# Gabrielcb/DaliID

Measured on AMD Instinct MI355X. Metric: images/sec (train step), higher is better.
Workload: dtype bf16; 1 GPU; configs[1]: ResNet-50 ReID bf16 256x128, PK batch 16x16=256 per GPU, center+proxy heads, Adam, EMA; global_batch=256, per_gpu_batch=256, parallelism=dp1

## Files before the change

### daliid_amd/_lib.py

```python
import ctypes
import os
import threading

import torch

_HERE = os.path.dirname(os.path.abspath(__file__))
LIB_PATH = os.environ.get("DALIID_LIB") or os.path.join(_HERE, "libdaliid_hip.so")

c_void_p, c_int, c_float, c_size_t = ctypes.c_void_p, ctypes.c_int, ctypes.c_float, ctypes.c_size_t


class DaliError(RuntimeError):
    pass


_SIGNATURES = {
    "dali_version": [],
    "dali_last_error": [],
    "dali_ctx_create": [c_int, ctypes.POINTER(c_void_p)],
    "dali_ctx_destroy": [c_void_p],
    "dali_ctx_reserve": [c_void_p, c_size_t],
    "dali_comm_unique_id": [c_void_p],
    "dali_ctx_comm_init": [c_void_p, c_void_p, c_int, c_int],
    "dali_ctx_comm_destroy": [c_void_p],
    "dali_allreduce_bucket": [c_void_p, c_void_p, c_void_p, ctypes.c_int64],
    "dali_l2norm_rows": [c_void_p, c_void_p, c_void_p, c_int, c_int, c_float, c_void_p, c_void_p],
    "dali_l2norm_rows_bwd": [c_void_p, c_void_p, c_void_p, c_void_p, c_int, c_int, c_float, c_void_p],
    "dali_pairdist": [c_void_p, c_void_p, c_void_p, c_void_p, c_int, c_int, c_int, c_int, c_int, c_int, c_void_p],
    "dali_pairdist_operand_bytes": [c_int, c_int, c_int],
    "dali_pairdist_prepare": [c_void_p, c_void_p, c_void_p, c_int, c_int, c_int, c_int, c_void_p, c_void_p],
    "dali_pairdist_prepared": [c_void_p, c_void_p, c_void_p, c_void_p, c_void_p, c_void_p, c_int, c_int, c_int, c_int, c_int,
                               c_void_p],
    "dali_rank_eval": [c_void_p, c_void_p, c_void_p, c_void_p, c_void_p, c_void_p, c_void_p, c_int, c_int, c_int,
                       c_void_p, c_void_p, c_void_p, c_void_p, c_void_p, c_void_p, c_void_p],
    "dali_rank_shard_matches": [c_void_p] * 7 + [c_int] * 4 + [c_void_p] * 3,
    "dali_rank_shard_bins": [c_void_p] * 7 + [c_int] * 3 + [c_void_p, c_void_p, c_int, c_int, c_void_p, c_int, c_void_p],
    "dali_rank_shard_finish": [c_void_p] * 4 + [c_int] * 4 + [c_void_p] * 6,
    "dali_rerank": [c_void_p] * 5 + [c_int] * 4 + [ctypes.c_double, c_void_p],
    "dali_roc_scratch_bytes": [c_int, c_int],
    "dali_roc_build": [c_void_p] * 5 + [c_int, c_int, c_void_p, c_size_t, c_void_p],
    "dali_roc_emit": [c_void_p] * 3 + [c_int, c_int, c_int, ctypes.c_int64, c_void_p, c_void_p, c_void_p],
    "dali_topk_rows": [c_void_p, c_void_p, c_void_p, c_int, c_int, ctypes.c_int64, c_int, c_int, c_int, c_int, c_void_p],
    "dali_topk_decode": [c_void_p, c_void_p, c_void_p, c_int, c_int, c_int, c_void_p, c_void_p],
    "dali_pairdist_topk_scratch_bytes": [c_int] * 7,
    "dali_pairdist_topk": [c_void_p] * 6 + [c_int] * 9 + [c_void_p] + [c_int] * 3 + [c_void_p],
    "dali_conv2d_fwd": [c_void_p, c_void_p, c_void_p, c_void_p, c_void_p] + [c_int] * 9 + [c_void_p, c_void_p, c_int, c_void_p],
    "dali_conv2d_bn_act": [c_void_p, c_void_p, c_void_p, c_void_p, c_void_p] + [c_int] * 9 + [c_void_p, c_void_p, c_int],
    "dali_stem_fused_supported": [c_int, c_int, c_int],
    "dali_stem_conv_bn_maxpool": [c_void_p, c_void_p, c_void_p, c_int, c_int, c_int, c_void_p, c_void_p, c_void_p, c_void_p],
    "dali_conv2d_stat_tiles": [c_int] * 10,
    "dali_conv2d_dgrad": [c_void_p, c_void_p, c_void_p, c_void_p, c_void_p, c_void_p, c_void_p] + [c_int] * 9,
    "dali_conv2d_wgrad": [c_void_p, c_void_p, c_void_p, c_void_p, c_void_p] + [c_int] * 9 + [c_void_p, c_void_p, c_int, c_int],
    "dali_conv1x1_fused": [c_void_p] * 5 + [c_int] * 3 + [c_void_p] * 4 + [c_int, c_void_p, c_void_p, c_void_p],
    "dali_conv1x1_cat": [c_void_p, c_void_p, c_void_p, c_int, c_void_p, c_int, c_void_p, c_void_p, c_void_p, c_int, c_int],
    "dali_conv1x1_cat_act": [c_void_p, c_void_p, c_void_p, c_int, c_void_p, c_int, c_void_p, c_int, c_void_p, c_void_p, c_int, c_void_p, c_int, c_int],
    "dali_bnlin_fwd": [c_void_p] * 4 + [c_int] * 3 + [c_void_p] * 4 + [c_float, c_float] + [c_void_p] * 7,
    "dali_bnlin_bwd": [c_void_p] * 5 + [c_int] * 3 + [c_void_p] * 11,
    "dali_bn_finalize": [c_void_p, c_void_p, c_void_p, c_int, c_int, ctypes.c_double, c_void_p, c_void_p, c_void_p, c_void_p,
                         c_float, c_float, c_void_p, c_void_p, c_void_p, c_void_p],
    "dali_bn_act": [c_void_p] * 9 + [c_int, ctypes.c_int64, c_int, c_void_p, c_void_p],
    "dali_bn_bwd": [c_void_p, c_void_p, c_void_p, c_void_p, c_void_p, c_int, ctypes.c_int64, c_int] + [c_void_p] * 16,
    "dali_maxpool_bn_fwd": [c_void_p] * 5 + [c_int] * 4 + [c_void_p, c_void_p],
    "dali_maxpool_bn_bwd": [c_void_p] * 8 + [c_int] * 4 + [c_void_p, c_void_p, c_void_p],
    "dali_head_pool_fwd": [c_void_p, c_void_p, c_void_p, c_int, c_int, c_int, c_int, c_void_p, c_void_p],
    "dali_head_pool_bwd": [c_void_p, c_void_p, c_void_p, c_void_p, c_int, c_int, c_int, c_int, c_void_p],
    "dali_bn1d_fwd": [c_void_p, c_void_p, c_void_p, c_int, c_int, c_void_p, c_void_p, c_void_p, c_void_p, c_int, c_float, c_float,
                      c_void_p, c_void_p, c_void_p],
    "dali_bn1d_bwd": [c_void_p, c_void_p, c_void_p, c_void_p, c_int, c_int] + [c_void_p] * 6,
    "dali_linear_fwd": [c_void_p] * 5 + [c_int] + [c_void_p] * 3 + [c_int] * 3,
    "dali_linear_fwd_scaled": [c_void_p] * 5 + [c_int] + [c_void_p] * 3 + [c_int] * 3,
    "dali_linear_dgrad": [c_void_p] * 7 + [c_int] * 3,
    "dali_linear_wgrad": [c_void_p] * 6 + [c_int] * 3,
    "dali_vit_patchify": [c_void_p, c_void_p, c_void_p] + [c_int] * 5 + [c_void_p],
    "dali_vit_assemble_tokens": [c_void_p] * 5 + [c_int] * 3 + [c_void_p],
    "dali_vit_assemble_tokens_bwd": [c_void_p] * 3 + [c_int] * 3 + [c_void_p] * 3,
    "dali_vit_assemble_tokens_sie": [c_void_p] * 7 + [c_int, c_float] + [c_int] * 3 + [c_void_p],
    "dali_vit_sie_grad": [c_void_p] * 4 + [c_int] * 4 + [c_float, c_void_p],
    "dali_vit_jpm_gather": [c_void_p] * 4 + [c_int] * 5 + [c_void_p],
    "dali_vit_jpm_head": [c_void_p] * 8 + [c_int] * 3 + [c_void_p],
    "dali_layernorm_fwd": [c_void_p] * 5 + [c_int, c_int, c_float] + [c_void_p] * 3,
    "dali_layernorm_bwd": [c_void_p] * 8 + [c_int, c_int] + [c_void_p] * 3,
    "dali_attention_fwd": [c_void_p] * 3 + [c_int] * 4 + [c_float, c_void_p, c_void_p],
    "dali_attention_fwd_short": [c_void_p] * 3 + [c_int] * 4 + [c_float, c_void_p, c_void_p],
    "dali_attention_bwd": [c_void_p] * 6 + [c_int] * 4 + [c_float, c_void_p],
    "dali_center_loss_fwd": [c_void_p] * 6 + [c_float, c_int, c_int, c_void_p, c_void_p],
    "dali_center_loss_bwd": [c_void_p] * 6 + [c_float, c_int, c_int, c_void_p, c_float, c_void_p],
    "dali_proxy_loss_fwd": [c_void_p] * 6 + [c_float, c_int, c_int] + [c_void_p] * 5,
    "dali_proxy_loss_bwd": [c_void_p] * 5 + [c_int, c_int, c_void_p, c_float, c_int, c_void_p],
    "dali_proxy_kmax": [],
    "dali_adam_step": [c_void_p] * 6 + [ctypes.c_int64, c_float, c_float, c_float, c_float, c_float, c_int, c_float, c_void_p],
    "dali_ema_update": [c_void_p, c_void_p, c_void_p, c_void_p, ctypes.c_int64, c_float],
    "dali_triplet_loss_fwd": [c_void_p, c_void_p, c_void_p, c_void_p, c_void_p, c_float, c_int, c_void_p, c_void_p, c_void_p, c_void_p,
                              c_void_p],
    "dali_triplet_loss_bwd": [c_void_p, c_void_p, c_void_p, c_void_p, c_int, c_void_p, c_float, c_void_p],
    "dali_pairdist_blend": [c_void_p, c_void_p, c_void_p, c_void_p, c_int, c_int, c_int, c_int, c_int, c_void_p, c_void_p, c_void_p,
                            c_void_p, c_void_p],
    "dali_class_targets": [c_void_p, c_void_p, c_void_p, c_int, c_int, c_void_p, c_void_p, c_int, c_void_p, c_int, c_void_p, c_void_p,
                           c_void_p, c_void_p],
    "dali_resize_bicubic_u8": [c_void_p] * 7 + [c_int, c_int, c_void_p, c_void_p, c_int, c_void_p, c_void_p, c_int, c_int, c_int, c_void_p],
    "dali_augment_batch": [c_void_p, c_void_p, c_void_p, c_void_p, c_int, c_int, c_int, ctypes.POINTER(c_float), ctypes.POINTER(c_float), c_void_p],
    "dali_augment_gather": [c_void_p, c_void_p, c_void_p, ctypes.c_int64, c_void_p, c_void_p, c_int, c_int, c_int, ctypes.POINTER(c_float),
                            ctypes.POINTER(c_float), c_void_p],
    "dali_gemm_profile_begin": [c_void_p, c_int],
    "dali_gemm_profile_end": [c_void_p, c_void_p, c_void_p, c_void_p],
    "dali_resnet_create": [c_void_p, c_void_p, ctypes.POINTER(c_void_p)],
    "dali_resnet_destroy": [c_void_p],
    "dali_resnet_set_feature": [c_void_p, c_int],
    "dali_resnet_sizes": [c_void_p] + [c_void_p] * 6,
    "dali_resnet_tensor_info": [c_void_p, c_int, c_int, c_void_p, c_int, c_void_p, c_void_p, c_void_p, c_void_p],
    "dali_resnet_stage_param_range": [c_void_p, c_int, c_void_p, c_void_p],
    "dali_resnet_bind": [c_void_p, c_void_p, c_void_p, c_void_p, c_void_p, c_size_t],
    "dali_resnet_refresh_weights": [c_void_p, c_void_p],
    "dali_resnet_forward": [c_void_p, c_void_p, c_void_p, c_int, c_void_p],
    "dali_resnet_backward": [c_void_p, c_void_p, c_void_p, c_int, c_int],
    "dali_resnet_debug_tensor": [c_void_p, ctypes.c_char_p, c_void_p, c_void_p],
    "dali_vit_create": [c_void_p, c_void_p, ctypes.POINTER(c_void_p)],
    "dali_vit_create_ex": [c_void_p, c_void_p, c_void_p, ctypes.POINTER(c_void_p)],
    "dali_vit_destroy": [c_void_p],
    "dali_vit_sizes": [c_void_p] + [c_void_p] * 6,
    "dali_vit_tensor_info": [c_void_p, c_int, c_int, c_void_p, c_int, c_void_p, c_void_p, c_void_p, c_void_p],
    "dali_vit_bind": [c_void_p, c_void_p, c_void_p, c_void_p, c_void_p, c_size_t],
    "dali_vit_refresh_weights": [c_void_p, c_void_p],
    "dali_vit_forward": [c_void_p, c_void_p, c_void_p, c_int, c_void_p, c_void_p],
    "dali_vit_forward_ex": [c_void_p, c_void_p, c_void_p, c_void_p, c_int, c_void_p, c_void_p, c_void_p],
    "dali_vit_backward": [c_void_p, c_void_p, c_void_p],
    "dali_vit_num_stages": [c_void_p],
    "dali_vit_stage_param_range": [c_void_p, c_int, c_void_p, c_void_p],
    "dali_vit_backward_stages": [c_void_p, c_void_p, c_void_p, c_int, c_int],
    "dali_vit_set_drop_path": [c_void_p, c_void_p],
}
_RESTYPES = {"dali_last_error": ctypes.c_char_p, "dali_pairdist_operand_bytes": ctypes.c_size_t, "dali_roc_scratch_bytes": ctypes.c_size_t,
             "dali_pairdist_topk_scratch_bytes": ctypes.c_size_t}

_lock = threading.Lock()
# ... 90 lines not shown
```

### daliid_amd/csrc/conv.hip

```cpp
#include "gemm_tile.h"
#include "kernels.h"
#include <cstdlib>
#include <type_traits>
#include <vector>
#include <string>
#include <cstdio>

namespace dali {

__device__ __forceinline__ void decode_pixel(const GatherGeom& g, int p, int& n, int& ho, int& wo) {
    if (g.lhw >= 0 && g.lw >= 0) {
        n = p >> g.lhw;
        const int rem = p & ((1 << g.lhw) - 1);
        ho = rem >> g.lw;
        wo = rem & ((1 << g.lw) - 1);
    } else {
        const int hw = g.Hout * g.Wout;
        n = p / hw;
        const int rem = p - n * hw;
        ho = rem / g.Wout;
        wo = rem - ho * g.Wout;
    }
}

// ... 86 lines not shown
        X = a.X; sc = a.in_scale; sh = a.in_shift; g = a.g; relu = a.in_relu;
        kc = threadIdx.x & 3;
        tiles_per_tap = g.Ck >> 5;
#pragma unroll
        for (int i = 0; i < BCH; ++i) {
            const int row = (threadIdx.x + i * 256) >> 2;
            const int p = p0 + row;
            ok[i] = p < a.P;
            int n = 0, ho = 0, wo = 0;
            if (ok[i]) decode_pixel(g, p, n, ho, wo);
            img_base[i] = (long long)n * g.img_pitch;
            if (g.mode == 0) { h0[i] = ho * g.stride - g.pad; w0[i] = wo * g.stride - g.pad; }
            else { h0[i] = ho + g.pad; w0[i] = wo + g.pad; }
        }
    }
    __device__ __forceinline__ uint4 operator()(int , int row, int kt, int ) const {
        const int i = row >> 6;
        const int tap = kt / tiles_per_tap;
        const int c0 = (kt - tap * tiles_per_tap) * 32 + kc * 8;
        const int r = tap / g.S, s = tap - r * g.S;
        long long off = -1;
#pragma unroll
        for (int t = 0; t < BCH; ++t)
            if (t == i && ok[t]) off = tap_offset(g, img_base[t], h0[t], w0[t], r, s);
        if (off < 0) return make_uint4(0, 0, 0, 0);
        uint4 v = *reinterpret_cast<const uint4*>(X + off + c0);
        if constexpr (IN_BN) v = bn_relu_chunk(v, sc + c0, sh + c0, relu);
        return v;
    }
};

struct WeightLoader {
    const uint16_t* W; int m0, Cm, K;
    __device__ __forceinline__ uint4 operator()(int , int row, int kt, int kc) const {
        const int m = m0 + row;
        if (m >= Cm) return make_uint4(0, 0, 0, 0);
        return *reinterpret_cast<const uint4*>(W + (size_t)m * K + kt * 32 + kc * 8);
    }
};

__device__ __forceinline__ void lds_barrier() {
    asm volatile("s_waitcnt lgkmcnt(0)" ::: "memory");
    __builtin_amdgcn_s_barrier();
}
__device__ __forceinline__ void lds_barrier_vm() {
    asm volatile("s_waitcnt vmcnt(0) lgkmcnt(0)" ::: "memory");
    __builtin_amdgcn_s_barrier();
}

__device__ __forceinline__ float row16_sum(float v) {
    v += __builtin_bit_cast(float, __builtin_amdgcn_update_dpp(0, __builtin_bit_cast(int, v), 0x128, 0xf, 0xf, false));
    v += __builtin_bit_cast(float, __builtin_amdgcn_update_dpp(0, __builtin_bit_cast(int, v), 0x124, 0xf, 0xf, false));
    v += __builtin_bit_cast(float, __builtin_amdgcn_update_dpp(0, __builtin_bit_cast(int, v), 0x122, 0xf, 0xf, false));
    v += __builtin_bit_cast(float, __builtin_amdgcn_update_dpp(0, __builtin_bit_cast(int, v), 0x121, 0xf, 0xf, false));
    return v;
}

#define DALI_DPP(v, CTRL) __builtin_bit_cast(float, __builtin_amdgcn_update_dpp(0, __builtin_bit_cast(int, (v)), (CTRL), 0xf, 0xf, false))
__device__ __forceinline__ float row16_reduce8(const float (&v)[8], int lane) {
    const bool hi8 = (lane & 8) != 0, hi4 = (lane & 4) != 0, hi2 = (lane & 2) != 0;
    float a[4], b[2];
#pragma unroll
    for (int k = 0; k < 4; ++k) {
        const float keep = hi8 ? v[4 + k] : v[k], send = hi8 ? v[k] : v[4 + k];
        a[k] = keep + DALI_DPP(send, 0x140);
    }
#pragma unroll
    for (int k = 0; k < 2; ++k) {
        const float keep = hi4 ? a[2 + k] : a[k], send = hi4 ? a[k] : a[2 + k];
        b[k] = keep + DALI_DPP(send, 0x141);
    }
    const float keep = hi2 ? b[1] : b[0], send = hi2 ? b[0] : b[1];
    const float c = keep + DALI_DPP(send, 0x4e);
    return c + DALI_DPP(c, 0xb1);
}

enum class Epi : int {
    CONV = 0,
    LIN = 1,
    GENERAL = 2,
    FUSED = 3,
    PARITY = 4,
    FUSED_LEAN = 5,
};
constexpr Epi epi_mode(bool own, Epi asked) { return own ? asked : Epi::GENERAL; }
constexpr bool epi_fused(Epi m) { return m == Epi::FUSED || m == Epi::FUSED_LEAN; }

__device__ __forceinline__ uint32_t gate_bf16x2(uint32_t w, unsigned bits) {
    const uint32_t lo = (uint32_t)__builtin_amdgcn_sbfe((int)bits, 0, 1) & 0xffffu;
    const uint32_t hi = (uint32_t)__builtin_amdgcn_sbfe((int)bits, 1, 1) << 16;
    return w & (lo | hi);
}
__device__ __forceinline__ void gate_bf16x8(uint4& v, unsigned m) {
    v.x = gate_bf16x2(v.x, m); v.y = gate_bf16x2(v.y, m >> 2); v.z = gate_bf16x2(v.z, m >> 4); v.w = gate_bf16x2(v.w, m >> 6);
}
__device__ __forceinline__ void gelu_parts(float v, float& cdf, float& pdf) {
    const float z = fabsf(v) * 0.70710678118654752f;
    const float e = __builtin_amdgcn_exp2f(-(z * z) * 1.44269504088896341f);
    const float t = __builtin_amdgcn_rcpf(__builtin_fmaf(0.3275911f, z, 1.0f));
    float poly = __builtin_fmaf(1.061405429f, t, -1.453152027f);
    poly = __builtin_fmaf(poly, t, 1.421413741f);
    poly = __builtin_fmaf(poly, t, -0.284496736f);
    poly = __builtin_fmaf(poly, t, 0.254829592f);
    const float erf_abs = __builtin_fmaf(-(poly * t), e, 1.0f);
    cdf = __builtin_fmaf(0.5f, copysignf(erf_abs, v), 0.5f);
    pdf = 0.3989422804014327f * e;
}
__device__ __forceinline__ float gelu_f(float v) { float c, p; gelu_parts(v, c, p); return v * c; }
__device__ __forceinline__ float gelu_grad_f(float x) { float c, p; gelu_parts(x, c, p); return __builtin_fmaf(x, p, c); }
__device__ __forceinline__ void unpack4(uint2 q, float (&f)[4]) {
    f[0] = bf16_bits_to_f32(q.x & 0xffffu); f[1] = bf16_bits_to_f32(q.x >> 16); f[2] = bf16_bits_to_f32(q.y & 0xffffu); f[3] = bf16_bits_to_f32(q.y >> 16);
}
__device__ __forceinline__ uint2 pack4(const float (&v)[4]) { return make_uint2(pack_bf16x2(v[0], v[1]), pack_bf16x2(v[2], v[3])); }
template <int FM>
__device__ __forceinline__ void load_rows4(float4 (&d)[FM], const float* vec) {
#pragma unroll
    for (int i = 0; i < FM; ++i) d[i] = *reinterpret_cast<const float4*>(vec + i * 16);
}
__device__ __forceinline__ unsigned pos_bits_bf16x2(uint32_t w) {
    return ((int)(int16_t)(w & 0xffffu) > 0 ? 1u : 0u) | (((int)w >> 16) > 0 ? 2u : 0u);
}
template <int TM, int TN, int FM_, int FN_, int WNW, int NT>
__device__ __forceinline__ void conv_epilogue_cols(const IGemmArgs& a, f32x4_t (&acc)[FM_][FN_], int tm, int tn, uint16_t* smem, int wm, int wn) {
    constexpr int ROWB = TM * 4 + 16, ROWS = WNW * 16, CPR = TM / 8, ITERS = ROWS * CPR / NT;
    static_assert(ROWS * CPR % NT == 0 && NT % CPR == 0, "staged store: threads must tile the column block evenly");
    const int lane = threadIdx.x & 63;
    const int mb = wm * (FM_ * 16) + (lane >> 4) * 4;
    char* stage = reinterpret_cast<char*>(smem);
    char* my_stage = stage + (wn * 16 + (lane & 15)) * ROWB + mb * 4;
    const int ch = threadIdx.x % CPR, lp0 = threadIdx.x / CPR;
    const uint16_t* in_tile = a.Res ? a.Res : a.dact_pre;
    const float* bias_c = a.bias ? a.bias + tm * TM + ch * 8 : nullptr;
#pragma unroll
    for (int j = 0; j < FN_; ++j) {
        uint32_t gofs[ITERS];
        uint4 tin[ITERS];
#pragma unroll
        for (int it = 0; it < ITERS; ++it) {
            const int lp = lp0 + it * (NT / CPR);
            const int pix = tn * TN + (lp >> 4) * (FN_ * 16) + j * 16 + (lp & 15);
            gofs[it] = ((uint32_t)pix * (uint32_t)a.Cm + (uint32_t)(tm * TM + ch * 8)) * 2u;
            if (in_tile) tin[it] = *reinterpret_cast<const uint4*>(reinterpret_cast<const char*>(in_tile) + gofs[it]);
        }
#pragma unroll
        for (int i = 0; i < FM_; ++i) *reinterpret_cast<f32x4_t*>(my_stage + i * 64) = acc[i][j];
        lds_barrier();
#pragma unroll
        for (int it = 0; it < ITERS; ++it) {
            const int lp = lp0 + it * (NT / CPR);
            float v[8];
            *reinterpret_cast<float4*>(v) = *reinterpret_cast<const float4*>(stage + lp * ROWB + ch * 32);
            *reinterpret_cast<float4*>(v + 4) = *reinterpret_cast<const float4*>(stage + lp * ROWB + ch * 32 + 16);
            if (bias_c) {
                const float4 b0 = *reinterpret_cast<const float4*>(bias_c), b1 = *reinterpret_cast<const float4*>(bias_c + 4);
                v[0] += b0.x; v[1] += b0.y; v[2] += b0.z; v[3] += b0.w; v[4] += b1.x; v[5] += b1.y; v[6] += b1.z; v[7] += b1.w;
            }
            if (a.O2) *reinterpret_cast<uint4*>(reinterpret_cast<char*>(a.O2) + gofs[it]) = pack8(v);
            if (a.act == 1) {
#pragma unroll
                for (int t = 0; t < 8; ++t) v[t] = gelu_f(v[t]);
            }
            if (a.dact_pre) {
                float x8[8];
                unpack8(tin[it], x8);
#pragma unroll
                for (int t = 0; t < 8; ++t) v[t] *= gelu_grad_f(x8[t]);
            }
            if (a.row_scale) {
// ... 43 lines not shown
    __device__ __forceinline__ uint4 in(const uint16_t* src, int h, int it) const {
        return *reinterpret_cast<const uint4*>(reinterpret_cast<const char*>(src) + offset(h, it));
    }
    __device__ __forceinline__ void out(uint16_t* dst, int h, int it) const {
        *reinterpret_cast<uint4*>(reinterpret_cast<char*>(dst) + offset(h, it)) = *chunk(it);
    }
};

template <int TM, int TN, int FM, int FN, int WNW, int NT>
__device__ __forceinline__ void epi_stats(const IGemmArgs& a, f32x4_t (&acc)[FM][FN], int tm, int tn, uint16_t* smem, int wn, int mb) {
    const int lane = threadIdx.x & 63;
    float* red = reinterpret_cast<float*>(reinterpret_cast<char*>(smem) + epi_stage_bytes(TM, TN));
#pragma unroll
    for (int i = 0; i < FM; ++i) {
        float s1[4] = {0.f, 0.f, 0.f, 0.f}, s2[4] = {0.f, 0.f, 0.f, 0.f};
#pragma unroll
        for (int j = 0; j < FN; ++j)
#pragma unroll
            for (int r = 0; r < 4; ++r) { const float v = acc[i][j][r]; s1[r] += v; s2[r] = __builtin_fmaf(v, v, s2[r]); }
        const float v8[8] = {s1[0], s1[1], s1[2], s1[3], s2[0], s2[1], s2[2], s2[3]};
        const float tot = row16_reduce8(v8, lane);
        if ((lane & 1) == 0) {
            const int r = ((lane & 4) >> 1) | ((lane & 2) >> 1);
            red[(wn * TM + mb + i * 16 + r) * 2 + ((lane >> 3) & 1)] = tot;
        }
    }
    lds_barrier();
    for (int t = threadIdx.x; t < TM; t += NT) {
        const int c = tm * TM + t;
        if (c < a.Cm) {
            float s1 = 0.f, s2 = 0.f;
#pragma unroll
            for (int w = 0; w < WNW; ++w) { const float2 v = *reinterpret_cast<const float2*>(red + (w * TM + t) * 2); s1 += v.x; s2 += v.y; }
            *reinterpret_cast<float2*>(a.stats + ((size_t)tn * a.Cm + c) * 2) = make_float2(s1, s2);
        }
    }
}
template <bool SUB, int TM, int TN, int FM, int FN, int WNW, int NT>
__device__ __forceinline__ void epi_store_lean(const IGemmArgs& a, f32x4_t (&acc)[FM][FN], int tm, int tn, uint16_t* smem, int wn, int mb) {
    using Stage = EpiStage<SUB, TM, TN, FM, FN, WNW, NT>;
    constexpr int ITERS = Stage::ITERS;
    const Stage st(a, tm, tn, smem, wn, mb);
    float4 bias4[FM];
#pragma unroll
    for (int i = 0; i < FM; ++i)
        bias4[i] = a.bias ? *reinterpret_cast<const float4*>(a.bias + tm * TM + mb + i * 16) : make_float4(0.f, 0.f, 0.f, 0.f);
#pragma unroll
    for (int h = 0; h < 2; ++h) {
        if (a.Res) {
            unsigned rm[ITERS];
            if (a.res_mask) {
#pragma unroll
                for (int it = 0; it < ITERS; ++it) rm[it] = a.res_mask[st.offset(h, it) >> 4];
            }
#pragma unroll
            for (int it = 0; it < ITERS; ++it) {
                uint4 rv = st.in(a.Res, h, it);
                if (a.res_mask) gate_bf16x8(rv, rm[it]);
                *st.chunk(it) = rv;
            }
            lds_barrier_vm();
        }
#pragma unroll
        for (int jj = 0; jj < Stage::HFN; ++jj) {
            const int j = h * Stage::HFN + jj;
#pragma unroll
            for (int i = 0; i < FM; ++i) {
                float v[4] = {acc[i][j][0] + bias4[i].x, acc[i][j][1] + bias4[i].y, acc[i][j][2] + bias4[i].z, acc[i][j][3] + bias4[i].w};
                uint2* slot = st.slot(jj, i);
                if (a.Res) {
                    float r4[4];
                    unpack4(*slot, r4);
                    v[0] += r4[0]; v[1] += r4[1]; v[2] += r4[2]; v[3] += r4[3];
                }
                *slot = pack4(v);
            }
        }
        lds_barrier();
        conv_stamp(a, 6 + 2 * h);
#pragma unroll
        for (int it = 0; it < ITERS; ++it) st.out(a.O, h, it);
        conv_stamp(a, 7 + 2 * h);
        if (h == 0) lds_barrier();
    }
}
template <int TM, int TN, int FM, int FN, int WNW, int NT>
__device__ __forceinline__ void epi_store_lin(const IGemmArgs& a, f32x4_t (&acc)[FM][FN], int tm, int tn, uint16_t* smem, int wn, int mb) {
    using Stage = EpiStage<false, TM, TN, FM, FN, WNW, NT>;
    constexpr int ITERS = Stage::ITERS;
    const Stage st(a, tm, tn, smem, wn, mb);
    const int lane = threadIdx.x & 63;
    float4 bias4[FM];
#pragma unroll
    for (int i = 0; i < FM; ++i)
        bias4[i] = a.bias ? *reinterpret_cast<const float4*>(a.bias + tm * TM + mb + i * 16) : make_float4(0.f, 0.f, 0.f, 0.f);
    const uint16_t* in_tile = a.Res ? a.Res : a.dact_pre;
#pragma unroll
    for (int h = 0; h < 2; ++h) {
        if (a.O2) {
#pragma unroll
            for (int jj = 0; jj < Stage::HFN; ++jj) {
                const int j = h * Stage::HFN + jj;
#pragma unroll
                for (int i = 0; i < FM; ++i) {
                    const float v[4] = {acc[i][j][0] + bias4[i].x, acc[i][j][1] + bias4[i].y, acc[i][j][2] + bias4[i].z, acc[i][j][3] + bias4[i].w};
                    *st.slot(jj, i) = pack4(v);
                }
            }
            lds_barrier();
#pragma unroll
            for (int it = 0; it < ITERS; ++it) st.out(a.O2, h, it);
            lds_barrier();
        }
        if (in_tile) {
#pragma unroll
            for (int it = 0; it < ITERS; ++it) *st.chunk(it) = st.in(in_tile, h, it);
            lds_barrier_vm();
        }
#pragma unroll
        for (int jj = 0; jj < Stage::HFN; ++jj) {
            const int j = h * Stage::HFN + jj;
#pragma unroll
            for (int i = 0; i < FM; ++i) {
                float v[4] = {acc[i][j][0] + bias4[i].x, acc[i][j][1] + bias4[i].y, acc[i][j][2] + bias4[i].z, acc[i][j][3] + bias4[i].w};
                uint2* slot = st.slot(jj, i);
                if (a.act == 1) {
#pragma unroll
                    for (int t = 0; t < 4; ++t) v[t] = gelu_f(v[t]);
                }
                if (a.row_scale) {
                    const float rs = a.row_scale[tn * TN + h * Stage::WROWS + wn * (FN * 16) + jj * 16 + (lane & 15)];
                    v[0] *= rs; v[1] *= rs; v[2] *= rs; v[3] *= rs;
                }
                if (in_tile) {
                    float x4[4];
                    unpack4(*slot, x4);
                    if (a.Res) {
                        v[0] += x4[0]; v[1] += x4[1]; v[2] += x4[2]; v[3] += x4[3];
                    } else {
#pragma unroll
                        for (int t = 0; t < 4; ++t) v[t] *= gelu_grad_f(x4[t]);
                    }
                }
                *slot = pack4(v);
            }
        }
        lds_barrier();
        conv_stamp(a, 6 + 2 * h);
#pragma unroll
        for (int it = 0; it < ITERS; ++it) st.out(a.O, h, it);
        conv_stamp(a, 7 + 2 * h);
        if (h == 0) lds_barrier();
    }
}
template <bool FULL, int TM, int TN, int FM, int FN, int WNW, int NT>
__device__ __forceinline__ void epi_store_fused(const IGemmArgs& a, f32x4_t (&acc)[FM][FN], int tm, int tn, uint16_t* smem, int wn, int mb) {
    using Stage = EpiStage<false, TM, TN, FM, FN, WNW, NT>;
    constexpr int ITERS = Stage::ITERS;
    const Stage st(a, tm, tn, smem, wn, mb);
    const uint16_t* const Res = FULL ? a.Res : nullptr;
    const uint8_t* const out_mask = FULL ? a.out_mask : nullptr;
    uint8_t* const bits_out = FULL ? a.bits_out : nullptr;
    float4 sc4[FM], sh4[FM];
#pragma unroll
    for (int i = 0; i < FM; ++i) { sc4[i] = make_float4(1.f, 1.f, 1.f, 1.f); sh4[i] = make_float4(0.f, 0.f, 0.f, 0.f); }
    if (a.out_scale) load_rows4(sc4, a.out_scale + tm * TM + mb);
// ... 61 lines not shown
            if (bits_out) bits_out[ob >> 4] = (uint8_t)(pos_bits_bf16x2(v.x) | (pos_bits_bf16x2(v.y) << 2) | (pos_bits_bf16x2(v.z) << 4) | (pos_bits_bf16x2(v.w) << 6));
        }
        if (h == 0) lds_barrier();
    }
}
template <Epi MODE, int TM, int TN, int FM, int FN>
__device__ __forceinline__ void epi_store_general(const IGemmArgs& a, f32x4_t (&acc)[FM][FN], int tm, int tn, int mb, int nb) {
    const int lane = threadIdx.x & 63;
#pragma unroll
    for (int j = 0; j < FN; ++j) {
        const int p = tn * TN + nb + j * 16;
        const size_t opix = (p < a.P) ? out_pixel(a.g, p) : 0;
#pragma unroll
        for (int i = 0; i < FM; ++i) {
            const int c = tm * TM + mb + i * 16;
            unsigned nib = 0;
            if (p < a.P && c < a.Cm) {
                float v[4] = {acc[i][j][0], acc[i][j][1], acc[i][j][2], acc[i][j][3]};
                const size_t o = opix * a.Cm + c;
                if constexpr (epi_fused(MODE)) {
                    if (a.out_scale) { const float4 sv = *reinterpret_cast<const float4*>(a.out_scale + c); v[0] *= sv.x; v[1] *= sv.y; v[2] *= sv.z; v[3] *= sv.w; }
                    if (a.out_shift) { const float4 sv = *reinterpret_cast<const float4*>(a.out_shift + c); v[0] += sv.x; v[1] += sv.y; v[2] += sv.z; v[3] += sv.w; }
                }
                if (a.bias) {
                    const float4 bv = *reinterpret_cast<const float4*>(a.bias + c);
                    v[0] += bv.x; v[1] += bv.y; v[2] += bv.z; v[3] += bv.w;
                }
                if constexpr (MODE == Epi::LIN || MODE == Epi::GENERAL) {
                    if (a.O2) *reinterpret_cast<uint2*>(a.O2 + o) = pack4(v);
                    if (a.act == 1) {
#pragma unroll
                        for (int t = 0; t < 4; ++t) v[t] = gelu_f(v[t]);
                    }
                    if (a.dact_pre) {
                        float x4[4];
                        unpack4(*reinterpret_cast<const uint2*>(a.dact_pre + o), x4);
#pragma unroll
                        for (int t = 0; t < 4; ++t) v[t] *= gelu_grad_f(x4[t]);
                    }
                    if (a.row_scale) {
                        const float rs = a.row_scale[p];
                        v[0] *= rs; v[1] *= rs; v[2] *= rs; v[3] *= rs;
                    }
                }
                if (MODE != Epi::FUSED_LEAN && a.Res) {
                    uint2 rv = *reinterpret_cast<const uint2*>(a.Res + o);
                    if constexpr (MODE != Epi::FUSED) if (a.res_mask) {
                        const unsigned m = a.res_mask[o >> 3] >> (o & 4);
                        rv.x = gate_bf16x2(rv.x, m); rv.y = gate_bf16x2(rv.y, m >> 2);
                    }
                    float r4[4];
                    unpack4(rv, r4);
                    if constexpr (MODE == Epi::FUSED) if (a.res_scale) {
                        const float4 rs = *reinterpret_cast<const float4*>(a.res_scale + c);
                        r4[0] *= rs.x; r4[1] *= rs.y; r4[2] *= rs.z; r4[3] *= rs.w;
                    }
                    v[0] += r4[0]; v[1] += r4[1]; v[2] += r4[2]; v[3] += r4[3];
                }
                if constexpr (epi_fused(MODE)) if (a.out_relu) { v[0] = fmaxf(v[0], 0.f); v[1] = fmaxf(v[1], 0.f); v[2] = fmaxf(v[2], 0.f); v[3] = fmaxf(v[3], 0.f); }
                uint2 ov = pack4(v);
                if constexpr (MODE == Epi::FUSED) {
                    if (a.out_mask) {
                        const unsigned m = a.out_mask[o >> 3] >> (o & 4);
                        ov.x = gate_bf16x2(ov.x, m); ov.y = gate_bf16x2(ov.y, m >> 2);
                    }
                    nib = pos_bits_bf16x2(ov.x) | (pos_bits_bf16x2(ov.y) << 2);
                }
                *reinterpret_cast<uint2*>(a.O + o) = ov;
            }
            if constexpr (MODE == Epi::FUSED) {
                const unsigned other = __shfl_xor(nib, 16, 64);
                if (a.bits_out && p < a.P && c < a.Cm && ((lane >> 4) & 1) == 0) a.bits_out[(opix * a.Cm + c) >> 3] = (uint8_t)(nib | (other << 4));
            }
        }
    }
}

template <int TM, int TN, int FM, int FN, int WNW, int NT, Epi MODE = Epi::GENERAL>
__device__ __forceinline__ void conv_epilogue_g(const IGemmArgs& a, f32x4_t (&acc)[FM][FN], int tm, int tn, uint16_t* smem, int wm, int wn) {
    constexpr bool EVEN = FN % 2 == 0;
    constexpr bool FUSED = epi_fused(MODE), SUB = MODE == Epi::PARITY;
    const int lane = threadIdx.x & 63;
    const int mb = wm * (FM * 16) + (lane >> 4) * 4, nb = wn * (FN * 16) + (lane & 15);
    if (a.stats) epi_stats<TM, TN, FM, FN, WNW, NT>(a, acc, tm, tn, smem, wn, mb);
    conv_stamp(a, 5);
    const bool interior = (tm + 1) * TM <= a.Cm && (tn + 1) * TN <= a.P;
    const bool chunks = (a.Cm & 7) == 0;
    const bool extras = a.O2 || a.act != 0 || a.dact_pre || a.row_scale;
    const bool plain = !FUSED && !extras && (SUB || !a.g.sub) && chunks;
    const bool in_once = !(a.Res && a.dact_pre);
    if constexpr (!EVEN) {
        if (interior && !FUSED && !a.g.sub && chunks && in_once && (unsigned long long)a.P * a.Cm * 2ull < 0xffffffffull)
            return conv_epilogue_cols<TM, TN, FM, FN, WNW, NT>(a, acc, tm, tn, smem, wm, wn);
    } else if constexpr (FUSED) {
        if (interior && !a.g.sub && chunks) return epi_store_fused<MODE == Epi::FUSED, TM, TN, FM, FN, WNW, NT>(a, acc, tm, tn, smem, wn, mb);
    } else {
        if (interior && plain) return epi_store_lean<SUB, TM, TN, FM, FN, WNW, NT>(a, acc, tm, tn, smem, wn, mb);
        if constexpr (MODE == Epi::LIN)
            if (interior && !plain && !a.g.sub && chunks && in_once) return epi_store_lin<TM, TN, FM, FN, WNW, NT>(a, acc, tm, tn, smem, wn, mb);
    }
    epi_store_general<MODE, TM, TN, FM, FN>(a, acc, tm, tn, mb, nb);
}
template <class Cfg, Epi MODE = Epi::GENERAL>
__device__ __forceinline__ void conv_epilogue(const IGemmArgs& a, f32x4_t (&acc)[Cfg::FM][Cfg::FN], int tm, int tn, uint16_t* smem) {
    const int wave = threadIdx.x >> 6;
    conv_epilogue_g<Cfg::TM, Cfg::TN, Cfg::FM, Cfg::FN, 2, 256, MODE>(a, acc, tm, tn, smem, wave >> 1, wave & 1);
}

template <int TM, int TN, bool IN_BN>
__global__ __launch_bounds__(256) void igemm_conv_kernel(IGemmArgs a, int tiles_m, int tiles_n) {
    using Cfg = GemmCfg<TM, TN, 1, 1, 1>;
    extern __shared__ __attribute__((aligned(16))) uint16_t smem[];
    int tm, tn;
    if (!xcd_tile_map(blockIdx.x, tiles_m, tiles_n, tm, tn)) return;
    f32x4_t acc[Cfg::FM][Cfg::FN];
#pragma unroll
    for (int i = 0; i < Cfg::FM; ++i)
#pragma unroll
        for (int j = 0; j < Cfg::FN; ++j) acc[i][j] = f32x4_t{0.f, 0.f, 0.f, 0.f};
    const int K = a.g.R * a.g.S * a.g.Ck;
    WeightLoader la{a.W, tm * TM, a.Cm, K};
    PixelLoader<TN, IN_BN> lb;
    lb.init(a, tn * TN);
    gemm_mainloop<Cfg>(acc, la, lb, K >> 5, smem);

    conv_epilogue<Cfg>(a, acc, tm, tn, smem);
}


template <int KT, int TM, int TN, int NW, bool SRC2>
struct ConvGather {
    static_assert(KT == 32 || KT == 64, "k-tile depth");
    static constexpr int ROWS = 512 / KT;
    static constexpr int A_BLK = TM / ROWS / NW, B_BLK = (TN / ROWS + NW - 1) / NW;
    static constexpr bool B_RAGGED = (TN / ROWS) % NW != 0;
    static constexpr int NDMA = A_BLK + B_BLK;
    static_assert(TM % (ROWS * NW) == 0 && TN % ROWS == 0, "DMA pieces: whole pieces, the weight pieces evenly over the waves");
    static_assert(KT == 64 || !B_RAGGED, "k-tile 32: the pixel pieces must divide evenly over the waves");
    static_assert(KT == 32 || NW % 2 == 0, "k-tile 64: an even number of issuing waves (piece wave + NW * i keeps the wave's parity)");
    static_assert(!(SRC2 && B_RAGGED), "the two-tensor branch has no ragged skip");

    const GatherGeom& g;
    int wave, Ck1, Ck2;
    __amdgpu_buffer_rsrc_t rs_w, rs_x, rs_x2;
    int kc;
    uint32_t a_off[A_BLK];
    int b_pix[B_BLK], b_h0[B_BLK], b_w0[B_BLK];
    int kr, ks, kc0, ks_end, kr_end;

    __device__ __forceinline__ ConvGather(const IGemmArgs& a, const GatherGeom& g_, int tm, int tn, int wave_, int lane) : g(g_) {
        wave = wave_;
        const int K = g.R * g.S * g.Ck;
        rs_w = __builtin_amdgcn_make_buffer_rsrc(const_cast<uint16_t*>(a.W), 0, a.Cm * K * 2, 0x00020000);
        const long long x_bytes = SRC2 ? (long long)a.P * a.Ck1 * 2 : (long long)g.img_pitch * 2 * ((a.P + g.Hout * g.Wout - 1) / (g.Hout * g.Wout));
        rs_x = __builtin_amdgcn_make_buffer_rsrc(const_cast<uint16_t*>(a.X), 0, (int)x_bytes, 0x00020000);
        Ck1 = a.Ck1; Ck2 = g.Ck - a.Ck1;
        rs_x2 = __builtin_amdgcn_make_buffer_rsrc(const_cast<uint16_t*>(SRC2 ? a.X2 : a.X), 0, SRC2 ? (int)((long long)a.P * Ck2 * 2) : (int)x_bytes, 0x00020000);
        int r_in;
        if constexpr (KT == 32) { r_in = lane >> 2; kc = (lane & 3) ^ lds_swz(r_in); }
        else { r_in = lane >> 3; kc = (lane & 7) ^ (((wave & 1) << 2) | (r_in >> 1)); }
#pragma unroll
        for (int i = 0; i < A_BLK; ++i) {
            const int m = tm * TM + ROWS * (wave + NW * i) + r_in;
            a_off[i] = (m < a.Cm) ? (uint32_t)(m * K + kc * 8) * 2u : DMA_OOB;
        }
#pragma unroll
// ... 1255 lines not shown
    return (P + tn - 1) / tn;
}


struct GemmProfiler {
    std::vector<hipEvent_t> ev;
    std::vector<int> cls;
    std::vector<double> flops;
    std::vector<std::string> desc;
    size_t used = 0, cap = 0;
};
static GemmProfiler* g_prof = nullptr;
struct ProfScope {
    hipStream_t st; bool on = false; size_t i = 0;
    ProfScope(hipStream_t s, int cls, double flops, const char* what = "") : st(s) {
        if (!g_prof || g_prof->used >= g_prof->cap) return;
        on = true; i = g_prof->used++;
        g_prof->cls[i] = cls; g_prof->flops[i] = flops; g_prof->desc[i] = what;
        (void)hipEventRecord(g_prof->ev[2 * i], st);
    }
    ~ProfScope() { if (on) (void)hipEventRecord(g_prof->ev[2 * i + 1], st); }
};

int gemm_profile_begin(hipStream_t st, int cls, double flops, const char* what) {
    if (!g_prof || g_prof->used >= g_prof->cap) return -1;
    const size_t i = g_prof->used++;
    g_prof->cls[i] = cls; g_prof->flops[i] = flops; g_prof->desc[i] = what;
    (void)hipEventRecord(g_prof->ev[2 * i], st);
    return (int)i;
}
void gemm_profile_end(hipStream_t st, int slot) {
    if (slot >= 0 && g_prof) (void)hipEventRecord(g_prof->ev[2 * slot + 1], st);
}

enum GemmGrid {
    GRID_XCD,
    GRID_CLASSES,
    GRID_CUS,
    GRID_HALO,
    GRID_SPLITS,
    GRID_SPLITS8,
};
struct GemmKernel {
    const void* fn;
    int block;
    int lds;
    int tm, tn;
    GemmGrid grid;
    int plan_wgs = 0;
    int f1_rb = 0;
    mutable DeviceOnce once{};
};
template <class F> static const void* kfn(F* f) { return reinterpret_cast<const void*>(f); }
constexpr int ring_lds(int tm, int tn, int k_tile, int stages) { return (tm + tn) * k_tile * 2 * stages; }
constexpr int REG128_LDS = GemmCfg<128, 128, 1, 1, 1>::LDS_BYTES, REG64_LDS = GemmCfg<64, 256, 1, 1, 1>::LDS_BYTES;
constexpr int DMA128_LDS = REG128_LDS / 2 * 3, DMA64_LDS = REG64_LDS / 2 * 3;
constexpr int HALO64_LDS = (3 * 64 * 64 + HALO64_PX * 64) * 2;

static const GemmKernel
    CONV128_BN{kfn(&igemm_conv_kernel<128, 128, true>), 256, REG128_LDS, 128, 128, GRID_XCD},
    CONV128{kfn(&igemm_conv_kernel<128, 128, false>), 256, REG128_LDS, 128, 128, GRID_XCD},
    DMA128{kfn(&igemm_conv_dma_kernel<128, 128, 3>), 256, DMA128_LDS, 128, 128, GRID_XCD},
    DMA128_LIN{kfn(&igemm_conv_dma_kernel<128, 128, 3, Epi::LIN>), 256, DMA128_LDS, 128, 128, GRID_XCD},
    DMA128_FUSED{kfn(&igemm_conv_dma_kernel<128, 128, 3, Epi::FUSED>), 256, DMA128_LDS, 128, 128, GRID_XCD},
    DMA128_CLS{kfn(&igemm_conv_dma_kernel<128, 128, 3, Epi::PARITY>), 256, DMA128_LDS, 128, 128, GRID_CLASSES},
    DMA128_SRC2{kfn(&igemm_conv_dma_kernel<128, 128, 3, Epi::CONV, true>), 256, DMA128_LDS, 128, 128, GRID_XCD},
    CONV64_BN{kfn(&igemm_conv_kernel<64, 256, true>), 256, REG64_LDS, 64, 256, GRID_XCD},
    CONV64{kfn(&igemm_conv_kernel<64, 256, false>), 256, REG64_LDS, 64, 256, GRID_XCD},
    DMA64{kfn(&igemm_conv_dma_kernel<64, 256, 3>), 256, DMA64_LDS, 64, 256, GRID_XCD},
    DMA64_LEAN{kfn(&igemm_conv_dma_kernel<64, 256, 3, Epi::FUSED_LEAN>), 256, DMA64_LDS, 64, 256, GRID_XCD},
    DMA64_SRC2{kfn(&igemm_conv_dma_kernel<64, 256, 3, Epi::CONV, true>), 256, DMA64_LDS, 64, 256, GRID_XCD},
    K64S64{kfn(&igemm_conv_k64s_kernel<1, 4, 4, 2>), 512, ring_lds(64, 256, 64, 2), 64, 256, GRID_XCD},
    HALO64{kfn(&igemm_conv_halo64_kernel<3>), 512, HALO64_LDS, 64, 256, GRID_HALO},
    HALO64_LEAN{kfn(&igemm_conv_halo64_kernel<3, Epi::FUSED_LEAN>), 512, HALO64_LDS, 64, 256, GRID_HALO},
    WG128{kfn(&igemm_conv_wg_kernel<2, 4, 3>), 512, ring_lds(128, 256, 32, 3), 128, 256, GRID_XCD},
    WG128_LIN{kfn(&igemm_conv_wg_kernel<2, 4, 3, Epi::LIN>), 512, ring_lds(128, 256, 32, 3), 128, 256, GRID_XCD},
    WG128_FUSED{kfn(&igemm_conv_wg_kernel<2, 4, 3, Epi::FUSED>), 512, ring_lds(128, 256, 32, 3), 128, 256, GRID_XCD},
    WG128_CLS{kfn(&igemm_conv_wg_kernel<2, 4, 3, Epi::PARITY>), 512, ring_lds(128, 256, 32, 3), 128, 256, GRID_CLASSES},
    WG256{kfn(&igemm_conv_wg_kernel<4, 4, 4>), 1024, ring_lds(256, 256, 32, 4), 256, 256, GRID_XCD},
    K64S{kfn(&igemm_conv_k64s_kernel<2, 4, 8, 3>), 1024, ring_lds(128, 256, 64, 3), 128, 256, GRID_XCD},
    K64S_LIN{kfn(&igemm_conv_k64s_kernel<2, 4, 8, 3, 4, 4, Epi::LIN>), 1024, ring_lds(128, 256, 64, 3), 128, 256, GRID_XCD},
    K64S_LEAN{kfn(&igemm_conv_k64s_kernel<2, 4, 8, 3, 4, 4, Epi::FUSED_LEAN>), 1024, ring_lds(128, 256, 64, 3), 128, 256, GRID_XCD},
    K64S_SRC2{kfn(&igemm_conv_k64s_kernel<2, 4, 8, 3, 4, 4, Epi::CONV, true>), 1024, ring_lds(128, 256, 64, 3), 128, 256, GRID_XCD},
    K64{kfn(&igemm_conv_k64_kernel<4, 4, 2>), 1024, ring_lds(256, 256, 64, 2), 256, 256, GRID_XCD},
    K64_LIN{kfn(&igemm_conv_k64_kernel<4, 4, 2, 4, 4, Epi::LIN>), 1024, ring_lds(256, 256, 64, 2), 256, 256, GRID_XCD},
    K64_FUSED{kfn(&igemm_conv_k64_kernel<4, 4, 2, 4, 4, Epi::FUSED>), 1024, ring_lds(256, 256, 64, 2), 256, 256, GRID_XCD},
    K64_CLS{kfn(&igemm_conv_k64_kernel<4, 4, 2, 4, 4, Epi::PARITY>), 1024, ring_lds(256, 256, 64, 2), 256, 256, GRID_CLASSES},
    K64_SRC2{kfn(&igemm_conv_k64_kernel<4, 4, 2, 4, 4, Epi::CONV, true>), 1024, ring_lds(256, 256, 64, 2), 256, 256, GRID_XCD},
    K64_FUSED_SRC2{kfn(&igemm_conv_k64_kernel<4, 4, 2, 4, 4, Epi::FUSED, true>), 1024, ring_lds(256, 256, 64, 2), 256, 256, GRID_XCD},
    K64_320{kfn(&igemm_conv_k64_kernel<4, 4, 2, 4, 5, Epi::LIN>), 1024, ring_lds(256, 320, 64, 2), 256, 320, GRID_XCD};

template <int RB, bool RES, bool OM, bool BITS, bool SRC2 = false>
static GemmKernel f1_kernel() {
    return {kfn(&fused1x1_persist_kernel<3, RB, RES, OM, BITS, SRC2>), (F1_NC + F1_NP + F1_NR) * 64, f1_lds_bytes(3, RB, RB == 2 ? 128 : F1_KMAX),
            F1_TM, F1_TN, GRID_CUS, 0, RB};
}
static const GemmKernel F1[2][2][2][2] = {
    {{{f1_kernel<2, false, false, false, true>(), f1_kernel<2, false, false, true>()}, {f1_kernel<2, false, true, false>(), f1_kernel<2, false, true, true>()}},
     {{f1_kernel<2, true, false, false>(), f1_kernel<2, true, false, true>()}, {f1_kernel<2, true, true, false>(), f1_kernel<2, true, true, true>()}}},
    {{{f1_kernel<1, false, false, false, true>(), f1_kernel<1, false, false, true>()}, {f1_kernel<1, false, true, false>(), f1_kernel<1, false, true, true>()}},
     {{f1_kernel<1, true, false, false>(), f1_kernel<1, true, false, true>()}, {f1_kernel<1, true, true, false>(), f1_kernel<1, true, true, true>()}}}};

static const GemmKernel
    WG_BN{kfn(&igemm_wgrad_kernel<true>), 256, 0, 128, 128, GRID_SPLITS},
    WG_PLAIN{kfn(&igemm_wgrad_kernel<false>), 256, 0, 128, 128, GRID_SPLITS},
    WG_3X3{kfn(&igemm_wgrad3x3_kernel<3>), 512, 3 * W3_STAGE * 2, 128, 9 * 64, GRID_SPLITS8, 256};
static const GemmKernel WG_DMA[2] = {
    {kfn(&igemm_wgrad_dma_kernel<false>), 256, 0, 128, 128, GRID_SPLITS8},
    {kfn(&igemm_wgrad_dma_kernel<true>), 256, 0, 128, 128, GRID_SPLITS8}};
static const GemmKernel WG_WG[2] = {
    {kfn(&igemm_wgrad_wg_kernel<2, 4, 3>), 512, ring_lds(128, 256, 32, 3), 128, 256, GRID_SPLITS8, 512},
    {kfn(&igemm_wgrad_wg_kernel<2, 4, 3, true>), 512, ring_lds(128, 256, 32, 3), 128, 256, GRID_SPLITS8, 512}};
static const GemmKernel WG_P[2][2] = {
    {{kfn(&igemm_wgrad_p_kernel<2, 4, 4, 4, 8, 6>), 1024, ring_lds(128, 256, 32, 6), 128, 256, GRID_SPLITS8, 256},
     {kfn(&igemm_wgrad_p_kernel<2, 4, 4, 4, 8, 6, true>), 1024, ring_lds(128, 256, 32, 6), 128, 256, GRID_SPLITS8, 256}},
    {{kfn(&igemm_wgrad_p_kernel<1, 4, 8, 4, 4, 6>), 512, ring_lds(128, 256, 32, 6), 128, 256, GRID_SPLITS8, 256},
     {kfn(&igemm_wgrad_p_kernel<1, 4, 8, 4, 4, 6, true>), 512, ring_lds(128, 256, 32, 6), 128, 256, GRID_SPLITS8, 256}}};

struct GemmChoice {
    const GemmKernel* k = nullptr;
    int tiles_m = 0, tiles_n = 0, lds = 0, class_grid = 0;
    unsigned grid = 0;
    int rc = DALI_OK, why_arg = 0;
    const char* why = nullptr;
    GemmChoice() = default;
    GemmChoice(int rc_, const char* why_, int why_arg_ = 0) : rc(rc_), why_arg(why_arg_), why(why_) {}
    int refuse() const { set_error(why, why_arg); return rc; }
};
static GemmChoice gemm_place(const GemmKernel& k, int rows, int cols, int mult, int Ck) {
    GemmChoice c;
    c.k = &k;
    c.tiles_m = (rows + k.tm - 1) / k.tm;
    c.tiles_n = (cols + k.tn - 1) / k.tn;
    c.lds = k.f1_rb ? f1_lds_bytes(3, k.f1_rb, Ck) : k.lds;
    switch (k.grid) {
        case GRID_XCD: c.grid = xcd_tile_grid(c.tiles_m, c.tiles_n); break;
        case GRID_CLASSES: c.class_grid = xcd_tile_grid(c.tiles_m, c.tiles_n); c.grid = mult * c.class_grid; break;
        case GRID_CUS: c.grid = mult; break;
        case GRID_HALO: c.grid = c.tiles_n; break;
        case GRID_SPLITS: c.grid = c.tiles_m * c.tiles_n * mult; break;
        case GRID_SPLITS8: c.grid = (c.tiles_m * c.tiles_n * mult + 7) / 8 * 8; break;
    }
    return c;
}
template <class Args>
static int gemm_launch(hipStream_t st, const GemmChoice& c, Args& args) {
    const GemmKernel& k = *c.k;
    DeviceOnce::Guard once(k.once);
    if (k.lds > 64 * 1024 && once.first()) {
        DALI_HIP(hipFuncSetAttribute(k.fn, hipFuncAttributeMaxDynamicSharedMemorySize, k.lds));
        once.done();
    }
    int tiles_m = c.tiles_m, tiles_n = c.tiles_n;
    void* tile_args[] = {&args, &tiles_m, &tiles_n};
    void* halo_args[] = {&args, &tiles_n};
    (void)hipLaunchKernel(k.fn, dim3(c.grid), dim3(k.block), k.grid == GRID_HALO ? halo_args : tile_args, c.lds, st);
    DALI_LAUNCH_CHECK();
    return DALI_OK;
}

static unsigned long long* g_conv_stamps = nullptr;

static bool dma_addressable(long long bytes) { return bytes < 0x7ff00000ll; }
static bool gather_dma_ok(const GatherGeom& g, int P, long long other_bytes) {
    return dma_addressable(g.img_pitch * 2 * ((P + g.Hout * g.Wout - 1) / (g.Hout * g.Wout))) && dma_addressable(other_bytes);
}
static bool conv_dma_ok(const IGemmArgs& a) { return !a.in_scale && gather_dma_ok(a.g, a.P, (long long)a.Cm * a.g.R * a.g.S * a.g.Ck * 2); }
static bool plain_rows(const GatherGeom& g) {
    return g.R == 1 && g.S == 1 && g.stride == 1 && g.pad == 0 && g.pix_pitch == g.Ck && g.row_pitch == g.Win * g.Ck &&
           g.img_pitch == (long long)g.Hin * g.Win * g.Ck && g.Hin == g.Hout && g.Win == g.Wout;
}
static bool halo64_ok(const IGemmArgs& a) {
// ... 9 lines not shown
        int dev = 0, v = 0;
        if (hipGetDevice(&dev) != hipSuccess || hipDeviceGetAttribute(&v, hipDeviceAttributeMultiprocessorCount, dev) != hipSuccess) { set_error("conv: device query failed"); return -1; }
        n_cus = v > 8 ? v & ~7 : 8;
    }
    return n_cus;
}
static bool f1_fills(int Cm, int P, int n_cus) {
    const int tiles_m = Cm / F1_TM, tiles_n = (P + F1_TN - 1) / F1_TN;
    return n_cus > 0 && (long long)tiles_m * tiles_n >= 2ll * n_cus && (n_cus / 8) % tiles_m == 0;
}
static bool cat_act_ok(int Cm, int c1, int c2, int P, int parts, int n_cus) {
    const int K = parts * (c1 + c2);
    if (parts != 1 && parts != 2) return false;
    if ((c1 & 63) || (c2 & 63) || (Cm % 128) || !dma_addressable((long long)P * Cm * 2) || !dma_addressable((long long)P * K * 2)) return false;
    if (K <= F1_KMAX) return f1_fills(Cm, P, n_cus);
    return parts == 1 && K >= 1024 && conv_pick_cfg(Cm, P, K) == CONV_256x256;
}
bool conv_cat_act_supported(int Cm, int c1, int c2, int P, int parts) { return cat_act_ok(Cm, c1, c2, P, parts, f1_cu_count()); }

static GemmChoice conv_choose(const IGemmArgs& a, int n_cus) {
    const GatherGeom& g = a.g;
    const bool in_bn = a.in_scale != nullptr, narrow = a.Cm <= 64, dma_ok = conv_dma_ok(a);
    const int K = g.nr * g.ns * g.Ck;
    const bool fused = a.out_scale || a.out_shift || a.out_relu || a.bits_out || a.out_mask || a.res_scale;
    const bool lin = a.act != 0 || a.O2 != nullptr || a.dact_pre != nullptr || a.row_scale != nullptr;
    if (a.res_mask && (fused || lin))
        return GemmChoice(DALI_ERR_INVALID, "conv: a residual mask goes with neither a fused output stage nor the linear-layer extras");
    int cfg = conv_pick_cfg(a.Cm, a.P, K);
    if (dma_ok && !a.stats && !fused && !g.sub && g.Ck % 64 == 0 && (a.Cm & 7) == 0 && conv_prefers_320(a.Cm, a.P, K)) cfg = CONV_256x320;
    if (!dma_ok && !in_bn && a.stats && (cfg == CONV_128x256 || cfg == CONV_256x256))
        return GemmChoice(DALI_ERR_LIMIT, "conv: tensors beyond 2 GiB are not supported together with the BatchNorm statistics epilogue");
    bool k64 = dma_ok && !narrow && g.Ck % 64 == 0;
    const bool narrow_k64 = dma_ok && narrow && g.Ck % 64 == 0 && K >= 512 && !a.X2;
    if (a.X2) {
        const bool fo_simple = !a.bits_out && !a.out_mask && !a.res_scale && !a.Res && (a.out_scale || a.out_shift || a.out_relu);
        const int xr = a.x_rep > 1 ? a.x_rep : 1, c2 = g.Ck / xr - a.Ck1;
        if (xr > 1 && !(fo_simple && g.Ck % xr == 0 && cat_act_ok(a.Cm, a.Ck1, c2, a.P, xr, n_cus) && g.Ck <= F1_KMAX))
            return GemmChoice(DALI_ERR_INVALID, "conv: split weight images (x_rep = %d) are served by the persistent streaming kernel only (K <= 256, >= 2 tiles per CU)", xr);
        if (fo_simple && ((a.Ck1 & 63) || (c2 & 63) || (a.Cm % 128)))
            return GemmChoice(DALI_ERR_INVALID, "conv: two operand tensors with a fused output stage need channel counts that are multiples of 64 and Cm %% 128 == 0");
        if (in_bn || !dma_ok || a.stats || (fused && !fo_simple) || lin || g.sub || g.R != 1 || g.S != 1 || g.stride != 1 || g.pad != 0 || a.Ck1 <= 0 ||
            a.Ck1 >= g.Ck / xr || (a.Ck1 & 31) || (c2 & 31) || (a.Cm & 7))
            return GemmChoice(DALI_ERR_INVALID, "conv: a second operand tensor needs a plain 1x1 / stride 1 problem with both channel counts multiples of 32");
        if ((a.Ck1 & 63) || (c2 & 63)) k64 = false;
    }
    if (k64 && cfg != CONV_256x320 && !((K >= 1024 && (cfg == CONV_256x256 || cfg == CONV_128x256)) || (K >= 768 && cfg == CONV_256x256))) k64 = false;
    if (a.X2 && !narrow && !(k64 && (cfg == CONV_256x256 || cfg == CONV_128x256))) { cfg = CONV_128; k64 = false; }
    auto use = [&](const GemmKernel& k) { return gemm_place(k, a.Cm, a.P, k.grid == GRID_CUS ? n_cus : (g.sub == 2 ? 4 : 1), g.Ck); };
    if (fused) {
        if (in_bn || !dma_ok || (a.Cm & 7) || lin)
            return GemmChoice(DALI_ERR_INVALID, "conv: the fused output stage needs Cm %% 8 == 0, tensors below 2 GiB, no operand transform and no linear-layer extras");
        if (plain_rows(g) && !g.sub && a.Cm % F1_TM == 0 && (g.Ck & 63) == 0 && g.Ck <= F1_KMAX && dma_addressable((long long)a.P * a.Cm * 2) &&
            (a.Res || a.out_mask || a.bits_out || a.X2)) {
            if (n_cus <= 0) return GemmChoice(DALI_ERR_HIP, "conv: device query failed");
            if (f1_fills(a.Cm, a.P, n_cus)) return use(F1[g.Ck > 128][a.Res != nullptr][a.out_mask != nullptr][a.bits_out != nullptr]);
        }
        const bool lean = !a.Res && !a.out_mask && !a.bits_out && !a.res_scale && !a.X2;
        if (lean && narrow_k64 && halo64_ok(a)) return use(HALO64_LEAN);
        if (lean && narrow) return use(DMA64_LEAN);
        if (lean && k64 && cfg == CONV_128x256 && !g.sub) return use(K64S_LEAN);
        if (a.X2) {
            if (!(k64 && cfg == CONV_256x256))
                return GemmChoice(DALI_ERR_INVALID, "conv: two operand tensors with a fused output stage need K <= 256 or a 256 x 256 k-tile-64 problem (K >= 1024, Cm >= 512, >= 16384 pixels)");
            return use(K64_FUSED_SRC2);
        }
        if (k64 && cfg == CONV_256x256) return use(K64_FUSED);
        return use(cfg == CONV_128x256 || cfg == CONV_256x256 ? WG128_FUSED : DMA128_FUSED);
    }
    if (g.sub && dma_ok && !narrow && !lin && (a.Cm & 7) == 0) {
        if (k64 && cfg == CONV_256x256) return use(K64_CLS);
        return use(cfg == CONV_128x256 || cfg == CONV_256x256 ? WG128_CLS : DMA128_CLS);
    }
    if (cfg == CONV_256x320) return use(K64_320);
    if (k64 && cfg == CONV_256x256) return use(a.X2 ? K64_SRC2 : lin ? K64_LIN : K64);
    if (k64 && cfg == CONV_128x256) return use(a.X2 ? K64S_SRC2 : lin ? K64S_LIN : K64S);
    if (narrow_k64 && !lin && halo64_ok(a)) return use(HALO64);
    if (narrow_k64) return use(K64S64);
    if (narrow) return use(in_bn ? CONV64_BN : !dma_ok ? CONV64 : a.X2 ? DMA64_SRC2 : DMA64);
    if (dma_ok && cfg == CONV_256x256) return use(WG256);
    if (dma_ok && cfg == CONV_128x256) return use(lin ? WG128_LIN : WG128);
    return use(in_bn ? CONV128_BN : !dma_ok ? CONV128 : a.X2 ? DMA128_SRC2 : lin ? DMA128_LIN : DMA128);
}

static int launch_igemm_conv_one(hipStream_t st, const IGemmArgs& a) {
    IGemmArgs args = a;
    args.g.lw = ilog2_exact(a.g.Wout);
    args.g.lhw = ilog2_exact(a.g.Hout * a.g.Wout);
    const GemmChoice c = conv_choose(args, f1_cu_count());
    if (c.rc == DALI_ERR_LIMIT) return c.refuse();
    const int K = a.g.nr * a.g.ns * a.g.Ck;
    char what[160] = "";
    if (g_prof)
        snprintf(what, sizeof what, "%s,Cm=%d,K=%d,P=%d,taps=%d,stride=%d,sub=%d,fused=%d,stats=%d,res=%d,mask=%d,lin=%d", a.g.mode ? "dgrad" : "fwd", a.Cm, K, a.P,
                 a.g.R * a.g.S, a.g.stride, a.g.sub, a.out_scale ? 1 : 0, a.stats ? 1 : 0, a.Res ? 1 : 0, (a.res_mask || a.out_mask) ? 1 : 0,
                 (a.bias || a.row_scale || a.act) ? 1 : 0);
    ProfScope prof_scope(st, 0, a.g.sub == 2 ? 2.0 * a.Cm * (double)a.P * a.g.R * a.g.S * a.g.Ck : 2.0 * a.Cm * (double)a.P * K, what);
    if (!c.k) return c.refuse();
    const int stat_tiles = a.stats ? igemm_conv_stat_tiles(a.Cm, a.P, K, a.in_scale != nullptr) : c.tiles_n;
    if (stat_tiles != c.tiles_n) {
        set_error("conv: the statistics slab has %d pixel tiles, the chosen kernel %d", stat_tiles, c.tiles_n);
        return DALI_ERR_UNSUPPORTED;
    }
    if (c.k->grid == GRID_CLASSES) args.g.class_grid = c.class_grid;
    return gemm_launch(st, c, args);
}

int launch_igemm_conv(hipStream_t st, const IGemmArgs& a) {
    IGemmArgs args = a;
    args.stamps = g_conv_stamps;
    GatherGeom& g = args.g;
    g.sub = 0; g.oph = g.opw = 0; g.Hfull = g.Hout; g.Wfull = g.Wout;
    g.r0 = 0; g.rstep = 1; g.nr = g.R; g.s0 = 0; g.sstep = 1; g.ns = g.S;
    if (g.mode == 1 && g.stride == 2 && conv_dma_ok(args) && !a.stats && (g.Hout % 2) == 0 && (g.Wout % 2) == 0 &&
        ilog2_exact(g.Wout / 2) >= 0 && ilog2_exact((g.Hout / 2) * (g.Wout / 2)) >= 0) {
        int nr[2], ns[2];
        for (int ph = 0; ph < 2; ++ph) {
            const int r0 = (ph + g.pad) & 1, s0 = (ph + g.pad) & 1;
            nr[ph] = r0 < g.R ? (g.R - r0 + 1) / 2 : 0;
            ns[ph] = s0 < g.S ? (g.S - s0 + 1) / 2 : 0;
        }
        const bool all_have = nr[0] && nr[1] && ns[0] && ns[1];
        if (all_have && a.Cm > 64 && (a.Cm & 7) == 0) {
            IGemmArgs s = args;
            s.g.sub = 2; s.g.oph = s.g.opw = 0; s.g.Hfull = g.Hout; s.g.Wfull = g.Wout;
            s.g.Hout = g.Hout / 2; s.g.Wout = g.Wout / 2; s.P = a.P / 4;
            s.g.r0 = s.g.s0 = 0; s.g.rstep = s.g.sstep = 2;
            s.g.nr = nr[0] > nr[1] ? nr[0] : nr[1]; s.g.ns = ns[0] > ns[1] ? ns[0] : ns[1];
            return launch_igemm_conv_one(st, s);
        }
        if (all_have || (a.Res != nullptr && a.Res == a.O)) {
            for (int ph = 0; ph < 2; ++ph)
                for (int pw = 0; pw < 2; ++pw) {
                    if (nr[ph] * ns[pw] == 0) continue;
                    IGemmArgs s = args;
                    s.g.sub = 1; s.g.oph = ph; s.g.opw = pw; s.g.Hfull = g.Hout; s.g.Wfull = g.Wout;
                    s.g.Hout = g.Hout / 2; s.g.Wout = g.Wout / 2; s.P = a.P / 4;
                    s.g.r0 = (ph + g.pad) & 1; s.g.rstep = 2; s.g.nr = nr[ph];
                    s.g.s0 = (pw + g.pad) & 1; s.g.sstep = 2; s.g.ns = ns[pw];
                    const int rc = launch_igemm_conv_one(st, s);
                    if (rc) return rc;
                }
            return DALI_OK;
        }
    }
    return launch_igemm_conv_one(st, args);
}

static bool wgrad_spec(int Cm, int Ntot) { return ((Cm + 127) / 128) * ((Ntot + 255) / 256) <= 100; }
static int wgrad_pick_cfg(int Cm, int Ntot, int taps, int P, int halo_w) {
    if (taps == 9 && (halo_w == 8 || halo_w == 16 || halo_w == 32) && Cm % 64 == 0 && (Ntot / 9) % 64 == 0 && P % 32 == 0) return 3;
    if (taps == 7 && Ntot == 224 && P >= 16384) return 2;
    return (taps == 1 && Ntot >= 256 && P >= 16384) ? 2 : 0;
}
static const GemmKernel& wgrad_kernel(int cfg, int Cm, int Ntot, bool in_bn, bool dma_ok, bool colsum, bool flat) {
    if (in_bn) return WG_BN;
    if (!dma_ok) return WG_PLAIN;
    if (cfg == 3) return WG_3X3;
    if (cfg == 2) return wgrad_spec(Cm, Ntot) ? WG_P[flat][colsum] : WG_WG[colsum];
    return WG_DMA[colsum];
}
static bool wgrad_colsum_ok(int cfg, bool in_bn, bool dma_ok) { return cfg != 3 && !in_bn && dma_ok; }
static int colsum_rows_of(const GemmKernel& k, int Ntot, int splits) { return k.tn == 128 ? splits : splits * ((Ntot + k.tn - 1) / k.tn); }

static void wgrad_plan(int Cm, int Ntot, int P, int target_blocks, int* splits, int* pix_per_split, int taps, int halo_w) {
    const GemmKernel& k = wgrad_kernel(wgrad_pick_cfg(Cm, Ntot, taps, P, halo_w), Cm, Ntot, false, true, false, true);
    if (k.plan_wgs) target_blocks = k.plan_wgs;
    const int tiles = ((Cm + k.tm - 1) / k.tm) * ((Ntot + k.tn - 1) / k.tn);
    int sp = (target_blocks + tiles - 1) / tiles;
    const int max_sp = (P + 255) / 256;
    if (sp > max_sp) sp = max_sp;
    if (sp < 1) sp = 1;
    {
        int best = sp;
        double best_cost = (double)((tiles * sp + target_blocks - 1) / target_blocks) / sp;
        for (int c = sp - 1; c >= 1 && c >= sp / 2; --c) {
            const double cost = (double)((tiles * c + target_blocks - 1) / target_blocks) / c;
            if (cost <= best_cost + 1e-12) { best = c; best_cost = cost; }
        }
        sp = best;
    }
    int pps = ((P + sp - 1) / sp + 31) & ~31;
    sp = (P + pps - 1) / pps;
    *splits = sp; *pix_per_split = pps;
}

static int wgrad_halo_w(const GatherGeom& g, bool in_bn) {
    const bool halo = !in_bn && g.R == 3 && g.S == 3 && g.stride == 1 && g.pad == 1 && g.mode == 0 && ilog2_exact(g.Wout) >= 0 &&
                      ilog2_exact(g.Hout * g.Wout) >= 7 && g.Hin == g.Hout && g.Win == g.Wout && g.pix_pitch == g.Ck && g.row_pitch == g.Win * g.Ck;
    return halo ? g.Wout : 0;
}

struct WGradChoice { int Ntot, splits, pix_per_split, colsum_rows; GemmChoice c; };
static WGradChoice wgrad_choose(int Cm, int P, const GatherGeom& g, bool in_bn, bool want_colsum) {
    WGradChoice w{};
    const int taps = g.R * g.S, halo_w = wgrad_halo_w(g, in_bn);
    w.Ntot = taps * g.Ck;
    wgrad_plan(Cm, w.Ntot, P, 512, &w.splits, &w.pix_per_split, taps, halo_w);
    const int cfg = wgrad_pick_cfg(Cm, w.Ntot, taps, P, halo_w);
    const bool dma_ok = gather_dma_ok(g, P, (long long)P * Cm * 2);
    const bool colsum = want_colsum && wgrad_colsum_ok(cfg, in_bn, dma_ok);
    w.c = gemm_place(wgrad_kernel(cfg, Cm, w.Ntot, in_bn, dma_ok, colsum, plain_rows(g)), Cm, w.Ntot, w.splits, g.Ck);
    w.colsum_rows = colsum ? colsum_rows_of(*w.c.k, w.Ntot, w.splits) : 0;
    return w;
}

WGradNeed wgrad_need(int Cm, int P, const GatherGeom& g, bool colsum, bool operand_transform) {
    const WGradChoice w = wgrad_choose(Cm, P, g, operand_transform, colsum);
    return WGradNeed{(size_t)w.splits * Cm * w.Ntot * sizeof(float), colsum ? std::max((size_t)w.colsum_rows * Cm, colsum_partial_floats(P, Cm)) : 0};
}

int launch_wgrad(hipStream_t st, WGradArgs a, const WGradBufs& ws, float* out, int accumulate, float* colsum_out) {
    const WGradChoice w = wgrad_choose(a.Cm, a.P, a.g, a.in_scale != nullptr, colsum_out != nullptr);
    a.Ntot = w.Ntot; a.splits = w.splits; a.pix_per_split = w.pix_per_split;
    a.partial = ws.slab;
    a.colsum = w.colsum_rows ? ws.cs_partial : nullptr;
    a.stamps = g_conv_stamps;
    a.g.lw = ilog2_exact(a.g.Wout);
    a.g.lhw = ilog2_exact(a.g.Hout * a.g.Wout);
    {
    char what[160] = "";
    if (g_prof)
        snprintf(what, sizeof what, "wgrad,Cm=%d,K=%d,P=%d,taps=%d,stride=%d,sub=0,fused=%d,stats=0,res=0,mask=0,lin=%d", a.Cm, a.Ntot, a.P, a.g.R * a.g.S, a.g.stride,
                 a.in_scale ? 1 : 0, a.colsum ? 1 : 0);
    ProfScope prof_scope(st, 1, 2.0 * a.Cm * (double)a.Ntot * a.P, what);
    if (int rc = gemm_launch(st, w.c, a)) return rc;
    }
    if (int rc = launch_splitk_reduce2(st, a.partial, out, (size_t)a.Cm * a.Ntot, a.splits, accumulate, a.colsum, colsum_out, (size_t)a.Cm, w.colsum_rows)) return rc;
    if (!colsum_out || a.colsum) return DALI_OK;
// ... 54 lines not shown
}

extern "C" int dali_gemm_profile_end(dali_ctx* ctx, double* total_ms, double* total_flops, long long* launches) {
    DALI_REQUIRE(ctx && total_ms && total_flops && launches, "dali_gemm_profile_end: null argument");
    DALI_REQUIRE(g_prof, "dali_gemm_profile_end: no open profile");
    GemmProfiler* p = g_prof;
    g_prof = nullptr;
    for (int c = 0; c < 2; ++c) { total_ms[c] = 0; total_flops[c] = 0; launches[c] = 0; }
    int rc = DALI_OK;
    const char* dump_path = getenv("DALI_GEMM_PROFILE_DUMP");
    FILE* dump = dump_path ? fopen(dump_path, "a") : nullptr;
    for (size_t i = 0; i < p->used; ++i) {
        float ms = 0.f;
        if (hipEventSynchronize(p->ev[2 * i + 1]) != hipSuccess || hipEventElapsedTime(&ms, p->ev[2 * i], p->ev[2 * i + 1]) != hipSuccess) {
            set_error("gemm_profile_end: event query failed"); rc = DALI_ERR_HIP; break;
        }
        total_ms[p->cls[i]] += ms; total_flops[p->cls[i]] += p->flops[i]; launches[p->cls[i]] += 1;
        if (dump) fprintf(dump, "%zu,%s,us=%.2f,gflop=%.3f\n", i, p->desc[i].c_str(), ms * 1e3, p->flops[i] * 1e-9);
    }
    if (dump) fclose(dump);
    for (auto& e : p->ev) (void)hipEventDestroy(e);
    delete p;
    return rc;
}

static int fill_geom(GatherGeom& g, int n_img, int Hin, int Win, int Ck, int Hout, int Wout, int R, int S, int stride, int pad, int mode) {
    g.Hout = Hout; g.Wout = Wout; g.Hin = Hin; g.Win = Win; g.Ck = Ck; g.R = R; g.S = S; g.stride = stride; g.pad = pad;
    g.mode = mode;
    g.pix_pitch = Ck; g.row_pitch = Win * Ck; g.img_pitch = (long long)Hin * Win * Ck;
    g.lw = g.lhw = -1;
    (void)n_img;
    return 0;
}

extern "C" int dali_conv2d_fwd(dali_ctx* ctx, void* stream, const uint16_t* x, const uint16_t* w, uint16_t* y,
                               int n, int h, int wd, int cin, int cout, int r, int s, int stride, int pad,
                               const float* in_scale, const float* in_shift, int in_relu, float* stats) {
    DALI_REQUIRE(ctx && x && w && y, "dali_conv2d_fwd: null argument");
    DALI_REQUIRE(cin % 32 == 0 && cout % 4 == 0, "dali_conv2d_fwd: cin must be a multiple of 32 and cout of 4 (cin=%d cout=%d)", cin, cout);
    DALI_REQUIRE(stride == 1 || stride == 2, "dali_conv2d_fwd: stride %d unsupported", stride);
    DALI_REQUIRE((in_scale == nullptr) == (in_shift == nullptr), "dali_conv2d_fwd: in_scale/in_shift must come together");
    const int ho = (h + 2 * pad - r) / stride + 1, wo = (wd + 2 * pad - s) / stride + 1;
    IGemmArgs a{};
    a.W = w; a.X = x; a.O = y; a.Res = nullptr; a.in_scale = in_scale; a.in_shift = in_shift; a.stats = stats;
    a.Cm = cout; a.P = n * ho * wo; a.in_relu = in_relu;
    fill_geom(a.g, n, h, wd, cin, ho, wo, r, s, stride, pad, 0);
    return launch_igemm_conv((hipStream_t)stream, a);
}

extern "C" int dali_conv2d_bn_act(dali_ctx* ctx, void* stream, const uint16_t* x, const uint16_t* w, uint16_t* y, int n, int h, int wd, int cin, int cout,
                                  int r, int s, int stride, int pad, const float* out_scale, const float* out_shift, int out_relu) {
    DALI_REQUIRE(ctx && x && w && y && out_scale && out_shift, "dali_conv2d_bn_act: null argument");
    DALI_REQUIRE(cin % 32 == 0 && cout % 8 == 0, "dali_conv2d_bn_act: cin must be a multiple of 32 and cout of 8 (cin=%d cout=%d)", cin, cout);
    DALI_REQUIRE(stride == 1 || stride == 2, "dali_conv2d_bn_act: stride %d unsupported", stride);
    const int ho = (h + 2 * pad - r) / stride + 1, wo = (wd + 2 * pad - s) / stride + 1;
    IGemmArgs a{};
    a.W = w; a.X = x; a.O = y;
    a.out_scale = out_scale; a.out_shift = out_shift; a.out_relu = out_relu;
    a.Cm = cout; a.P = n * ho * wo;
    fill_geom(a.g, n, h, wd, cin, ho, wo, r, s, stride, pad, 0);
    return launch_igemm_conv((hipStream_t)stream, a);
}

extern "C" int dali_conv2d_stat_tiles(int cout, int cin, int r, int s, int stride, int pad, int n, int ho, int wo, int fused_operand) {
    (void)stride; (void)pad;
    return igemm_conv_stat_tiles(cout, n * ho * wo, r * s * cin, fused_operand != 0);
}

extern "C" int dali_conv2d_dgrad(dali_ctx* ctx, void* stream, const uint16_t* dy, const uint16_t* wt, uint16_t* dx,
                                 const uint16_t* residual, const uint8_t* residual_mask, int n, int h, int wd, int cin, int cout, int r, int s,
                                 int stride, int pad) {
    DALI_REQUIRE(ctx && dy && wt && dx, "dali_conv2d_dgrad: null argument");
    DALI_REQUIRE(!residual_mask || (residual && cin % 8 == 0), "dali_conv2d_dgrad: residual_mask needs a residual and cin %% 8 == 0 (cin=%d)", cin);
    DALI_REQUIRE(cout % 32 == 0 && cin % 4 == 0, "dali_conv2d_dgrad: cout must be a multiple of 32 and cin of 4 (cin=%d cout=%d)", cin, cout);
    DALI_REQUIRE(stride == 1 || stride == 2, "dali_conv2d_dgrad: stride %d unsupported", stride);
    const int ho = (h + 2 * pad - r) / stride + 1, wo = (wd + 2 * pad - s) / stride + 1;
    IGemmArgs a{};
    a.W = wt; a.X = dy; a.O = dx; a.Res = residual; a.res_mask = residual_mask; a.in_scale = nullptr; a.in_shift = nullptr; a.stats = nullptr;
    a.Cm = cin; a.P = n * h * wd; a.in_relu = 0;
    fill_geom(a.g, n, ho, wo, cout, h, wd, r, s, stride, pad, 1);
    return launch_igemm_conv((hipStream_t)stream, a);
}

extern "C" int dali_conv2d_wgrad(dali_ctx* ctx, void* stream, const uint16_t* x, const uint16_t* dy, float* dw,
                                 int n, int h, int wd, int cin, int cout, int r, int s, int stride, int pad,
                                 const float* in_scale, const float* in_shift, int in_relu, int accumulate) {
    DALI_REQUIRE(ctx && x && dy && dw, "dali_conv2d_wgrad: null argument");
    DALI_REQUIRE(cin % 8 == 0 && cout % 8 == 0, "dali_conv2d_wgrad: cin and cout must be multiples of 8 (cin=%d cout=%d)", cin, cout);
    DALI_REQUIRE(stride == 1 || stride == 2, "dali_conv2d_wgrad: stride %d unsupported", stride);
    DALI_REQUIRE((in_scale == nullptr) == (in_shift == nullptr), "dali_conv2d_wgrad: in_scale/in_shift must come together");
    const int ho = (h + 2 * pad - r) / stride + 1, wo = (wd + 2 * pad - s) / stride + 1;
    WGradArgs a{};
    a.dY = dy; a.X = x; a.in_scale = in_scale; a.in_shift = in_shift; a.in_relu = in_relu;
    a.Cm = cout; a.P = n * ho * wo;
    fill_geom(a.g, n, h, wd, cin, ho, wo, r, s, stride, pad, 0);
    float* slab = static_cast<float*>(workspace(ctx, wgrad_need(a.Cm, a.P, a.g, false, in_scale != nullptr).slab_bytes));
    if (!slab) return DALI_ERR_NOMEM;
    return launch_wgrad((hipStream_t)stream, a, WGradBufs{slab, nullptr, nullptr}, dw, accumulate);
}

extern "C" int dali_conv1x1_fused(dali_ctx* ctx, void* stream, const uint16_t* x, const uint16_t* w, uint16_t* y, int pixels, int cin, int cout,
                                  const float* out_scale, const float* out_shift, const float* bias, const uint16_t* residual, int out_relu,
                                  uint8_t* bits_out, const uint8_t* out_mask, const float* res_scale) {
    DALI_REQUIRE(ctx && x && w && y, "dali_conv1x1_fused: null argument");
    DALI_REQUIRE(cin % 32 == 0 && cout % 8 == 0 && pixels > 0, "dali_conv1x1_fused: cin %% 32, cout %% 8 (cin=%d cout=%d)", cin, cout);
    IGemmArgs a{};
    a.W = w; a.X = x; a.O = y; a.Res = residual; a.bias = bias;
    a.out_scale = out_scale; a.out_shift = out_shift; a.out_relu = out_relu; a.bits_out = bits_out; a.out_mask = out_mask; a.res_scale = res_scale;
    a.Cm = cout; a.P = pixels;
    fill_geom(a.g, 1, 1, pixels, cin, 1, pixels, 1, 1, 1, 0, 0);
    return launch_igemm_conv((hipStream_t)stream, a);
}

extern "C" int dali_conv1x1_cat(dali_ctx* ctx, void* stream, const uint16_t* x1, int c1, const uint16_t* x2, int c2, const uint16_t* w, const float* bias,
                                uint16_t* y, int pixels, int cout) {
    DALI_REQUIRE(ctx && x1 && x2 && w && y, "dali_conv1x1_cat: null argument");
    DALI_REQUIRE(c1 > 0 && c2 > 0 && c1 % 32 == 0 && c2 % 32 == 0 && cout % 8 == 0 && pixels > 0, "dali_conv1x1_cat: c1 %% 32, c2 %% 32, cout %% 8 (c1=%d c2=%d cout=%d)", c1, c2, cout);
    IGemmArgs a{};
    a.W = w; a.X = x1; a.X2 = x2; a.Ck1 = c1; a.O = y; a.bias = bias;
    a.Cm = cout; a.P = pixels;
    fill_geom(a.g, 1, 1, pixels, c1 + c2, 1, pixels, 1, 1, 1, 0, 0);
    return launch_igemm_conv((hipStream_t)stream, a);
}

extern "C" int dali_conv1x1_cat_act(dali_ctx* ctx, void* stream, const uint16_t* x1, int c1, const uint16_t* x2, int c2, const uint16_t* w, int weight_parts,
                                    const float* out_scale, const float* out_shift, int out_relu, uint16_t* y, int pixels, int cout) {
    DALI_REQUIRE(ctx && x1 && x2 && w && y && out_shift, "dali_conv1x1_cat_act: null argument");
    DALI_REQUIRE(c1 > 0 && c2 > 0 && c1 % 64 == 0 && c2 % 64 == 0 && cout % 128 == 0 && pixels > 0, "dali_conv1x1_cat_act: c1 %% 64, c2 %% 64, cout %% 128 (c1=%d c2=%d cout=%d)", c1, c2, cout);
    IGemmArgs a{};
    DALI_REQUIRE(weight_parts == 1 || weight_parts == 2, "dali_conv1x1_cat_act: weight_parts must be 1 or 2");
    a.W = w; a.X = x1; a.X2 = x2; a.Ck1 = c1; a.x_rep = weight_parts; a.O = y;
    a.out_scale = out_scale; a.out_shift = out_shift; a.out_relu = out_relu;
    a.Cm = cout; a.P = pixels;
    fill_geom(a.g, 1, 1, pixels, weight_parts * (c1 + c2), 1, pixels, 1, 1, 1, 0, 0);
    return launch_igemm_conv((hipStream_t)stream, a);
}

static void linear_geom(GatherGeom& g, int K) {
    g.Hout = 1; g.Wout = 1; g.Hin = 1; g.Win = 1; g.Ck = K; g.R = 1; g.S = 1; g.stride = 1; g.pad = 0; g.mode = 0;
    g.pix_pitch = K; g.row_pitch = K; g.img_pitch = K; g.lw = g.lhw = -1;
}
namespace dali {
int launch_linear_fwd(hipStream_t st, const uint16_t* x, const uint16_t* w, const float* bias, int act, const uint16_t* residual, uint16_t* y,
                      uint16_t* pre, const uint16_t* dact_pre, int rows, int K, int N, const float* row_scale) {
    IGemmArgs a{};
    a.W = w; a.X = x; a.O = y; a.Res = residual; a.bias = bias; a.act = act; a.O2 = pre; a.dact_pre = dact_pre; a.row_scale = row_scale;
    a.Cm = N; a.P = rows;
    linear_geom(a.g, K);
    return launch_igemm_conv(st, a);
}
int launch_linear_wgrad(hipStream_t st, const uint16_t* x, const uint16_t* dy, float* dw, int rows, int K, int N, const WGradBufs& ws, float* dbias) {
    WGradArgs a{};
    a.dY = dy; a.X = x; a.Cm = N; a.P = rows;
    linear_geom(a.g, K);
    return launch_wgrad(st, a, ws, dw, 0, dbias);
}
WGradNeed linear_wgrad_need(int rows, int K, int N, bool bias) {
    GatherGeom g{};
    linear_geom(g, K);
    return wgrad_need(N, rows, g, bias);
}
}

extern "C" int dali_linear_fwd(dali_ctx* ctx, void* stream, const uint16_t* x, const uint16_t* w, const float* bias, int act,
                               const uint16_t* residual, uint16_t* y, uint16_t* pre, int rows, int K, int N) {
    DALI_REQUIRE(ctx && x && w && y, "dali_linear_fwd: null argument");
// ... 29 lines not shown
```

### daliid_amd/csrc/kernels.h

```cpp
#pragma once
#include "common.h"

namespace dali {

struct GatherGeom {
    int Hout, Wout;
    int Hin, Win;
    int Ck;
    int R, S, stride, pad;
    int mode;
    long long img_pitch;
    int row_pitch, pix_pitch;
    int lw, lhw;
    int sub, oph, opw, Hfull, Wfull;
    int r0, rstep, nr, s0, sstep, ns;
    int class_grid;
};

struct IGemmArgs {
    const uint16_t* W;
    const uint16_t* X;
    uint16_t* O;
    const uint16_t* Res;
    const uint8_t* res_mask;
    const float* in_scale;
    const float* in_shift;
    float* stats;
    const float* bias;
    uint16_t* O2;
    const uint16_t* dact_pre;
    int act;
    int Cm, P, in_relu;
    GatherGeom g;
    unsigned long long* stamps;
    const float* row_scale;
    const float* res_scale;
    const float* out_scale;
    const float* out_shift;
    int out_relu;
    uint8_t* bits_out;
    const uint8_t* out_mask;
    const uint16_t* X2;
    int Ck1;
    int x_rep;
};

struct WGradArgs {
    const uint16_t* dY;
    const uint16_t* X;
    float* partial;
    const float* in_scale; const float* in_shift;
    int Cm, P, Ntot, in_relu;
    int splits, pix_per_split;
    GatherGeom g;
    unsigned long long* stamps;
    float* colsum;
};


struct TransposeJob { const uint16_t* w; uint16_t* wt; int Co, T, Ci, first_block; };
int launch_weight_transpose_batched(hipStream_t st, const TransposeJob* jobs, int n);

struct BnBwdSide { const uint16_t* raw; const float* mean; const float* invstd; const float* scale; const float* shift; };

int launch_igemm_conv(hipStream_t st, const IGemmArgs& a);
int gemm_profile_begin(hipStream_t st, int cls, double flops, const char* what);
void gemm_profile_end(hipStream_t st, int slot);
int igemm_conv_stat_tiles(int Cm, int P, int K, bool operand_transform = false);
bool conv_cat_act_supported(int Cm, int c1, int c2, int P, int parts = 1);
struct WGradNeed { size_t slab_bytes, colsum_floats; };
WGradNeed wgrad_need(int Cm, int P, const GatherGeom& g, bool colsum, bool operand_transform = false);
struct WGradBufs { float* slab; float* cs_partial; double* scratch; };
int launch_wgrad(hipStream_t st, WGradArgs a, const WGradBufs& ws, float* out, int accumulate, float* colsum_out = nullptr);
int launch_splitk_reduce2(hipStream_t st, const float* partial, float* out, size_t elems, int splits, int accumulate,
                          const float* partial2, float* out2, size_t elems2, int splits2);
int launch_splitk_reduce(hipStream_t st, const float* partial, float* out, size_t elems, int splits, int accumulate);

int launch_linear_fwd(hipStream_t st, const uint16_t* x, const uint16_t* w, const float* bias, int act, const uint16_t* residual, uint16_t* y,
                      uint16_t* pre, const uint16_t* dact_pre, int rows, int K, int N, const float* row_scale = nullptr);
int launch_linear_wgrad(hipStream_t st, const uint16_t* x, const uint16_t* dy, float* dw, int rows, int K, int N, const WGradBufs& ws, float* dbias = nullptr);
WGradNeed linear_wgrad_need(int rows, int K, int N, bool bias);

int launch_bnlin_stats(hipStream_t st, const uint16_t* W, const uint16_t* Wt, const float* gram, const float* m2, int C, int w, double count, const float* gamma,
                       const float* beta, float* rm, float* rv, float momentum, float eps, float* ut, float* dot, float* scale, float* shift,
                       float* mean, float* invstd);
int launch_bnlin_ut(hipStream_t st, const uint16_t* W, const float* gram, int C, int w, float* ut);
int launch_bnlin_bwd(hipStream_t st, const uint16_t* W, const uint16_t* Wt, const float* ut, const float* m2, const float* s_dz, int C,
                     int w, double count, const float* scale, const float* mean, const float* invstd, float* dW, float* dgamma, float* dbeta,
                     uint16_t* wd1, uint16_t* wd2, float* bvec, float* qk, int ld1 = 0, int ld2 = 0);

constexpr int REDUCE_SMAX = 64;
inline size_t reduce_scratch_bytes(int C, int NV) { return (size_t)REDUCE_SMAX * C * NV * sizeof(double); }
int launch_bn_finalize(hipStream_t st, const float* partial, int tiles, int C, double count, const float* gamma, const float* beta,
                       float* rm, float* rv, float momentum, float eps, float* scale, float* shift, float* mean, float* invstd,
                       double* scratch);
struct BnEvalJob { const float *gamma, *beta, *rm, *rv; float *scale, *shift; int C; };
struct BnEvalJobs { static constexpr int MAX = 56; BnEvalJob job[MAX]; };
int launch_bn_eval_coeffs_batched(hipStream_t st, const BnEvalJob* jobs, int n, float eps);
int launch_fold_cat_weights(hipStream_t st, const float* w3, const float* wd, const float* s3, const float* sd, const float* h3, const float* hd, int C, int w,
                            int cin, int parts, uint16_t* wcat, float* shcat);
int launch_bn_act(hipStream_t st, const uint16_t* raw, const float* scale, const float* shift, const uint16_t* idn, const uint16_t* raw2,
                  const float* scale2, const float* shift2, int relu, size_t elems, int C, uint16_t* y, uint8_t* mask_out);
int bn_bwd_blocks(int P, int C, int* rows_per_block);
size_t bn_bwd_partial_floats(int P, int C, bool dual);
int launch_bn_bwd(hipStream_t st, const uint16_t* g, const uint16_t* ymask, const uint8_t* ybits, const BnBwdSide& a, const BnBwdSide* b, int relu, int P, int C,
                  float* partial, float* coef_a, float* coef_b, float* dgamma_a, float* dbeta_a, float* dgamma_b, float* dbeta_b,
                  uint16_t* draw_a, uint16_t* draw_b, uint16_t* dz_out, double* scratch);
GatherGeom stem_geom(int H, int W);
int launch_stem_pack_image(hipStream_t st, const float* img, int N, int H, int W, uint16_t* out);
int launch_stem_pack_weight(hipStream_t st, const float* w, int Cout, uint16_t* out);
bool stem_fused_supported(int N, int H, int W, int C);
bool stem_train_supported(int N, int H, int W, int C);
int stem_train_tiles(int N, int H);
int launch_stem_conv_stats(hipStream_t st, const uint16_t* ximg, const uint16_t* w_packed, int N, int H, int W, uint16_t* raw, float* stats);
int launch_stem_conv_bn_pool(hipStream_t st, const uint16_t* ximg, const uint16_t* w_packed, const float* scale, const float* shift, int N, int H, int W,
                             uint16_t* out);
int launch_stem_unpack_wgrad(hipStream_t st, const float* padded, int Cout, float* dw);
int launch_maxpool_bn_fwd(hipStream_t st, const uint16_t* raw, const float* scale, const float* shift, int N, int H, int W, int C,
                          uint16_t* out, uint8_t* arg);
int maxpool_bn_bwd_blocks(int N, int H, int W, int C, int* quads_per_block);
int launch_maxpool_bn_bwd(hipStream_t st, const uint16_t* dp, const uint8_t* arg, const uint16_t* raw, const float* mean, const float* invstd,
                          const float* scale, int N, int H, int W, int C, float* partial, float* coef, float* dgamma, float* dbeta,
                          uint16_t* draw, double* scratch);
int launch_head_pool_fwd(hipStream_t st, const uint16_t* x, int N, int HW, int C, int mode, float* f, int16_t* arg);
int launch_head_pool_bwd(hipStream_t st, const float* df, const int16_t* arg, int N, int HW, int C, int mode, uint16_t* dx, const uint8_t* ybits = nullptr);
int launch_bn1d_fwd(hipStream_t st, const float* x, int N, int C, const float* gamma, const float* beta, float* rm, float* rv, int training,
                    float momentum, float eps, float* y, float* mean, float* invstd);
int launch_bn1d_bwd(hipStream_t st, const float* x, const float* dy, int N, int C, const float* gamma, const float* mean, const float* invstd,
                    float* dx, float* dgamma, float* dbeta);
int launch_cast_bf16(hipStream_t st, const float* x, size_t n, uint16_t* y);
int launch_weight_transpose(hipStream_t st, const uint16_t* w, int Co, int T, int Ci, uint16_t* wt);


int launch_patchify(hipStream_t st, const float* img, int B, int H, int W, int ps, int stride, uint16_t* out);
int launch_assemble_tokens(hipStream_t st, const uint16_t* pe, const float* cls, const float* pos, int B, int T, int C, uint16_t* x);
int launch_assemble_tokens_bwd(hipStream_t st, const uint16_t* dx, int B, int T, int C, float* dpos, float* dcls, uint16_t* dpe);
int launch_layernorm_fwd(hipStream_t st, const uint16_t* x, const float* gamma, const float* beta, int rows, int C, float eps,
                         uint16_t* y, float* mean, float* rstd, float* y32);
size_t layernorm_bwd_partial_floats(int rows, int C);
int launch_layernorm_bwd(hipStream_t st, const uint16_t* g, const uint16_t* x, const float* gamma, const float* mean, const float* rstd,
                         const uint16_t* add, int rows, int C, uint16_t* dx, float* dgamma, float* dbeta, float* partial, double* scratch,
                         const float* g32 = nullptr);
size_t colsum_partial_floats(int rows, int C);
int launch_colsum(hipStream_t st, const uint16_t* y, int rows, int C, float* out, float* partial, double* scratch);
int launch_rowscale_add(hipStream_t st, const uint16_t* branch, const float* scale, int samples, int rows_per_sample, int C, const uint16_t* res,
                        uint16_t* out);
int launch_expand_rowscale(hipStream_t st, const float* scale, int n_vec, int B, int T, float* out);
int launch_attention_fwd(hipStream_t st, const uint16_t* qkv, int B, int T, int H, float scale, uint16_t* out, float* lse);
int launch_attention_fwd_short(hipStream_t st, const uint16_t* qkv, int B, int T, int H, float scale, uint16_t* out, float* lse);
int launch_assemble_tokens_sie(hipStream_t st, const uint16_t* pe, const float* cls, const float* pos, const float* sie, const int32_t* idx, int n_sie,
                               float coef, int B, int T, int C, uint16_t* x);
int launch_sie_grad(hipStream_t st, const uint16_t* dx, const int32_t* idx, int B, int T, int C, int n_sie, float coef, float* dsie);
int launch_jpm_gather(hipStream_t st, const uint16_t* feat, const int32_t* map, int B, int T, int C, int G, int L, uint16_t* out);
struct JpmNecks { const float *gamma[5], *beta[5], *rm[5], *rv[5]; };
int launch_jpm_head(hipStream_t st, const float* glob, const float* loc, const JpmNecks& nk, int B, int C, int after, float eps, float* out);
int launch_tokens_f32(hipStream_t st, const uint16_t* x, size_t elems, float* y);
int launch_attention_bwd(hipStream_t st, const uint16_t* qkv, const uint16_t* o, const uint16_t* d_o, const float* lse, int B, int T, int H,
                         float scale, uint16_t* dqkv);

struct PairTopk;
int pairdist_dma_max_rows(int d, bool split);
int launch_pairdist_matrix(int num_cus, hipStream_t st, const uint16_t* g_img, const float* gsq, const uint16_t* q_img, const float* qsq, int nq, int ng,
                           int d, int metric, bool split, float* out, const int* gate);
int launch_pairdist_select(int num_cus, hipStream_t st, const uint16_t* g_img, const float* gsq, const uint16_t* q_img, const float* qsq, int nq, int ng,
                           int d, int metric, bool split, const PairTopk& sel);

}
```

### daliid_amd/csrc/nnops.hip

```cpp
#include "kernels.h"
#include "reduce_finish.h"

namespace dali {

struct FinBnFwd {
    double count;
    const float *gamma, *beta;
    float *running_mean, *running_var;
    float momentum, eps;
    float *scale, *shift, *mean_out, *invstd_out;
    __device__ void operator()(int c, const double* v) const {
        const double mean = v[0] / count;
        double var = v[1] / count - mean * mean;
        if (var < 0.0) var = 0.0;
        const float invstd = (float)(1.0 / sqrt(var + (double)eps));
        const float sc = gamma[c] * invstd;
        scale[c] = sc;
        shift[c] = beta[c] - (float)mean * sc;
        mean_out[c] = (float)mean;
        invstd_out[c] = invstd;
        if (running_mean) {
            const double unbiased = count > 1.0 ? var * count / (count - 1.0) : var;
            running_mean[c] = (1.f - momentum) * running_mean[c] + momentum * (float)mean;
            running_var[c] = (1.f - momentum) * running_var[c] + momentum * (float)unbiased;
// ... 582 lines not shown
    __syncthreads();
#pragma unroll
    for (int k = 0; k < 2; ++k) {
        const int row = r0 + 32 * k;
        uint16_t e[8];
#pragma unroll
        for (int t = 0; t < 8; ++t) e[t] = tile[ch * 8 + t][row];
        const uint4 v = make_uint4((uint32_t)e[0] | ((uint32_t)e[1] << 16), (uint32_t)e[2] | ((uint32_t)e[3] << 16),
                                   (uint32_t)e[4] | ((uint32_t)e[5] << 16), (uint32_t)e[6] | ((uint32_t)e[7] << 16));
        *reinterpret_cast<uint4*>(jb.wt + ((size_t)(tci * 64 + row) * T + tap) * Co + tco * 64 + ch * 8) = v;
    }
}
__global__ __launch_bounds__(256) void weight_transpose_batched_kernel(TransposeBatch batch) {
    __shared__ uint16_t tile[32][33];
    int ji = 0;
    while (ji + 1 < batch.n && (int)blockIdx.x >= batch.job[ji + 1].first_block) ++ji;
    const TransposeJob jb = batch.job[ji];
    const int Co = jb.Co, T = jb.T, Ci = jb.Ci;
    const int tiles_ci = (Ci + 31) / 32, tiles_co = (Co + 31) / 32;
    const int b = blockIdx.x - jb.first_block;
    const int tci = b % tiles_ci, tco = (b / tiles_ci) % tiles_co, tap = b / (tiles_ci * tiles_co);
    const int x = threadIdx.x & 31, y0 = threadIdx.x >> 5;
    for (int y = y0; y < 32; y += 8) {
        const int co = tco * 32 + y, ci = tci * 32 + x;
        tile[y][x] = (co < Co && ci < Ci) ? jb.w[((size_t)co * T + tap) * Ci + ci] : (uint16_t)0;
    }
    __syncthreads();
    for (int y = y0; y < 32; y += 8) {
        const int ci = tci * 32 + y, co = tco * 32 + x;
        if (ci < Ci && co < Co) jb.wt[((size_t)ci * T + tap) * Co + co] = tile[x][y];
    }
}

static inline int grid_for(size_t work_items, int cap = 16384) {
    size_t b = (work_items + 255) / 256;
    if (b > (size_t)cap) b = cap;
    if (b < 1) b = 1;
    return (int)b;
}

int launch_bn_finalize(hipStream_t st, const float* partial, int tiles, int C, double count, const float* gamma, const float* beta,
                       float* rm, float* rv, float momentum, float eps, float* scale, float* shift, float* mean, float* invstd,
                       double* scratch) {
    return launch_reduce_finish<2>(st, partial, tiles, C, scratch, FinBnFwd{count, gamma, beta, rm, rv, momentum, eps, scale, shift, mean, invstd});
}
int launch_bn_eval_coeffs_batched(hipStream_t st, const BnEvalJob* jobs, int n, float eps) {
    for (int first = 0; first < n; first += BnEvalJobs::MAX) {
        BnEvalJobs chunk;
        const int m = n - first < BnEvalJobs::MAX ? n - first : BnEvalJobs::MAX;
        int cmax = 1;
        for (int i = 0; i < m; ++i) { chunk.job[i] = jobs[first + i]; cmax = chunk.job[i].C > cmax ? chunk.job[i].C : cmax; }
        hipLaunchKernelGGL(bn_eval_coeffs_batched_kernel, dim3((cmax + 255) / 256, m), dim3(256), 0, st, chunk, eps);
        DALI_LAUNCH_CHECK();
    }
    return DALI_OK;
}
int launch_fold_cat_weights(hipStream_t st, const float* w3, const float* wd, const float* s3, const float* sd, const float* h3, const float* hd, int C, int w,
                            int cin, int parts, uint16_t* wcat, float* shcat) {
    const size_t n = (size_t)C * parts * (w + cin);
    hipLaunchKernelGGL(fold_cat_weights_kernel, dim3(grid_for(n, 1024)), dim3(256), 0, st, w3, wd, s3, sd, h3, hd, C, w, cin, parts, wcat, shcat);
    DALI_LAUNCH_CHECK();
    return DALI_OK;
}
int launch_bn_act(hipStream_t st, const uint16_t* raw, const float* scale, const float* shift, const uint16_t* idn, const uint16_t* raw2,
                  const float* scale2, const float* shift2, int relu, size_t elems, int C, uint16_t* y, uint8_t* mask_out) {
    const size_t chunks = elems / 8;
    hipLaunchKernelGGL(bn_act_kernel, dim3(grid_for(chunks)), dim3(256), 0, st, raw, scale, shift, idn, raw2, scale2, shift2, relu, chunks, C, y, mask_out);
    DALI_LAUNCH_CHECK();
    return DALI_OK;
}
int bn_bwd_blocks(int P, int C, int* rows_per_block) {
    const int rif = 256 / (C / 8);
    int blocks = (P + rif * 8 - 1) / (rif * 8);
    if (blocks > 1024) blocks = 1024;
    if (blocks < 1) blocks = 1;
    int rpb = (P + blocks - 1) / blocks;
    rpb = (rpb + rif - 1) / rif * rif;
    blocks = (P + rpb - 1) / rpb;
    *rows_per_block = rpb;
    return blocks;
}
int launch_bn_bwd(hipStream_t st, const uint16_t* g, const uint16_t* ymask, const uint8_t* ybits, const BnBwdSide& a, const BnBwdSide* b, int relu, int P, int C,
                  float* partial, float* coef_a, float* coef_b, float* dgamma_a, float* dbeta_a, float* dgamma_b, float* dbeta_b,
                  uint16_t* draw_a, uint16_t* draw_b, uint16_t* dz_out, double* scratch) {
    int rpb;
    const int blocks = bn_bwd_blocks(P, C, &rpb);
    const int rif = 256 / (C / 8);
    const bool dual = b != nullptr;
    const int NV = dual ? 3 : 2;
    const size_t lds = (size_t)rif * C * NV * sizeof(float);
    BnBwdSide bb = dual ? *b : a;
    if (dual) {
        hipLaunchKernelGGL(bn_bwd_reduce_kernel<true>, dim3(blocks), dim3(256), lds, st, g, ymask, ybits, a, bb, relu, P, C, rpb, partial);
    } else {
        hipLaunchKernelGGL(bn_bwd_reduce_kernel<false>, dim3(blocks), dim3(256), lds, st, g, ymask, ybits, a, bb, relu, P, C, rpb, partial);
    }
    DALI_LAUNCH_CHECK();
    int rc;
    if (dual) {
        FinBnBwd<3> fin{(double)P, C, {{a.scale, a.mean, a.invstd, coef_a, dgamma_a, dbeta_a}, {bb.scale, bb.mean, bb.invstd, coef_b, dgamma_b, dbeta_b}}};
        rc = launch_reduce_finish<3>(st, partial, blocks, C, scratch, fin);
    } else {
        FinBnBwd<2> fin{(double)P, C, {{a.scale, a.mean, a.invstd, coef_a, dgamma_a, dbeta_a}}};
        rc = launch_reduce_finish<2>(st, partial, blocks, C, scratch, fin);
    }
    if (rc) return rc;
    const size_t chunks = (size_t)P * C / 8;
    if (dual) hipLaunchKernelGGL(bn_bwd_apply_kernel<true>, dim3(grid_for(chunks)), dim3(256), 0, st, g, ymask, ybits, a, bb, coef_a, coef_b, relu, chunks, C, draw_a, draw_b, dz_out);
    else hipLaunchKernelGGL(bn_bwd_apply_kernel<false>, dim3(grid_for(chunks)), dim3(256), 0, st, g, ymask, ybits, a, bb, coef_a, coef_a, relu, chunks, C, draw_a, draw_b, dz_out);
    DALI_LAUNCH_CHECK();
    return DALI_OK;
}
size_t bn_bwd_partial_floats(int P, int C, bool dual) {
    int rpb;
    return (size_t)bn_bwd_blocks(P, C, &rpb) * C * (dual ? 3 : 2);
}
GatherGeom stem_geom(int H, int W) {
    GatherGeom g{};
    g.Hout = (H - 1) / 2 + 1; g.Wout = (W - 1) / 2 + 1;
    g.Hin = H + 6; g.Win = W + 8;
    g.Ck = 32; g.R = 7; g.S = 1; g.stride = 2; g.pad = 0; g.mode = 0;
    g.pix_pitch = 4; g.row_pitch = (W + 8) * 4; g.img_pitch = (long long)(H + 6) * (W + 8) * 4;
    g.lw = g.lhw = -1;
    return g;
}
int launch_stem_pack_image(hipStream_t st, const float* img, int N, int H, int W, uint16_t* out) {
    const int Hp = H + 6, Wp = W + 8;
    hipLaunchKernelGGL(stem_pack_image_kernel, dim3(grid_for((size_t)N * Hp * Wp)), dim3(256), 0, st, img, N, H, W, Hp, Wp, out);
    DALI_LAUNCH_CHECK();
    return DALI_OK;
}
int launch_stem_pack_weight(hipStream_t st, const float* w, int Cout, uint16_t* out) {
    hipLaunchKernelGGL(stem_pack_weight_kernel, dim3((Cout * 224 + 255) / 256), dim3(256), 0, st, w, Cout, out);
    DALI_LAUNCH_CHECK();
    return DALI_OK;
}
int launch_stem_unpack_wgrad(hipStream_t st, const float* padded, int Cout, float* dw) {
    hipLaunchKernelGGL(stem_unpack_wgrad_kernel, dim3((Cout * 147 + 255) / 256), dim3(256), 0, st, padded, Cout, dw);
    DALI_LAUNCH_CHECK();
    return DALI_OK;
}
int launch_maxpool_bn_fwd(hipStream_t st, const uint16_t* raw, const float* scale, const float* shift, int N, int H, int W, int C,
                          uint16_t* out, uint8_t* arg) {
    const int Ho = (H + 2 - 3) / 2 + 1, Wo = (W + 2 - 3) / 2 + 1;
    hipLaunchKernelGGL(maxpool_bn_fwd_kernel, dim3(grid_for((size_t)N * Ho * Wo * (C / 8))), dim3(256), 0, st, raw, scale, shift, N, H, W, C,
                       Ho, Wo, out, arg);
    DALI_LAUNCH_CHECK();
    return DALI_OK;
}
int maxpool_bn_bwd_blocks(int N, int H, int W, int C, int* quads_per_block) {
    return bn_bwd_blocks(N * ((H + 2 - 3) / 2 + 1) * ((W + 2 - 3) / 2 + 1), C, quads_per_block);
}
int launch_maxpool_bn_bwd(hipStream_t st, const uint16_t* dp, const uint8_t* arg, const uint16_t* raw, const float* mean, const float* invstd,
                          const float* scale, int N, int H, int W, int C, float* partial, float* coef, float* dgamma, float* dbeta,
                          uint16_t* draw, double* scratch) {
    const int Ho = (H + 2 - 3) / 2 + 1, Wo = (W + 2 - 3) / 2 + 1;
    const int P = N * H * W;
    if ((long long)P * (C / 8) >= (1ll << 32)) { set_error("maxpool_bn_bwd: more than 2^32 16-byte chunks"); return DALI_ERR_LIMIT; }
    int qpb;
    const int blocks = maxpool_bn_bwd_blocks(N, H, W, C, &qpb);
    const bool even = (H & 1) == 0 && (W & 1) == 0;
    const size_t lds = (size_t)(256 / (C / 8)) * C * 2 * sizeof(float);
    auto reduce = even ? maxpool_bn_bwd_reduce_kernel<true> : maxpool_bn_bwd_reduce_kernel<false>;
    hipLaunchKernelGGL(reduce, dim3(blocks), dim3(256), lds, st, dp, arg, raw, mean, invstd, N, H, W, C, Ho, Wo, qpb, partial);
    DALI_LAUNCH_CHECK();
    FinBnBwd<2> fin{(double)P, C, {{scale, mean, invstd, coef, dgamma, dbeta}}};
    if (int rc = launch_reduce_finish<2>(st, partial, blocks, C, scratch, fin)) return rc;
    auto apply = even ? maxpool_bn_bwd_apply_kernel<true> : maxpool_bn_bwd_apply_kernel<false>;
    hipLaunchKernelGGL(apply, dim3(grid_for((size_t)N * Ho * Wo * (C / 8))), dim3(256), 0, st, dp, arg, raw, coef, N, H, W, C, Ho, Wo, draw);
    DALI_LAUNCH_CHECK();
    return DALI_OK;
}
int launch_head_pool_fwd(hipStream_t st, const uint16_t* x, int N, int HW, int C, int mode, float* f, int16_t* arg) {
    hipLaunchKernelGGL(head_pool_fwd_kernel, dim3((N * (C / 8) * 8 + 255) / 256), dim3(256), 0, st, x, N, HW, C, mode, f, arg);
    DALI_LAUNCH_CHECK();
// ... 18 lines not shown
    return DALI_OK;
}
int launch_cast_bf16(hipStream_t st, const float* x, size_t n, uint16_t* y) {
    hipLaunchKernelGGL(cast_f32_bf16_kernel, dim3(grid_for((n + 3) / 4, 4096)), dim3(256), 0, st, x, n, y);
    DALI_LAUNCH_CHECK();
    return DALI_OK;
}
int launch_weight_transpose_batched(hipStream_t st, const TransposeJob* jobs, int n) {
    bool all64 = true;
    for (int i = 0; i < n; ++i)
        all64 = all64 && jobs[i].Ci % 64 == 0 && jobs[i].Co % 64 == 0 && ((reinterpret_cast<uintptr_t>(jobs[i].w) | reinterpret_cast<uintptr_t>(jobs[i].wt)) & 15) == 0;
    const int tile = all64 ? 64 : 32;
    for (int begin = 0; begin < n; begin += TRANSPOSE_BATCH) {
        TransposeBatch batch{};
        batch.n = n - begin < TRANSPOSE_BATCH ? n - begin : TRANSPOSE_BATCH;
        int blocks = 0;
        for (int i = 0; i < batch.n; ++i) {
            batch.job[i] = jobs[begin + i];
            batch.job[i].first_block = blocks;
            blocks += ((batch.job[i].Ci + tile - 1) / tile) * ((batch.job[i].Co + tile - 1) / tile) * batch.job[i].T;
        }
        if (all64) hipLaunchKernelGGL(weight_transpose64_batched_kernel, dim3(blocks), dim3(256), 0, st, batch);
        else hipLaunchKernelGGL(weight_transpose_batched_kernel, dim3(blocks), dim3(256), 0, st, batch);
        DALI_LAUNCH_CHECK();
    }
    return DALI_OK;
}
int launch_weight_transpose(hipStream_t st, const uint16_t* w, int Co, int T, int Ci, uint16_t* wt) {
    const TransposeJob job{w, wt, Co, T, Ci, 0};
    return launch_weight_transpose_batched(st, &job, 1);
}

}

using namespace dali;

extern "C" int dali_bn_finalize(dali_ctx* ctx, void* stream, const float* partial, int tiles, int C, double count,
                                const float* gamma, const float* beta, float* running_mean, float* running_var,
                                float momentum, float eps, float* scale, float* shift, float* mean, float* invstd) {
    DALI_REQUIRE(ctx && partial && gamma && beta && scale && shift && mean && invstd, "dali_bn_finalize: null argument");
    DALI_REQUIRE(tiles > 0 && C > 0 && count > 0, "dali_bn_finalize: bad sizes");
    double* scratch = static_cast<double*>(workspace(ctx, reduce_scratch_bytes(C, 2)));
    if (!scratch) return DALI_ERR_NOMEM;
    return launch_bn_finalize((hipStream_t)stream, partial, tiles, C, count, gamma, beta, running_mean, running_var, momentum, eps, scale,
                              shift, mean, invstd, scratch);
}

extern "C" int dali_bn_act(dali_ctx* ctx, void* stream, const uint16_t* raw, const float* scale, const float* shift,
                           const uint16_t* identity, const uint16_t* raw2, const float* scale2, const float* shift2, int relu,
                           int64_t pixels, int C, uint16_t* y, uint8_t* mask_out) {
    DALI_REQUIRE(ctx && raw && scale && shift && y, "dali_bn_act: null argument");
    DALI_REQUIRE(C % 8 == 0 && pixels >= 0, "dali_bn_act: C must be a multiple of 8");
    DALI_REQUIRE(!(identity && raw2), "dali_bn_act: identity and raw2 are exclusive");
    DALI_REQUIRE(!raw2 || (scale2 && shift2), "dali_bn_act: raw2 needs scale2/shift2");
    if (pixels == 0) return DALI_OK;
    return launch_bn_act((hipStream_t)stream, raw, scale, shift, identity, raw2, scale2, shift2, relu, (size_t)pixels * C, C, y, mask_out);
}

extern "C" int dali_bn_bwd(dali_ctx* ctx, void* stream, const uint16_t* g, const uint16_t* ymask, const uint8_t* ybits, int relu, int64_t pixels, int C,
                           const uint16_t* raw_a, const float* mean_a, const float* invstd_a, const float* scale_a, const float* shift_a,
                           const uint16_t* raw_b, const float* mean_b, const float* invstd_b, const float* scale_b,
                           float* dgamma_a, float* dbeta_a, float* dgamma_b, float* dbeta_b, uint16_t* draw_a, uint16_t* draw_b,
                           uint16_t* dz_out) {
    DALI_REQUIRE(ctx && g && raw_a && mean_a && invstd_a && scale_a && dgamma_a && dbeta_a && draw_a, "dali_bn_bwd: null argument");
    DALI_REQUIRE(C % 8 == 0 && C <= 2048 && pixels > 0 && pixels < (1ll << 31), "dali_bn_bwd: C must be a multiple of 8, <= 2048");
    DALI_REQUIRE(ymask || ybits || !relu || shift_a, "dali_bn_bwd: relu mask needs ymask, ybits or scale/shift");
    DALI_REQUIRE(!(ymask && ybits), "dali_bn_bwd: ymask and ybits are exclusive");
    const bool dual = raw_b != nullptr;
    DALI_REQUIRE(!dual || (mean_b && invstd_b && scale_b && dgamma_b && dbeta_b && draw_b), "dali_bn_bwd: incomplete second side");
    const size_t pf = bn_bwd_partial_floats((int)pixels, C, dual);
    const size_t need = align_up(pf * 4, 256) + 2 * align_up((size_t)C * 12, 256) + reduce_scratch_bytes(C, 3);
    char* ws = static_cast<char*>(workspace(ctx, need));
    if (!ws) return DALI_ERR_NOMEM;
    float* partial = reinterpret_cast<float*>(ws);
    float* coef_a = reinterpret_cast<float*>(ws + align_up(pf * 4, 256));
    float* coef_b = reinterpret_cast<float*>(ws + align_up(pf * 4, 256) + align_up((size_t)C * 12, 256));
    double* scratch = reinterpret_cast<double*>(ws + align_up(pf * 4, 256) + 2 * align_up((size_t)C * 12, 256));
    BnBwdSide a{raw_a, mean_a, invstd_a, scale_a, shift_a};
    BnBwdSide b{raw_b, mean_b, invstd_b, scale_b, nullptr};
    return launch_bn_bwd((hipStream_t)stream, g, ymask, ybits, a, dual ? &b : nullptr, relu, (int)pixels, C, partial, coef_a, coef_b, dgamma_a, dbeta_a,
                         dgamma_b, dbeta_b, draw_a, draw_b, dz_out, scratch);
}

extern "C" int dali_maxpool_bn_fwd(dali_ctx* ctx, void* stream, const uint16_t* raw, const float* scale, const float* shift, int n, int h,
                                   int w, int C, uint16_t* out, uint8_t* arg) {
    DALI_REQUIRE(ctx && raw && scale && shift && out && arg, "dali_maxpool_bn_fwd: null argument");
    DALI_REQUIRE(C % 8 == 0 && n > 0 && h > 0 && w > 0, "dali_maxpool_bn_fwd: bad shape");
    return launch_maxpool_bn_fwd((hipStream_t)stream, raw, scale, shift, n, h, w, C, out, arg);
}

extern "C" int dali_maxpool_bn_bwd(dali_ctx* ctx, void* stream, const uint16_t* dpool, const uint8_t* arg, const uint16_t* raw,
                                   const float* mean, const float* invstd, const float* scale, int n, int h, int w, int C,
                                   float* dgamma, float* dbeta, uint16_t* draw) {
    DALI_REQUIRE(ctx && dpool && arg && raw && mean && invstd && scale && dgamma && dbeta && draw, "dali_maxpool_bn_bwd: null argument");
    DALI_REQUIRE(C % 8 == 0 && C <= 2048, "dali_maxpool_bn_bwd: C must be a multiple of 8, <= 2048");
    int qpb;
    const size_t pf = (size_t)maxpool_bn_bwd_blocks(n, h, w, C, &qpb) * C * 2;
    const size_t need = align_up(pf * 4, 256) + align_up((size_t)C * 12, 256) + reduce_scratch_bytes(C, 2);
    char* ws = static_cast<char*>(workspace(ctx, need));
    if (!ws) return DALI_ERR_NOMEM;
    return launch_maxpool_bn_bwd((hipStream_t)stream, dpool, arg, raw, mean, invstd, scale, n, h, w, C, reinterpret_cast<float*>(ws),
                                 reinterpret_cast<float*>(ws + align_up(pf * 4, 256)), dgamma, dbeta, draw,
                                 reinterpret_cast<double*>(ws + align_up(pf * 4, 256) + align_up((size_t)C * 12, 256)));
}

extern "C" int dali_head_pool_fwd(dali_ctx* ctx, void* stream, const uint16_t* x, int n, int hw, int C, int mode, float* f, int16_t* arg) {
    DALI_REQUIRE(ctx && x && f && arg, "dali_head_pool_fwd: null argument");
    DALI_REQUIRE(mode >= DALI_FEATURE_BOTH && mode <= DALI_FEATURE_GMP, "dali_head_pool_fwd: bad feature mode %d", mode);
    DALI_REQUIRE(C % 8 == 0 && hw > 0 && hw < 32768, "dali_head_pool_fwd: bad shape");
    return launch_head_pool_fwd((hipStream_t)stream, x, n, hw, C, mode, f, arg);
}
extern "C" int dali_head_pool_bwd(dali_ctx* ctx, void* stream, const float* df, const int16_t* arg, int n, int hw, int C, int mode, uint16_t* dx) {
    DALI_REQUIRE(ctx && df && arg && dx, "dali_head_pool_bwd: null argument");
    DALI_REQUIRE(mode >= DALI_FEATURE_BOTH && mode <= DALI_FEATURE_GMP, "dali_head_pool_bwd: bad feature mode %d", mode);
    DALI_REQUIRE(C % 8 == 0 && hw > 0, "dali_head_pool_bwd: bad shape");
    return launch_head_pool_bwd((hipStream_t)stream, df, arg, n, hw, C, mode, dx);
}
extern "C" int dali_debug_head_pool_bwd_masked(dali_ctx* ctx, void* stream, const float* df, const int16_t* arg, int n, int hw, int C, int mode,
                                               const uint8_t* ybits, uint16_t* dx) {
    DALI_REQUIRE(ctx && df && arg && ybits && dx, "dali_debug_head_pool_bwd_masked: null argument");
    DALI_REQUIRE(mode >= DALI_FEATURE_BOTH && mode <= DALI_FEATURE_GMP, "dali_debug_head_pool_bwd_masked: bad feature mode %d", mode);
    DALI_REQUIRE(C % 8 == 0 && hw > 0 && n > 0, "dali_debug_head_pool_bwd_masked: bad shape");
    return launch_head_pool_bwd((hipStream_t)stream, df, arg, n, hw, C, mode, dx, ybits);
}
extern "C" int dali_debug_stem_wgrad(dali_ctx* ctx, void* stream, const float* images, const uint16_t* d_raw0, int N, int H, int W, int Cout, float* dw) {
    DALI_REQUIRE(ctx && images && d_raw0 && dw, "dali_debug_stem_wgrad: null argument");
    DALI_REQUIRE(N > 0 && H >= 32 && W >= 32 && H % 32 == 0 && W % 16 == 0 && (Cout == 32 || Cout == 64),
                 "dali_debug_stem_wgrad: bad shape %dx%dx%d, Cout %d (height %% 32, width %% 16, Cout 32 or 64)", N, H, W, Cout);
    DALI_REQUIRE((long long)N * (H / 2) * (W / 2) < (1ll << 31), "dali_debug_stem_wgrad: more than 2^31 pixels");
    hipStream_t st = (hipStream_t)stream;
    WGradArgs a{};
    a.Cm = Cout; a.P = N * (H / 2) * (W / 2);
    a.g = stem_geom(H, W);
    const size_t b_img = align_up((size_t)N * (H + 6) * (W + 8) * 4 * 2, 256), b_slab = align_up(wgrad_need(a.Cm, a.P, a.g, false).slab_bytes, 256);
    const size_t b_pad = align_up((size_t)Cout * 224 * 4, 256);
    char* ws = static_cast<char*>(workspace(ctx, b_img + b_slab + b_pad));
    if (!ws) return DALI_ERR_NOMEM;
    uint16_t* ximg = reinterpret_cast<uint16_t*>(ws);
    float* dw_pad = reinterpret_cast<float*>(ws + b_img + b_slab);
    a.dY = d_raw0; a.X = ximg;
    int rc;
    if ((rc = launch_stem_pack_image(st, images, N, H, W, ximg))) return rc;
    if ((rc = launch_wgrad(st, a, WGradBufs{reinterpret_cast<float*>(ws + b_img), nullptr, nullptr}, dw_pad, 0))) return rc;
    return launch_stem_unpack_wgrad(st, dw_pad, Cout, dw);
}
extern "C" int dali_bn1d_fwd(dali_ctx* ctx, void* stream, const float* x, int n, int C, const float* gamma, const float* beta,
                             float* running_mean, float* running_var, int training, float momentum, float eps, float* y, float* mean,
                             float* invstd) {
    DALI_REQUIRE(ctx && x && gamma && beta && y, "dali_bn1d_fwd: null argument");
    DALI_REQUIRE(training || (running_mean && running_var), "dali_bn1d_fwd: eval mode needs running statistics");
    return launch_bn1d_fwd((hipStream_t)stream, x, n, C, gamma, beta, running_mean, running_var, training, momentum, eps, y, mean, invstd);
}
extern "C" int dali_bn1d_bwd(dali_ctx* ctx, void* stream, const float* x, const float* dy, int n, int C, const float* gamma,
                             const float* mean, const float* invstd, float* dx, float* dgamma, float* dbeta) {
    DALI_REQUIRE(ctx && x && dy && gamma && mean && invstd && dx && dgamma && dbeta, "dali_bn1d_bwd: null argument");
    return launch_bn1d_bwd((hipStream_t)stream, x, dy, n, C, gamma, mean, invstd, dx, dgamma, dbeta);
}
```

### daliid_amd/csrc/resnet_plan.hip

```cpp
#include "kernels.h"
#include "plan_table.h"
#include <cstring>
#include <new>

using namespace dali;

namespace {

struct Conv {
    int cin, cout, r, s, stride, pad, hin, win, hout, wout;
    int64_t w_off;
    uint16_t* w_bf16;
    uint16_t* wt_bf16;
};
struct Bn {
    int C;
    int64_t g_off, b_off;
    int64_t rm_off, rv_off;
    float *scale, *shift, *mean, *invstd, *coef;
};
struct LinBn {
    int w = 0, C = 0;
    bool stats = false;
    float *gram = nullptr, *m2 = nullptr, *bvec = nullptr, *qk = nullptr;
// ... 221 lines not shown
extern "C" int dali_resnet_sizes(const dali_resnet* net, int64_t* param_elems, int64_t* buffer_elems, int64_t* arena_bytes,
                                 int* feat_dim, int* n_params, int* n_buffers) {
    DALI_REQUIRE(net, "dali_resnet_sizes: null net");
    return net->sizes(net->feat_dim, param_elems, buffer_elems, arena_bytes, feat_dim, n_params, n_buffers);
}

extern "C" int dali_resnet_tensor_info(const dali_resnet* net, int kind, int index, char* name, int name_cap, int64_t* offset,
                                       int64_t* numel, int* shape4, int* ndim) {
    DALI_REQUIRE(net, "dali_resnet_tensor_info: null argument");
    return net->tensor_info("dali_resnet_tensor_info", kind, index, name, name_cap, offset, numel, shape4, ndim);
}

extern "C" int dali_resnet_stage_param_range(const dali_resnet* net, int stage, int64_t* begin, int64_t* end) {
    DALI_REQUIRE(net && begin && end && stage >= 0 && stage < 4, "dali_resnet_stage_param_range: bad argument");
    const int li = 3 - stage;
    const Block& first = net->blocks[net->stage_first[li]];
    *begin = (li == 0) ? 0 : first.c1.w_off;
    if (li == 3) *end = net->param_elems;
    else *end = net->blocks[net->stage_first[li + 1]].c1.w_off;
    return DALI_OK;
}

extern "C" int dali_resnet_bind(dali_resnet* net, float* params, float* grads, float* buffers, void* arena, size_t arena_bytes) {
    DALI_REQUIRE(net && params && buffers && arena, "dali_resnet_bind: null argument");
    DALI_REQUIRE(arena_bytes >= net->arena_bytes, "dali_resnet_bind: arena too small (%zu < %zu)", arena_bytes, net->arena_bytes);
    DALI_REQUIRE((reinterpret_cast<uintptr_t>(arena) & 255) == 0 && (reinterpret_cast<uintptr_t>(params) & 255) == 0 &&
                 (reinterpret_cast<uintptr_t>(grads) & 255) == 0 && (reinterpret_cast<uintptr_t>(buffers) & 255) == 0,
                 "dali_resnet_bind: storages must be 256-byte aligned");
    net->P = params; net->G = grads; net->B = buffers; net->arena = static_cast<char*>(arena);
    net->bind_arena(net->arena);
    for (auto& b : net->blocks) for_each_conv(b, [&](Conv& c) { c.w_bf16 = net->wbf16_flat + c.w_off; });
    return DALI_OK;
}

extern "C" int dali_resnet_refresh_weights(dali_resnet* net, void* stream) {
    DALI_REQUIRE(net && net->P, "dali_resnet_refresh_weights: net not bound");
    hipStream_t st = (hipStream_t)stream;
    int rc = launch_cast_bf16(st, net->P, (size_t)net->param_elems, net->wbf16_flat);
    if (rc) return rc;
    rc = launch_stem_pack_weight(st, net->P + net->stem.w_off, net->stem.cout, net->w_stem);
    if (rc) return rc;
    std::vector<TransposeJob> jobs;
    for (auto& b : net->blocks) for_each_conv(b, [&](Conv& c) { jobs.push_back(TransposeJob{c.w_bf16, c.wt_bf16, c.cout, c.r * c.s, c.cin, 0}); });
    return launch_weight_transpose_batched(st, jobs.data(), (int)jobs.size());
}

namespace {

int bn_train(dali_resnet* net, hipStream_t st, Bn& b, int tiles, double count) {
    const BnParams p = bn_params(net, b);
    return launch_bn_finalize(st, net->stat_partial, tiles, b.C, count, p.gamma, p.beta, p.rm, p.rv, 0.1f, 1e-5f, b.scale, b.shift, b.mean, b.invstd,
                              net->red_scratch);
}

int conv_bn_fwd(dali_resnet* net, hipStream_t st, const Conv& c, Bn& out_bn, const uint16_t* x, uint16_t* raw) {
    IGemmArgs a{};
    a.W = c.w_bf16; a.X = x; a.O = raw;
    a.stats = net->fwd_training ? net->stat_partial : nullptr;
    a.Cm = c.cout; a.P = net->N * c.hout * c.wout;
    a.g = conv_geom(c, 0);
    int rc = launch_igemm_conv(st, a);
    if (rc) return rc;
    if (net->fwd_training) return bn_train(net, st, out_bn, igemm_conv_stat_tiles(a.Cm, a.P, a.g.R * a.g.S * a.g.Ck), (double)a.P);
    return DALI_OK;
}
int bn_relu(hipStream_t st, const Bn& bn, const uint16_t* raw, size_t elems, uint16_t* act) {
    return launch_bn_act(st, raw, bn.scale, bn.shift, nullptr, nullptr, nullptr, nullptr, 1, elems, bn.C, act, nullptr);
}

int conv_bn_relu_eval(dali_resnet* net, hipStream_t st, const Conv& c, const Bn& bn, const uint16_t* x, uint16_t* act) {
    IGemmArgs a{};
    a.W = c.w_bf16; a.X = x; a.O = act;
    a.out_scale = bn.scale; a.out_shift = bn.shift; a.out_relu = 1;
    a.Cm = c.cout; a.P = net->N * c.hout * c.wout;
    a.g = conv_geom(c, 0);
    return launch_igemm_conv(st, a);
}

int conv_wgrad(dali_resnet* net, hipStream_t st, const Conv& c, const uint16_t* x, const uint16_t* dy) {
    return run_wgrad(net, st, conv_wgrad_desc(net, c), dy, x, net->G + c.w_off);
}

int conv_dgrad(dali_resnet* net, hipStream_t st, const Conv& c, const uint16_t* dy, const uint16_t* residual, uint16_t* dx,
               const uint8_t* out_mask = nullptr) {
    IGemmArgs a{};
    a.W = c.wt_bf16; a.X = dy; a.O = dx; a.Res = residual; a.out_mask = out_mask;
    a.Cm = c.cin; a.P = net->N * c.hin * c.win;
    a.g = conv_geom(c, 1);
    return launch_igemm_conv(st, a);
}

int cat_gemm(dali_resnet* net, hipStream_t st, const Conv& c, int mode, const uint16_t* W, const uint16_t* X, int c1, const uint16_t* X2, int c2, int Cm,
             uint16_t* O, IGemmArgs stage = IGemmArgs{}) {
    IGemmArgs& a = stage;
    a.W = W; a.X = X; a.X2 = X2; a.Ck1 = c1; a.O = O;
    a.Cm = Cm; a.P = net->N * (mode == 0 ? c.hout * c.wout : c.hin * c.win);
    Conv cat = c;
    (mode == 0 ? cat.cin : cat.cout) = (a.x_rep ? a.x_rep : 1) * (c1 + c2);
    a.g = conv_geom(cat, mode);
    return launch_igemm_conv(st, a);
}

int linbn_fwd(dali_resnet* net, hipStream_t st, LinBn& l, const Conv& c, Bn& bn, const uint16_t* x) {
    const WGradDesc d = gram_desc(net, c);
    int rc;
    if ((rc = run_wgrad(net, st, d, x, x, l.gram, l.m2))) return rc;
    if (!l.stats) return launch_bnlin_ut(st, c.w_bf16, l.gram, l.C, l.w, l.ut);
    const BnParams p = bn_params(net, bn);
    return launch_bnlin_stats(st, c.w_bf16, c.wt_bf16, l.gram, l.m2, l.C, l.w, (double)d.P, p.gamma, p.beta, p.rm, p.rv, 0.1f, 1e-5f, l.ut, l.dot, bn.scale,
                              bn.shift, bn.mean, bn.invstd);
}
int linbn_bwd(dali_resnet* net, hipStream_t st, LinBn& l, const Conv& c, const Bn& bn, const uint16_t* dz, const uint16_t* x, float* s_dz, bool sum_dz) {
    const WGradDesc d = conv_wgrad_desc(net, c);
    int rc;
    if ((rc = run_wgrad(net, st, d, dz, x, net->G + c.w_off, sum_dz ? s_dz : nullptr))) return rc;
    const int ld = l.C + l.w;
    return launch_bnlin_bwd(st, c.w_bf16, c.wt_bf16, l.ut, l.m2, s_dz, l.C, l.w, (double)d.P, bn.scale, bn.mean, bn.invstd, net->G + c.w_off, net->G + bn.g_off,
                            net->G + bn.b_off, l.wd, l.wd + l.C, l.bvec, l.qk, ld, ld);
}

int bn_bwd(dali_resnet* net, hipStream_t st, const Bn& bn, const uint16_t* raw, const uint16_t* g, int relu, int P, uint16_t* out) {
    const BnBwdSide s{raw, bn.mean, bn.invstd, bn.scale, bn.shift};
    return launch_bn_bwd(st, g, nullptr, nullptr, s, nullptr, relu, P, bn.C, net->bwd_partial, bn.coef, nullptr, net->G + bn.g_off, net->G + bn.b_off,
                         nullptr, nullptr, out, nullptr, nullptr, net->red_scratch);
}

uint16_t* next_gbuf(dali_resnet* net, const uint16_t* avoid0, const uint16_t* avoid1 = nullptr, const uint16_t* avoid2 = nullptr,
                    const uint16_t* avoid3 = nullptr) {
    for (int i = 0; i < 6; ++i) {
        uint16_t* g = net->gbuf[i];
        if (g != avoid0 && g != avoid1 && g != avoid2 && g != avoid3) return g;
    }
    return nullptr;
}

int stem_forward(dali_resnet* net, hipStream_t st, const float* images, bool tr) {
    const Conv& c = net->stem;
    Bn& bn = net->stem_bn;
    int rc;
    if ((rc = launch_stem_pack_image(st, images, net->N, net->H, net->W, net->ximg))) return rc;
    if (!tr && stem_fused_supported(net->N, net->H, net->W, c.cout))
        return launch_stem_conv_bn_pool(st, net->ximg, net->w_stem, bn.scale, bn.shift, net->N, net->H, net->W, net->pool0);
    if (tr && stem_train_supported(net->N, net->H, net->W, c.cout)) {
        if ((rc = launch_stem_conv_stats(st, net->ximg, net->w_stem, net->N, net->H, net->W, net->raw0, net->stat_partial))) return rc;
        if ((rc = bn_train(net, st, bn, stem_train_tiles(net->N, net->H), (double)net->N * net->stem_h * net->stem_w))) return rc;
    } else {
        IGemmArgs a{};
        a.W = net->w_stem; a.X = net->ximg; a.O = net->raw0;
        a.stats = tr ? net->stat_partial : nullptr;
        a.Cm = c.cout; a.P = net->N * net->stem_h * net->stem_w;
        a.g = stem_geom(net->H, net->W);
        if ((rc = launch_igemm_conv(st, a))) return rc;
        if (tr && (rc = bn_train(net, st, bn, igemm_conv_stat_tiles(a.Cm, a.P, 224), (double)a.P))) return rc;
    }
    return launch_maxpool_bn_fwd(st, net->raw0, bn.scale, bn.shift, net->N, net->stem_h, net->stem_w, c.cout, net->pool0, net->pool_arg);
}

int block_forward(dali_resnet* net, hipStream_t st, Block& b, const uint16_t* x, bool tr) {
    int rc;
    b.x = const_cast<uint16_t*>(x);
    if (!tr) {
        if ((rc = conv_bn_relu_eval(net, st, b.c1, b.b1, x, b.a1))) return rc;
        if ((rc = conv_bn_relu_eval(net, st, b.c2, b.b2, b.a1, b.a2))) return rc;
    } else {
        if ((rc = conv_bn_fwd(net, st, b.c1, b.b1, x, b.raw1))) return rc;
        if ((rc = bn_relu(st, b.b1, b.raw1, (size_t)net->N * b.hin * b.win * b.width, b.a1))) return rc;
        if ((rc = conv_bn_fwd(net, st, b.c2, b.b2, b.a1, b.raw2))) return rc;
        if ((rc = bn_relu(st, b.b2, b.raw2, (size_t)net->N * b.hout * b.wout * b.width, b.a2))) return rc;
        if ((rc = linbn_fwd(net, st, b.l3, b.c3, b.b3, b.a2))) return rc;
    }
    if (!tr && b.cat_eval) {
        if ((rc = launch_fold_cat_weights(st, net->P + b.c3.w_off, net->P + b.cd.w_off, b.b3.scale, b.bd.scale, b.b3.shift, b.bd.shift, b.cout, b.width,
                                          b.cin, 2, b.wcat, b.shcat))) return rc;
        IGemmArgs stage{};
        stage.x_rep = 2; stage.out_shift = b.shcat; stage.out_relu = 1;
        return cat_gemm(net, st, b.c3, 0, b.wcat, b.a2, b.width, x, b.cin, b.cout, b.y, stage);
    }
    IGemmArgs a{};
    a.W = b.c3.w_bf16; a.X = b.a2; a.O = b.y; a.Res = x; a.out_scale = b.b3.scale; a.out_shift = b.b3.shift; a.out_relu = 1;
    if (b.has_ds) {
        if ((rc = conv_bn_fwd(net, st, b.cd, b.bd, x, b.rawd))) return rc;
        a.Res = b.rawd; a.res_scale = b.bd.scale; a.bias = b.bd.shift;
        if (b.lin_ds && tr && (rc = linbn_fwd(net, st, b.ld, b.cd, b.bd, x))) return rc;
    }
    a.bits_out = tr ? b.ybits : nullptr;
    a.Cm = b.cout; a.P = net->N * b.hout * b.wout; a.g = conv_geom(b.c3, 0);
    return launch_igemm_conv(st, a);
}

}

extern "C" int dali_resnet_set_feature(dali_resnet* net, int mode) {
    DALI_REQUIRE(net, "dali_resnet_set_feature: null net");
    DALI_REQUIRE(mode >= DALI_FEATURE_BOTH && mode <= DALI_FEATURE_GMP, "dali_resnet_set_feature: bad feature mode %d", mode);
    net->feature_mode = mode;
    return DALI_OK;
}

extern "C" int dali_resnet_forward(dali_resnet* net, void* stream, const float* images, int training, float* emb) {
    DALI_REQUIRE(net && net->P && images && emb, "dali_resnet_forward: null argument or net not bound");
    hipStream_t st = (hipStream_t)stream;
    const bool tr = training != 0;
    net->fwd_training = tr;
    int rc;
    if (!tr) {
        std::vector<BnEvalJob> jobs;
        auto add = [&](Bn& b) { const BnParams p = bn_params(net, b); jobs.push_back(BnEvalJob{p.gamma, p.beta, p.rm, p.rv, b.scale, b.shift, b.C}); };
        add(net->stem_bn);
        for (auto& b : net->blocks) for_each_bn(b, add);
        if ((rc = launch_bn_eval_coeffs_batched(st, jobs.data(), (int)jobs.size(), 1e-5f))) return rc;
    }
    if ((rc = stem_forward(net, st, images, tr))) return rc;
    const uint16_t* x = net->pool0;
    for (auto& b : net->blocks) {
        if ((rc = block_forward(net, st, b, x, tr))) return rc;
        x = b.y;
    }
    if ((rc = launch_head_pool_fwd(st, x, net->N, net->head_hw, net->feat_dim, net->feature_mode, net->feat, net->head_arg))) return rc;
    const BnParams p = bn_params(net, net->neck);
    return launch_bn1d_fwd(st, net->feat, net->N, net->feat_dim, p.gamma, p.beta, p.rm, p.rv, tr ? 1 : 0, 0.1f, 1e-5f, emb, net->neck_mean, net->neck_invstd);
}

static int block_backward(dali_resnet* net, hipStream_t st, Block& b, const uint8_t* prev_bits) {
    int rc;
    uint16_t* dz = net->cur_dy;
    const int Pout = net->N * b.hout * b.wout, Pin = net->N * b.hin * b.win;
    uint16_t* d_rawd = nullptr;
    if ((rc = linbn_bwd(net, st, b.l3, b.c3, b.b3, dz, b.a2, b.sdz, true))) return rc;
    uint16_t* d_a2 = next_gbuf(net, dz);
    uint16_t* scratch_a = next_gbuf(net, dz, d_a2);
    {
        IGemmArgs stage{};
        stage.bias = b.l3.bvec;
        if ((rc = cat_gemm(net, st, b.c3, 1, b.l3.wd, dz, b.cout, b.a2, b.width, b.width, d_a2, stage))) return rc;
    }
    if (b.lin_ds) {
        if ((rc = linbn_bwd(net, st, b.ld, b.cd, b.bd, dz, b.x, b.sdz, false))) return rc;
    } else if (b.has_ds) {
        d_rawd = next_gbuf(net, dz, d_a2, scratch_a);
        if ((rc = bn_bwd(net, st, b.bd, b.rawd, dz, 0, Pout, d_rawd))) return rc;
    }
    if ((rc = bn_bwd(net, st, b.b2, b.raw2, d_a2, 1, Pout, d_a2))) return rc;
    if ((rc = conv_wgrad(net, st, b.c2, b.a1, d_a2))) return rc;
    uint16_t* d_a1 = scratch_a;
    if ((rc = conv_dgrad(net, st, b.c2, d_a2, nullptr, d_a1))) return rc;
    if ((rc = bn_bwd(net, st, b.b1, b.raw1, d_a1, 1, Pin, d_a1))) return rc;
    b.dbg_d_raw1 = d_a1;
    if ((rc = conv_wgrad(net, st, b.c1, b.x, d_a1))) return rc;
    uint16_t* dx = d_a2;
    if (b.lin_ds) {
        if ((rc = conv_dgrad(net, st, b.c1, d_a1, nullptr, dx, prev_bits))) return rc;
        IGemmArgs stage{};
        stage.Res = dx; stage.bias = b.ld.bvec;
        if ((rc = cat_gemm(net, st, b.cd, 1, b.ld.wd, dz, b.cout, b.x, b.cin, b.cin, dx, stage))) return rc;
    } else if (b.has_ds) {
        if ((rc = conv_wgrad(net, st, b.cd, b.x, d_rawd))) return rc;
        if ((rc = conv_dgrad(net, st, b.c1, d_a1, nullptr, dx, prev_bits))) return rc;
        if ((rc = conv_dgrad(net, st, b.cd, d_rawd, dx, dx, prev_bits))) return rc;
    } else {
        if ((rc = conv_dgrad(net, st, b.c1, d_a1, dz, dx, prev_bits))) return rc;
    }
    net->cur_dy = dx;
    net->cur_dy_bytes = (int64_t)Pin * b.cin * 2;
    return DALI_OK;
}

static int head_backward(dali_resnet* net, hipStream_t st, const float* d_emb) {
    int rc;
    if ((rc = launch_bn1d_bwd(st, net->feat, d_emb, net->N, net->feat_dim, net->P + net->neck.g_off, net->neck_mean, net->neck_invstd,
                              net->dfeat, net->G + net->neck.g_off, net->G + net->neck.b_off))) return rc;
    net->cur_dy = net->gbuf[0];
    if ((rc = launch_head_pool_bwd(st, net->dfeat, net->head_arg, net->N, net->head_hw, net->feat_dim, net->feature_mode, net->cur_dy,
                                   net->blocks.back().ybits))) return rc;
    net->cur_dy_bytes = (int64_t)net->N * net->head_hw * net->feat_dim * 2;
    return DALI_OK;
}

static int stem_backward(dali_resnet* net, hipStream_t st) {
    int rc;
    uint16_t* d_raw0 = next_gbuf(net, net->cur_dy);
    if ((rc = launch_maxpool_bn_bwd(st, net->cur_dy, net->pool_arg, net->raw0, net->stem_bn.mean, net->stem_bn.invstd, net->stem_bn.scale,
                                    net->N, net->stem_h, net->stem_w, net->stem.cout, net->bwd_partial, net->stem_bn.coef,
                                    net->G + net->stem_bn.g_off, net->G + net->stem_bn.b_off, d_raw0, net->red_scratch))) return rc;
    net->dbg_d_raw0 = d_raw0;
    if ((rc = run_wgrad(net, st, stem_wgrad_desc(net), d_raw0, net->ximg, net->stem_dw_pad))) return rc;
    return launch_stem_unpack_wgrad(st, net->stem_dw_pad, net->stem.cout, net->G + net->stem.w_off);
}

extern "C" int dali_resnet_backward(dali_resnet* net, void* stream, const float* d_emb, int stage_begin, int stage_end) {
    DALI_REQUIRE(net && net->P && net->G, "dali_resnet_backward: net not bound (grads required)");
    DALI_REQUIRE(net->fwd_training, "dali_resnet_backward: the last forward was not in training mode");
    DALI_REQUIRE(stage_begin >= 0 && stage_end <= 3 && stage_begin <= stage_end, "dali_resnet_backward: bad stage range %d..%d", stage_begin, stage_end);
    hipStream_t st = (hipStream_t)stream;
    int rc;
    for (int stage = stage_begin; stage <= stage_end; ++stage) {
        const int li = 3 - stage;
        if (stage == 0) {
            DALI_REQUIRE(d_emb != nullptr, "dali_resnet_backward: d_emb is null");
            if ((rc = head_backward(net, st, d_emb))) return rc;
        }
        for (int bi = net->stage_last[li]; bi >= net->stage_first[li]; --bi)
            if ((rc = block_backward(net, st, net->blocks[bi], bi > 0 ? net->blocks[bi - 1].ybits : nullptr))) return rc;
        if (stage == 3 && (rc = stem_backward(net, st))) return rc;
    }
    return DALI_OK;
}

extern "C" int dali_debug_resnet_backward_block(dali_resnet* net, void* stream, const float* d_emb, int block) {
    DALI_REQUIRE(net && net->P && net->G, "dali_debug_resnet_backward_block: net not bound (grads required)");
    DALI_REQUIRE(net->fwd_training, "dali_debug_resnet_backward_block: the last forward was not in training mode");
    const int nb = (int)net->blocks.size();
    if (block == -1) return stem_backward(net, (hipStream_t)stream);
    DALI_REQUIRE(block >= 0 && block < nb, "dali_debug_resnet_backward_block: block %d out of range", block);
    hipStream_t st = (hipStream_t)stream;
    int rc;
    if (block == nb - 1) {
        DALI_REQUIRE(d_emb != nullptr, "dali_debug_resnet_backward_block: d_emb is null");
        if ((rc = head_backward(net, st, d_emb))) return rc;
    }
    return block_backward(net, st, net->blocks[block], block > 0 ? net->blocks[block - 1].ybits : nullptr);
}

extern "C" int dali_resnet_debug_tensor(dali_resnet* net, const char* name, void** ptr, int64_t* bytes) {
    DALI_REQUIRE(net && name && ptr && bytes && net->arena, "dali_resnet_debug_tensor: bad argument / net not bound");
    const std::string n(name);
    const size_t N = net->N;
    auto bn_field = [&](Bn& b, const std::string& f) -> bool {
        float* p = f == "scale" ? b.scale : f == "shift" ? b.shift : f == "mean" ? b.mean : f == "invstd" ? b.invstd : nullptr;
        if (!p) return false;
// ... 43 lines not shown
```

### daliid_amd/ops_nn.py

```python
import torch

from . import _lib

bf16 = torch.bfloat16


def _out_hw(h, w, r, s, stride, pad):
    return (h + 2 * pad - r) // stride + 1, (w + 2 * pad - s) // stride + 1


def conv2d_fwd(x, w, stride=1, pad=0, in_scale=None, in_shift=None, in_relu=False, want_stats=False):
    n, h, wd, cin = x.shape
    cout, r, s, _ = w.shape
    ho, wo = _out_hw(h, wd, r, s, stride, pad)
    y = torch.empty(n, ho, wo, cout, device=x.device, dtype=bf16)
    stats = None
    if want_stats:
        tiles = _lib.lib().dali_conv2d_stat_tiles(cout, cin, r, s, stride, pad, n, ho, wo, int(in_scale is not None))
        stats = torch.empty(tiles, cout, 2, device=x.device, dtype=torch.float32)
    _lib.check(_lib.lib().dali_conv2d_fwd(_lib.ctx(x.device), _lib.stream_ptr(), _lib.ptr(x, bf16, "x"), _lib.ptr(w, bf16, "w"),
                                           _lib.ptr(y), n, h, wd, cin, cout, r, s, stride, pad,
                                           _lib.ptr(in_scale), _lib.ptr(in_shift), int(in_relu), _lib.ptr(stats)),
               "dali_conv2d_fwd")
    return (y, stats) if want_stats else y


def conv2d_bn_act(x, w, scale, shift, stride=1, pad=0, relu=True):
    n, h, wd, cin = x.shape
    cout, r, s, _ = w.shape
    ho, wo = _out_hw(h, wd, r, s, stride, pad)
    y = torch.empty(n, ho, wo, cout, device=x.device, dtype=bf16)
    _lib.check(_lib.lib().dali_conv2d_bn_act(_lib.ctx(x.device), _lib.stream_ptr(), _lib.ptr(x, bf16, "x"), _lib.ptr(w, bf16, "w"), _lib.ptr(y),
                                              n, h, wd, cin, cout, r, s, stride, pad, _lib.ptr(scale, torch.float32, "scale"),
                                              _lib.ptr(shift, torch.float32, "shift"), int(relu)), "dali_conv2d_bn_act")
    return y


def stem_conv_bn_maxpool(images, weight, scale, shift):
    n, c, h, w = images.shape
    if c != 3 or tuple(weight.shape) != (64, 7, 7, 3):
        raise _lib.DaliError("stem_conv_bn_maxpool: images [N,3,H,W] and weight [64,7,7,3] expected, got %s / %s" % (tuple(images.shape), tuple(weight.shape)))
    y = torch.empty(n, h // 4, w // 4, 64, device=images.device, dtype=bf16)
    _lib.check(_lib.lib().dali_stem_conv_bn_maxpool(_lib.ctx(images.device), _lib.stream_ptr(), _lib.ptr(images, torch.float32, "images"), n, h, w,
                                                     _lib.ptr(weight, torch.float32, "weight"), _lib.ptr(scale, torch.float32, "scale"),
                                                     _lib.ptr(shift, torch.float32, "shift"), _lib.ptr(y)), "dali_stem_conv_bn_maxpool")
    return y


def conv2d_dgrad(dy, wt, x_hw, stride=1, pad=0, residual=None, inplace=False, residual_mask=None):
    n, ho, wo, cout = dy.shape
    cin, r, s, _ = wt.shape
    h, wd = x_hw
    assert _out_hw(h, wd, r, s, stride, pad) == (ho, wo)
    if inplace:
        assert residual is not None and tuple(residual.shape) == (n, h, wd, cin) and residual.is_contiguous()
    dx = residual if inplace else torch.empty(n, h, wd, cin, device=dy.device, dtype=bf16)
    _lib.check(_lib.lib().dali_conv2d_dgrad(_lib.ctx(dy.device), _lib.stream_ptr(), _lib.ptr(dy, bf16, "dy"), _lib.ptr(wt, bf16, "wt"),
                                             _lib.ptr(dx), _lib.ptr(residual), _lib.ptr(residual_mask, torch.uint8, "residual_mask"),
                                             n, h, wd, cin, cout, r, s, stride, pad),
               "dali_conv2d_dgrad")
    return dx


def conv2d_wgrad(x, dy, rs, stride=1, pad=0, in_scale=None, in_shift=None, in_relu=False, out=None, accumulate=False):
    n, h, wd, cin = x.shape
    cout = dy.shape[3]
    r, s = rs
    if out is None:
        out = torch.empty(cout, r, s, cin, device=x.device, dtype=torch.float32)
    _lib.check(_lib.lib().dali_conv2d_wgrad(_lib.ctx(x.device), _lib.stream_ptr(), _lib.ptr(x, bf16, "x"), _lib.ptr(dy, bf16, "dy"),
                                             _lib.ptr(out, torch.float32, "dw"), n, h, wd, cin, cout, r, s, stride, pad,
                                             _lib.ptr(in_scale), _lib.ptr(in_shift), int(in_relu), int(accumulate)),
               "dali_conv2d_wgrad")
    return out


def conv1x1_fused(x, w, out_scale=None, out_shift=None, bias=None, residual=None, relu=False, want_bits=False, out_mask=None, inplace=False,
                  res_scale=None):
    P, cin = x.shape
    cout = w.shape[0]
    y = residual if inplace else torch.empty(P, cout, device=x.device, dtype=bf16)
    bits = torch.empty(P * cout // 8, device=x.device, dtype=torch.uint8) if want_bits else None
    _lib.check(_lib.lib().dali_conv1x1_fused(_lib.ctx(x.device), _lib.stream_ptr(), _lib.ptr(x, bf16, "x"), _lib.ptr(w, bf16, "w"), _lib.ptr(y),
                                              P, cin, cout, _lib.ptr(out_scale), _lib.ptr(out_shift), _lib.ptr(bias), _lib.ptr(residual), int(relu),
                                              _lib.ptr(bits), _lib.ptr(out_mask, torch.uint8, "out_mask"), _lib.ptr(res_scale)), "dali_conv1x1_fused")
    return (y, bits) if want_bits else y


def conv1x1_cat(x1, x2, w, bias=None):
    P, c1 = x1.shape
    c2 = x2.shape[1]
    cout = w.shape[0]
    assert x2.shape[0] == P and w.shape[1] == c1 + c2
    y = torch.empty(P, cout, device=x1.device, dtype=bf16)
    _lib.check(_lib.lib().dali_conv1x1_cat(_lib.ctx(x1.device), _lib.stream_ptr(), _lib.ptr(x1, bf16, "x1"), c1, _lib.ptr(x2, bf16, "x2"), c2,
                                            _lib.ptr(w, bf16, "w"), _lib.ptr(bias), _lib.ptr(y), P, cout), "dali_conv1x1_cat")
    return y


def conv1x1_cat_act(x1, x2, w, out_shift, out_scale=None, relu=True, parts=1):
    P, c1 = x1.shape
    c2 = x2.shape[1]
    cout = w.shape[0]
    assert x2.shape[0] == P and w.shape[1] == parts * (c1 + c2)
    y = torch.empty(P, cout, device=x1.device, dtype=bf16)
    _lib.check(_lib.lib().dali_conv1x1_cat_act(_lib.ctx(x1.device), _lib.stream_ptr(), _lib.ptr(x1, bf16, "x1"), c1, _lib.ptr(x2, bf16, "x2"), c2,
                                                _lib.ptr(w, bf16, "w"), int(parts), _lib.ptr(out_scale), _lib.ptr(out_shift, torch.float32, "out_shift"), int(relu),
                                                _lib.ptr(y), P, cout), "dali_conv1x1_cat_act")
    return y


def bnlin_fwd(a, w, gamma, beta, running_mean=None, running_var=None, momentum=0.1, eps=1e-5):
    P, wd = a.shape
    C = w.shape[0]
    dev = a.device
    o = dict(gram=torch.empty(wd, wd, device=dev), m2=_f32(wd, dev), ut=torch.empty(wd, C, device=dev), scale=_f32(C, dev), shift=_f32(C, dev),
             mean=_f32(C, dev), invstd=_f32(C, dev))
    _lib.check(_lib.lib().dali_bnlin_fwd(_lib.ctx(dev), _lib.stream_ptr(), _lib.ptr(a, bf16, "a"), _lib.ptr(w, bf16, "w"), P, C, wd, _lib.ptr(gamma),
                                          _lib.ptr(beta), _lib.ptr(running_mean), _lib.ptr(running_var), momentum, eps, _lib.ptr(o["gram"]),
                                          _lib.ptr(o["m2"]), _lib.ptr(o["ut"]), _lib.ptr(o["scale"]), _lib.ptr(o["shift"]), _lib.ptr(o["mean"]), _lib.ptr(o["invstd"])),
               "dali_bnlin_fwd")
    return o


def bnlin_bwd(dz, a, w, fwd):
    P, wd = a.shape
    C = w.shape[0]
    dev = a.device
    o = dict(dW=torch.empty(C, wd, device=dev), dgamma=_f32(C, dev), dbeta=_f32(C, dev), wd1=torch.empty(wd, C, device=dev, dtype=bf16),
             wd2=torch.empty(wd, wd, device=dev, dtype=bf16), bvec=_f32(wd, dev))
    _lib.check(_lib.lib().dali_bnlin_bwd(_lib.ctx(dev), _lib.stream_ptr(), _lib.ptr(dz, bf16, "dz"), _lib.ptr(a, bf16, "a"), _lib.ptr(w, bf16, "w"), P, C, wd,
                                          _lib.ptr(fwd["ut"]), _lib.ptr(fwd["m2"]), _lib.ptr(fwd["scale"]), _lib.ptr(fwd["mean"]), _lib.ptr(fwd["invstd"]),
                                          _lib.ptr(o["dW"]), _lib.ptr(o["dgamma"]), _lib.ptr(o["dbeta"]), _lib.ptr(o["wd1"]), _lib.ptr(o["wd2"]),
                                          _lib.ptr(o["bvec"])), "dali_bnlin_bwd")
    return o


def _f32(n, dev):
    return torch.empty(n, device=dev, dtype=torch.float32)


def bn_finalize(partial, count, gamma, beta, running_mean=None, running_var=None, momentum=0.1, eps=1e-5):
    tiles, C, _ = partial.shape
    dev = partial.device
# ... 99 lines not shown
```

### include/daliid.h

```cpp
#ifndef DALIID_H
#define DALIID_H

#include <stddef.h>
#include <stdint.h>

#ifdef __cplusplus
extern "C" {
#endif

typedef enum {
    DALI_OK = 0,
    DALI_ERR_INVALID = -1,
    DALI_ERR_HIP = -2,
    DALI_ERR_NOMEM = -3,
    DALI_ERR_LIMIT = -4,
    DALI_ERR_UNSUPPORTED = -5
} dali_status;

typedef struct dali_ctx dali_ctx;

int dali_version(void);
const char* dali_last_error(void);
int dali_ctx_create(int device, dali_ctx** out);
int dali_ctx_destroy(dali_ctx* ctx);
// ... 3 lines not shown
               DALI_METRIC_L2SQ = 1,
               DALI_METRIC_DOT = 2
} dali_metric;
typedef enum { DALI_PREC_BF16X3 = 0,
               DALI_PREC_BF16 = 1
} dali_precision;
typedef enum { DALI_FEATURE_BOTH = 0, DALI_FEATURE_GAP = 1, DALI_FEATURE_GMP = 2 } dali_feature;

int dali_l2norm_rows(dali_ctx* ctx, void* stream, const float* x, int n, int d, float eps,
                     float* y, float* norms);
int dali_l2norm_rows_bwd(dali_ctx* ctx, void* stream, const float* x, const float* dy, int n, int d,
                         float eps, float* dx);

int dali_pairdist(dali_ctx* ctx, void* stream, const float* Q, const float* G, int nq, int ng, int d,
                  int metric, int precision, int normalize, float* out);

size_t dali_pairdist_operand_bytes(int n, int d, int precision);
int dali_pairdist_prepare(dali_ctx* ctx, void* stream, const float* X, int n, int d, int normalize, int precision,
                          void* image, float* sq);
int dali_pairdist_prepared(dali_ctx* ctx, void* stream, const void* q_image, const float* q_sq, const void* g_image,
                           const float* g_sq, int nq, int ng, int d, int metric, int precision, float* out);

int dali_pairdist_blend(dali_ctx* ctx, void* stream, const float* Q, const float* G, int nq, int ng, int d,
                        int precision, int normalize, const float* q_mag_prev, const float* g_mag_prev,
                        const float* q_mag, const float* g_mag, float* inout);

int dali_rank_eval(dali_ctx* ctx, void* stream, const float* distmat, const int32_t* q_pids,
                   const int32_t* g_pids, const int32_t* q_camids, const int32_t* g_camids, int nq, int ng,
                   int max_rank, float* cmc, float* mAP, double* map64, int32_t* num_valid,
                   float* ap, int32_t* first_rank, int32_t* status);

int dali_rank_shard_matches(dali_ctx* ctx, void* stream, const float* dist_shard, const int32_t* q_pids, const int32_t* g_pids,
                            const int32_t* q_camids, const int32_t* g_camids, int nq, int ng, int g_offset, int cap,
                            int64_t* keys, int32_t* counts, int32_t* status);
int dali_rank_shard_bins(dali_ctx* ctx, void* stream, const float* dist_shard, const int32_t* q_pids, const int32_t* g_pids,
                         const int32_t* q_camids, const int32_t* g_camids, int nq, int ng, int g_offset, const int64_t* keys_all,
                         const int32_t* counts_all, int world, int cap, int32_t* bins, int bins_cap, int32_t* status);
int dali_rank_shard_finish(dali_ctx* ctx, void* stream, const int32_t* bins, const int32_t* counts_all, int world, int nq, int bins_cap,
                           int max_rank, float* cmc, float* mAP, double* map64, int32_t* num_valid, float* ap, int32_t* first_rank);

int dali_rerank(dali_ctx* ctx, void* stream, const float* q_g, const float* q_q, const float* g_g, int nq, int ng, int k1, int k2,
                double lambda_value, float* out);

size_t dali_roc_scratch_bytes(int nq, int ng);
int dali_roc_build(dali_ctx* ctx, void* stream, const float* distmat, const int32_t* q_ids, const int32_t* g_ids, int nq, int ng,
                   void* scratch, size_t scratch_bytes, int64_t* out);
int dali_roc_emit(dali_ctx* ctx, void* stream, const void* scratch, int nq, int ng, int drop_intermediate, int64_t n_points,
                  float* thresholds, int64_t* fps, int64_t* tps);

int dali_topk_rows(dali_ctx* ctx, void* stream, const float* x, int nq, int ncols, int64_t ld, int col_offset, int k, int largest,
                   int accumulate, int64_t* keys);
int dali_topk_decode(dali_ctx* ctx, void* stream, const int64_t* keys, int nq, int k, int largest, float* values, int32_t* indices);
size_t dali_pairdist_topk_scratch_bytes(int nq, int ng, int d, int k, int boot_cols, int chunk_cols, int cand_cap);
int dali_pairdist_topk(dali_ctx* ctx, void* stream, const void* q_image, const float* q_sq, const void* g_image, const float* g_sq,
                       int nq, int ng, int d, int metric, int precision, int k, int largest, int g_offset, int accumulate,
                       int64_t* keys, int boot_cols, int chunk_cols, int cand_cap, int32_t* stats);


int dali_conv2d_fwd(dali_ctx* ctx, void* stream, const uint16_t* x, const uint16_t* w, uint16_t* y,
                    int n, int h, int wd, int cin, int cout, int r, int s, int stride, int pad,
                    const float* in_scale, const float* in_shift, int in_relu, float* stats);
int dali_conv2d_bn_act(dali_ctx* ctx, void* stream, const uint16_t* x, const uint16_t* w, uint16_t* y, int n, int h, int wd, int cin, int cout,
                       int r, int s, int stride, int pad, const float* out_scale, const float* out_shift, int out_relu);
int dali_stem_fused_supported(int n, int h, int w);
int dali_stem_conv_bn_maxpool(dali_ctx* ctx, void* stream, const float* images, int n, int h, int w, const float* weight, const float* scale,
                              const float* shift, uint16_t* y);
int dali_conv1x1_fused(dali_ctx* ctx, void* stream, const uint16_t* x, const uint16_t* w, uint16_t* y, int pixels, int cin, int cout,
                       const float* out_scale, const float* out_shift, const float* bias, const uint16_t* residual, int out_relu,
                       uint8_t* bits_out, const uint8_t* out_mask, const float* res_scale);
int dali_conv1x1_cat(dali_ctx* ctx, void* stream, const uint16_t* x1, int c1, const uint16_t* x2, int c2, const uint16_t* w, const float* bias,
                     uint16_t* y, int pixels, int cout);
int dali_conv1x1_cat_act(dali_ctx* ctx, void* stream, const uint16_t* x1, int c1, const uint16_t* x2, int c2, const uint16_t* w, int weight_parts,
                         const float* out_scale, const float* out_shift, int out_relu, uint16_t* y, int pixels, int cout);
int dali_bnlin_fwd(dali_ctx* ctx, void* stream, const uint16_t* a, const uint16_t* W, int P, int C, int w, const float* gamma,
                   const float* beta, float* running_mean, float* running_var, float momentum, float eps, float* gram, float* m2,
                   float* ut, float* scale, float* shift, float* mean, float* invstd);
int dali_bnlin_bwd(dali_ctx* ctx, void* stream, const uint16_t* dz, const uint16_t* a, const uint16_t* W, int P, int C, int w,
                   const float* ut, const float* m2, const float* scale, const float* mean, const float* invstd, float* dW,
                   float* dgamma, float* dbeta, uint16_t* wd1, uint16_t* wd2, float* bvec);
int dali_conv2d_stat_tiles(int cout, int cin, int r, int s, int stride, int pad, int n, int ho, int wo, int fused_operand);
int dali_conv2d_dgrad(dali_ctx* ctx, void* stream, const uint16_t* dy, const uint16_t* wt, uint16_t* dx,
                      const uint16_t* residual, const uint8_t* residual_mask, int n, int h, int wd, int cin, int cout, int r, int s,
                      int stride, int pad);
int dali_conv2d_wgrad(dali_ctx* ctx, void* stream, const uint16_t* x, const uint16_t* dy, float* dw,
                      int n, int h, int wd, int cin, int cout, int r, int s, int stride, int pad,
                      const float* in_scale, const float* in_shift, int in_relu, int accumulate);

int dali_bn_finalize(dali_ctx* ctx, void* stream, const float* partial, int tiles, int C, double count,
                     const float* gamma, const float* beta, float* running_mean, float* running_var,
                     float momentum, float eps, float* scale, float* shift, float* mean, float* invstd);
int dali_bn_act(dali_ctx* ctx, void* stream, const uint16_t* raw, const float* scale, const float* shift,
                const uint16_t* identity, const uint16_t* raw2, const float* scale2, const float* shift2, int relu,
                int64_t pixels, int C, uint16_t* y, uint8_t* mask_out);
int dali_bn_bwd(dali_ctx* ctx, void* stream, const uint16_t* g, const uint16_t* ymask, const uint8_t* ybits, int relu,
                int64_t pixels, int C,
                const uint16_t* raw_a, const float* mean_a, const float* invstd_a, const float* scale_a, const float* shift_a,
                const uint16_t* raw_b, const float* mean_b, const float* invstd_b, const float* scale_b,
                float* dgamma_a, float* dbeta_a, float* dgamma_b, float* dbeta_b, uint16_t* draw_a, uint16_t* draw_b,
                uint16_t* dz_out);
int dali_maxpool_bn_fwd(dali_ctx* ctx, void* stream, const uint16_t* raw, const float* scale, const float* shift, int n, int h,
                        int w, int C, uint16_t* out, uint8_t* arg);
int dali_maxpool_bn_bwd(dali_ctx* ctx, void* stream, const uint16_t* dpool, const uint8_t* arg, const uint16_t* raw,
                        const float* mean, const float* invstd, const float* scale, int n, int h, int w, int C,
                        float* dgamma, float* dbeta, uint16_t* draw);
int dali_head_pool_fwd(dali_ctx* ctx, void* stream, const uint16_t* x, int n, int hw, int C, int mode, float* f, int16_t* arg);
int dali_head_pool_bwd(dali_ctx* ctx, void* stream, const float* df, const int16_t* arg, int n, int hw, int C, int mode,
                       uint16_t* dx);
int dali_bn1d_fwd(dali_ctx* ctx, void* stream, const float* x, int n, int C, const float* gamma, const float* beta,
                  float* running_mean, float* running_var, int training, float momentum, float eps, float* y, float* mean,
                  float* invstd);
int dali_bn1d_bwd(dali_ctx* ctx, void* stream, const float* x, const float* dy, int n, int C, const float* gamma,
                  const float* mean, const float* invstd, float* dx, float* dgamma, float* dbeta);

int dali_linear_fwd(dali_ctx* ctx, void* stream, const uint16_t* x, const uint16_t* w, const float* bias, int act,
                    const uint16_t* residual, uint16_t* y, uint16_t* pre, int rows, int K, int N);
int dali_linear_fwd_scaled(dali_ctx* ctx, void* stream, const uint16_t* x, const uint16_t* w, const float* bias, int act,
                           const uint16_t* residual, const float* row_scale, uint16_t* y, int rows, int K, int N);
int dali_linear_dgrad(dali_ctx* ctx, void* stream, const uint16_t* dy, const uint16_t* wt, const uint16_t* gelu_pre,
                      const uint16_t* residual, uint16_t* dx, int rows, int K, int N);
int dali_linear_wgrad(dali_ctx* ctx, void* stream, const uint16_t* x, const uint16_t* dy, float* dw, float* dbias, int rows,
                      int K, int N);
int dali_vit_patchify(dali_ctx* ctx, void* stream, const float* img, int B, int H, int W, int patch, int stride, uint16_t* out);
int dali_vit_assemble_tokens(dali_ctx* ctx, void* stream, const uint16_t* patch_emb, const float* cls, const float* pos, int B, int T,
                             int C, uint16_t* x);
int dali_vit_assemble_tokens_bwd(dali_ctx* ctx, void* stream, const uint16_t* dx, int B, int T, int C, float* dpos, float* dcls,
                                 uint16_t* dpatch_emb);
int dali_vit_assemble_tokens_sie(dali_ctx* ctx, void* stream, const uint16_t* patch_emb, const float* cls, const float* pos, const float* sie,
                                 const int32_t* idx, int n_sie, float coef, int B, int T, int C, uint16_t* x);
int dali_vit_sie_grad(dali_ctx* ctx, void* stream, const uint16_t* dx, const int32_t* idx, int B, int T, int C, int n_sie, float coef,
                      float* dsie);
int dali_vit_jpm_gather(dali_ctx* ctx, void* stream, const uint16_t* features, const int32_t* map, int B, int T, int C, int G, int L,
                        uint16_t* out);
int dali_vit_jpm_head(dali_ctx* ctx, void* stream, const float* global_feat, const float* local_feat, const float* gamma, const float* beta,
                      const float* running_mean, const float* running_var, int B, int C, int after, float* out);
int dali_layernorm_fwd(dali_ctx* ctx, void* stream, const uint16_t* x, const float* gamma, const float* beta, int rows, int C,
                       float eps, uint16_t* y, float* mean, float* rstd);
int dali_layernorm_bwd(dali_ctx* ctx, void* stream, const uint16_t* g, const uint16_t* x, const float* gamma, const float* mean,
                       const float* rstd, const uint16_t* add, int rows, int C, uint16_t* dx, float* dgamma, float* dbeta);
int dali_attention_fwd(dali_ctx* ctx, void* stream, const uint16_t* qkv, int B, int T, int H, int head_dim, float scale,
                       uint16_t* out, float* lse);
int dali_attention_bwd(dali_ctx* ctx, void* stream, const uint16_t* qkv, const uint16_t* out, const uint16_t* d_out, const float* lse,
                       int B, int T, int H, int head_dim, float scale, uint16_t* dqkv);
int dali_attention_fwd_short(dali_ctx* ctx, void* stream, const uint16_t* qkv, int B, int T, int H, int head_dim, float scale,
                             uint16_t* out, float* lse);


int dali_center_loss_fwd(dali_ctx* ctx, void* stream, const float* S, const int32_t* labels, const int32_t* center_labels,
                         const float* w, float tau, int nb, int NC, float* rowstat, float* sums);
int dali_center_loss_bwd(dali_ctx* ctx, void* stream, const float* S, const int32_t* labels, const int32_t* center_labels,
                         const float* w, float tau, int nb, int NC, const float* denom, float gscale, float* dS);
int dali_proxy_loss_fwd(dali_ctx* ctx, void* stream, const float* S, const int32_t* labels, const int32_t* proxy_labels,
                        const float* w, float tau, int nb, int NP, float* rowstat, float* sums, int32_t* sel_idx,
                        float* sel_coef, int32_t* status);
int dali_proxy_loss_bwd(dali_ctx* ctx, void* stream, const int32_t* sel_idx, const float* sel_coef, const float* proxies, int nb,
                        int D, const float* denom, float gscale, int accumulate, float* dfn);
int dali_proxy_kmax(void);

int dali_comm_unique_id(void* id128);
int dali_ctx_comm_init(dali_ctx* ctx, const void* id128, int rank, int world);
int dali_ctx_comm_destroy(dali_ctx* ctx);
int dali_allreduce_bucket(dali_ctx* ctx, void* stream, float* buf, int64_t count);

int dali_adam_step(dali_ctx* ctx, void* stream, float* params, const float* grads, float* exp_avg, float* exp_avg_sq,
                   int64_t n, float lr, float beta1, float beta2, float eps, float weight_decay, int step, float grad_scale,
                   float* weights_sqsum);
int dali_ema_update(dali_ctx* ctx, void* stream, float* momentum, const float* online, int64_t n, float beta);

int dali_triplet_loss_fwd(dali_ctx* ctx, void* stream, const float* S, const int32_t* labels, const float* w, float tau, int nb,
                          float* rowstat, float* sums, int32_t* sel_idx, float* sel_coef, int32_t* status);
int dali_triplet_loss_bwd(dali_ctx* ctx, void* stream, const int32_t* sel_idx, const float* sel_coef, int nb, const float* denom,
                          float gscale, float* dS_sym);

int dali_class_targets(dali_ctx* ctx, void* stream, const float* fvs, int n, int d, const int32_t* order,
                       const int32_t* bounds, int n_classes, const int32_t* first_pick, int num_proxies,
                       float* centers, float* proxies, int32_t* proxy_rows, float* max_dist);

int dali_resize_bicubic_u8(dali_ctx* ctx, void* stream, const uint8_t* src, const int64_t* src_off, const int32_t* in_h,
                           const int32_t* in_w, const int32_t* table_of, int n, int max_in_h, const int32_t* bounds_h,
                           const int32_t* coefs_h, int ksize_h, const int32_t* bounds_v, const int32_t* coefs_v, int ksize_v,
                           int out_h, int out_w, uint8_t* out);
int dali_augment_batch(dali_ctx* ctx, void* stream, const uint8_t* images, const int32_t* params, int n, int h, int w,
                       const float* mean3, const float* std3, float* out);
// ... 68 lines not shown
```

Measured before the change: 17750 images/s.

## Fuse BN-backward partial reductions into dgrad conv epilogue

Adds a BNBWD epilogue mode to the implicit-GEMM dgrad kernels. While storing dx, it reloads the BN raw input, recomputes the ReLU mask and accumulates the per-channel sums of g and g*xhat into a partial slab. The following bn_bwd call can then skip its separate reduction kernel, saving a full read pass over the gradient and raw activations for the bottleneck conv2/conv3 BNs. In exchange the epilogue does more work and uses more LDS, only certain channel counts and tilings qualify, and the downsample bn_bwd is moved earlier so that it does not clobber the shared partial buffer.

```diff
diff --git a/daliid_amd/_lib.py b/daliid_amd/_lib.py
--- a/daliid_amd/_lib.py
+++ b/daliid_amd/_lib.py
@@ -50,6 +50,8 @@
     "dali_stem_conv_bn_maxpool": [c_void_p, c_void_p, c_void_p, c_int, c_int, c_int, c_void_p, c_void_p, c_void_p, c_void_p],
     "dali_conv2d_stat_tiles": [c_int] * 10,
     "dali_conv2d_dgrad": [c_void_p, c_void_p, c_void_p, c_void_p, c_void_p, c_void_p, c_void_p] + [c_int] * 9,
+    "dali_conv2d_dgrad_bnstats": [c_void_p, c_void_p, c_void_p, c_void_p, c_int, c_void_p, c_void_p, c_void_p] + [c_int] * 9 + [c_void_p] * 6 + [ctypes.c_int64],
+    "dali_bn_bwd_partials": [c_void_p, c_void_p, c_void_p, ctypes.c_int64, c_int] + [c_void_p] * 6 + [c_int] + [c_void_p] * 4,
     "dali_conv2d_wgrad": [c_void_p, c_void_p, c_void_p, c_void_p, c_void_p] + [c_int] * 9 + [c_void_p, c_void_p, c_int, c_int],
     "dali_conv1x1_fused": [c_void_p] * 5 + [c_int] * 3 + [c_void_p] * 4 + [c_int, c_void_p, c_void_p, c_void_p],
     "dali_conv1x1_cat": [c_void_p, c_void_p, c_void_p, c_int, c_void_p, c_int, c_void_p, c_void_p, c_void_p, c_int, c_int],
diff --git a/daliid_amd/csrc/conv.hip b/daliid_amd/csrc/conv.hip
--- a/daliid_amd/csrc/conv.hip
+++ b/daliid_amd/csrc/conv.hip
@@ -192,8 +192,9 @@
     FUSED = 3,
     PARITY = 4,
     FUSED_LEAN = 5,
+    BNBWD = 6,
 };
-constexpr Epi epi_mode(bool own, Epi asked) { return own ? asked : Epi::GENERAL; }
+constexpr Epi epi_mode(bool own, Epi asked) { return own || asked == Epi::BNBWD ? asked : Epi::GENERAL; }
 constexpr bool epi_fused(Epi m) { return m == Epi::FUSED || m == Epi::FUSED_LEAN; }
 
 __device__ __forceinline__ uint32_t gate_bf16x2(uint32_t w, unsigned bits) {
@@ -403,6 +404,92 @@
         for (int it = 0; it < ITERS; ++it) st.out(a.O, h, it);
         conv_stamp(a, 7 + 2 * h);
         if (h == 0) lds_barrier();
+    }
+}
+template <int TM, int TN, int FM, int FN, int WNW, int NT>
+__device__ __forceinline__ void epi_store_bnbwd(const IGemmArgs& a, f32x4_t (&acc)[FM][FN], int tm, int tn, uint16_t* smem, int wn, int mb) {
+    using Stage = EpiStage<false, TM, TN, FM, FN, WNW, NT>;
+    constexpr int ITERS = Stage::ITERS, RIF = NT / Stage::CPR;
+    static_assert(TN == 256 && FN == 4 && RIF == 32 && ITERS == 4 && Stage::WROWS == 32, "the chains of bn_bwd_reduce_kernel on a 256-pixel tile");
+    static_assert(RIF * TM * 2 * 4 <= 64 * 1024, "the partial sums fit the smallest ring");
+    const Stage st(a, tm, tn, smem, wn, mb);
+    const int rif = a.bnb_rif;
+    const bool by_block = rif == 4;
+    uint2 pk[FM][FN];
+#pragma unroll
+    for (int i = 0; i < FM; ++i) {
+        const float4 b4 = a.bias ? *reinterpret_cast<const float4*>(a.bias + tm * TM + mb + i * 16) : make_float4(0.f, 0.f, 0.f, 0.f);
+#pragma unroll
+        for (int j = 0; j < FN; ++j) {
+            const float v[4] = {acc[i][j][0] + b4.x, acc[i][j][1] + b4.y, acc[i][j][2] + b4.z, acc[i][j][3] + b4.w};
+            pk[i][j] = pack4(v);
+        }
+        __builtin_amdgcn_sched_barrier(0);
+    }
+    const int c0 = tm * TM + st.ch * 8;
+    const int w = st.lp0 >> 3, r = by_block ? (st.lp0 & 3) : (st.lp0 & 7), b = (st.lp0 >> 2) & 1;
+    const int row0 = w * 32 + (by_block ? b * 16 + r : r);
+    const int pix0 = w * 64 + (by_block ? b * 32 + r : r), pix_h = by_block ? 16 : 32;
+    float s1[8] = {0.f, 0.f, 0.f, 0.f, 0.f, 0.f, 0.f, 0.f}, s2[8] = {0.f, 0.f, 0.f, 0.f, 0.f, 0.f, 0.f, 0.f};
+#pragma unroll
+    for (int h = 0; h < 2; ++h) {
+        const size_t o0 = ((size_t)(tn * TN + pix0 + h * pix_h) * a.Cm + c0) * 2, ostep = (size_t)rif * a.Cm * 2;
+        uint4 rq[ITERS];
+#pragma unroll
+        for (int it = 0; it < ITERS; ++it) rq[it] = *reinterpret_cast<const uint4*>(reinterpret_cast<const char*>(a.bnb.raw) + o0 + it * ostep);
+#pragma unroll
+        for (int jj = 0; jj < Stage::HFN; ++jj) {
+#pragma unroll
+            for (int i = 0; i < FM; ++i) {
+                const uint2 lean = pk[i][h * Stage::HFN + jj], alt = pk[i][2 * jj + h];
+                *st.slot(jj, i) = by_block ? alt : lean;
+            }
+        }
+        lds_barrier();
+        const char* my_rows = st.stage + row0 * Stage::ROWB + st.ch * 16;
+        const int rstep = rif * Stage::ROWB;
+#pragma unroll
+        for (int it = 0; it < ITERS; ++it)
+            *reinterpret_cast<uint4*>(reinterpret_cast<char*>(a.O) + o0 + it * ostep) = *reinterpret_cast<const uint4*>(my_rows + it * rstep);
+        asm volatile("" ::: "memory");
+#pragma unroll
+        for (int k = 0; k < 2; ++k) {
+            __builtin_amdgcn_sched_barrier(0);
+            const float4 mean = *reinterpret_cast<const float4*>(a.bnb.mean + c0 + 4 * k), istd = *reinterpret_cast<const float4*>(a.bnb.invstd + c0 + 4 * k);
+            const float4 sc = *reinterpret_cast<const float4*>(a.bnb.scale + c0 + 4 * k), sh = *reinterpret_cast<const float4*>(a.bnb.shift + c0 + 4 * k);
+            const float m4[4] = {mean.x, mean.y, mean.z, mean.w}, i4[4] = {istd.x, istd.y, istd.z, istd.w};
+            const float c4[4] = {sc.x, sc.y, sc.z, sc.w}, h4[4] = {sh.x, sh.y, sh.z, sh.w};
+#pragma unroll
+            for (int it = 0; it < ITERS; ++it) {
+                const uint2 q = *reinterpret_cast<const uint2*>(my_rows + it * rstep + 8 * k);
+                float gv[4], rv[4];
+                unpack4(q, gv);
+                unpack4(k ? make_uint2(rq[it].z, rq[it].w) : make_uint2(rq[it].x, rq[it].y), rv);
+#pragma unroll
+                for (int t = 0; t < 4; ++t) {
+                    const float g = (rv[t] * c4[t] + h4[t]) > 0.f ? gv[t] : 0.f;
+                    s1[4 * k + t] += g;
+                    s2[4 * k + t] += g * ((rv[t] - m4[t]) * i4[t]);
+                }
+#pragma unroll
+                for (int t = 0; t < 4; ++t) asm volatile("" : "+v"(s1[4 * k + t]), "+v"(s2[4 * k + t]));
+            }
+            asm volatile("" ::: "memory");
+        }
+        __builtin_amdgcn_sched_barrier(0);
+        lds_barrier();
+    }
+    float* red = reinterpret_cast<float*>(smem);
+    float* mine = red + ((size_t)st.lp0 * TM + st.ch * 8) * 2;
+#pragma unroll
+    for (int t = 0; t < 8; t += 2) *reinterpret_cast<float4*>(mine + t * 2) = make_float4(s1[t], s2[t], s1[t + 1], s2[t + 1]);
+    lds_barrier();
+    const int nblk = RIF / rif;
+    for (int e = threadIdx.x; e < nblk * TM; e += NT) {
+        const int bi = e / TM, t = e - bi * TM;
+        float x1 = 0.f, x2 = 0.f;
+        for (int q = 0; q < rif; ++q) { const float2 v = *reinterpret_cast<const float2*>(red + ((size_t)(bi * rif + q) * TM + t) * 2); x1 += v.x; x2 += v.y; }
+        *reinterpret_cast<float2*>(a.bnb_slab + ((size_t)(tn * nblk + bi) * a.Cm + tm * TM + t) * 2) = make_float2(x1, x2);
     }
 }
 template <int TM, int TN, int FM, int FN, int WNW, int NT>
@@ -630,6 +717,10 @@
     constexpr bool FUSED = epi_fused(MODE), SUB = MODE == Epi::PARITY;
     const int lane = threadIdx.x & 63;
     const int mb = wm * (FM * 16) + (lane >> 4) * 4, nb = wn * (FN * 16) + (lane & 15);
+    if constexpr (MODE == Epi::BNBWD) {
+        static_assert(EVEN, "Epi::BNBWD stores by half tiles");
+        return epi_store_bnbwd<TM, TN, FM, FN, WNW, NT>(a, acc, tm, tn, smem, wn, mb);
+    }
     if (a.stats) epi_stats<TM, TN, FM, FN, WNW, NT>(a, acc, tm, tn, smem, wn, mb);
     conv_stamp(a, 5);
     const bool interior = (tm + 1) * TM <= a.Cm && (tn + 1) * TN <= a.P;
@@ -2051,12 +2142,16 @@
     K64S_LIN{kfn(&igemm_conv_k64s_kernel<2, 4, 8, 3, 4, 4, Epi::LIN>), 1024, ring_lds(128, 256, 64, 3), 128, 256, GRID_XCD},
     K64S_LEAN{kfn(&igemm_conv_k64s_kernel<2, 4, 8, 3, 4, 4, Epi::FUSED_LEAN>), 1024, ring_lds(128, 256, 64, 3), 128, 256, GRID_XCD},
     K64S_SRC2{kfn(&igemm_conv_k64s_kernel<2, 4, 8, 3, 4, 4, Epi::CONV, true>), 1024, ring_lds(128, 256, 64, 3), 128, 256, GRID_XCD},
+    K64S_BNB{kfn(&igemm_conv_k64s_kernel<2, 4, 8, 3, 4, 4, Epi::BNBWD>), 1024, ring_lds(128, 256, 64, 3), 128, 256, GRID_XCD},
+    K64S_SRC2_BNB{kfn(&igemm_conv_k64s_kernel<2, 4, 8, 3, 4, 4, Epi::BNBWD, true>), 1024, ring_lds(128, 256, 64, 3), 128, 256, GRID_XCD},
     K64{kfn(&igemm_conv_k64_kernel<4, 4, 2>), 1024, ring_lds(256, 256, 64, 2), 256, 256, GRID_XCD},
     K64_LIN{kfn(&igemm_conv_k64_kernel<4, 4, 2, 4, 4, Epi::LIN>), 1024, ring_lds(256, 256, 64, 2), 256, 256, GRID_XCD},
     K64_FUSED{kfn(&igemm_conv_k64_kernel<4, 4, 2, 4, 4, Epi::FUSED>), 1024, ring_lds(256, 256, 64, 2), 256, 256, GRID_XCD},
     K64_CLS{kfn(&igemm_conv_k64_kernel<4, 4, 2, 4, 4, Epi::PARITY>), 1024, ring_lds(256, 256, 64, 2), 256, 256, GRID_CLASSES},
     K64_SRC2{kfn(&igemm_conv_k64_kernel<4, 4, 2, 4, 4, Epi::CONV, true>), 1024, ring_lds(256, 256, 64, 2), 256, 256, GRID_XCD},
     K64_FUSED_SRC2{kfn(&igemm_conv_k64_kernel<4, 4, 2, 4, 4, Epi::FUSED, true>), 1024, ring_lds(256, 256, 64, 2), 256, 256, GRID_XCD},
+    K64_BNB{kfn(&igemm_conv_k64_kernel<4, 4, 2, 4, 4, Epi::BNBWD>), 1024, ring_lds(256, 256, 64, 2), 256, 256, GRID_XCD},
+    K64_SRC2_BNB{kfn(&igemm_conv_k64_kernel<4, 4, 2, 4, 4, Epi::BNBWD, true>), 1024, ring_lds(256, 256, 64, 2), 256, 256, GRID_XCD},
     K64_320{kfn(&igemm_conv_k64_kernel<4, 4, 2, 4, 5, Epi::LIN>), 1024, ring_lds(256, 320, 64, 2), 256, 320, GRID_XCD};
 
 template <int RB, bool RES, bool OM, bool BITS, bool SRC2 = false>
@@ -2232,11 +2327,31 @@
     return use(in_bn ? CONV128_BN : !dma_ok ? CONV128 : a.X2 ? DMA128_SRC2 : lin ? DMA128_LIN : DMA128);
 }
 
-static int launch_igemm_conv_one(hipStream_t st, const IGemmArgs& a) {
+static int conv_bnbwd_rif(int C, int P) {
+    if (C != 256 && C != 512) return 0;
+    int rpb = 0;
+    const int rif = 256 / (C / 8), blocks = bn_bwd_blocks(P, C, &rpb);
+    return rpb == 8 * rif && (long long)blocks * rpb == P ? rif : 0;
+}
+static const GemmKernel* conv_bnbwd_twin(const IGemmArgs& a, const GemmChoice& c) {
+    static const struct { const GemmKernel *plain, *twin; } twins[] = {{&K64S_SRC2, &K64S_SRC2_BNB}, {&K64_SRC2, &K64_SRC2_BNB}, {&K64S, &K64S_BNB}, {&K64, &K64_BNB}};
+    if (!a.bnb_slab || !c.k || a.g.sub || a.Res || a.res_mask || a.stats || a.in_scale || (a.Cm & 7) || a.Cm % c.k->tm || a.P % c.k->tn) return nullptr;
+    if (!a.bnb.raw || !a.bnb.mean || !a.bnb.invstd || !a.bnb.scale || !a.bnb.shift || conv_bnbwd_rif(a.Cm, a.P) == 0) return nullptr;
+    for (const auto& t : twins)
+        if (c.k == t.plain) return t.twin;
+    return nullptr;
+}
+
+static int launch_igemm_conv_one(hipStream_t st, const IGemmArgs& a, int* bnb_rows = nullptr) {
     IGemmArgs args = a;
     args.g.lw = ilog2_exact(a.g.Wout);
     args.g.lhw = ilog2_exact(a.g.Hout * a.g.Wout);
-    const GemmChoice c = conv_choose(args, f1_cu_count());
+    GemmChoice c = conv_choose(args, f1_cu_count());
+    if (const GemmKernel* twin = conv_bnbwd_twin(args, c)) {
+        c.k = twin;
+        args.bnb_rif = conv_bnbwd_rif(a.Cm, a.P);
+        if (bnb_rows) *bnb_rows = a.P / (8 * args.bnb_rif);
+    }
     if (c.rc == DALI_ERR_LIMIT) return c.refuse();
     const int K = a.g.nr * a.g.ns * a.g.Ck;
     char what[160] = "";
@@ -2255,8 +2370,10 @@
     return gemm_launch(st, c, args);
 }
 
-int launch_igemm_conv(hipStream_t st, const IGemmArgs& a) {
+int launch_igemm_conv(hipStream_t st, const IGemmArgs& a, int* bnb_rows) {
     IGemmArgs args = a;
+    if (bnb_rows) *bnb_rows = 0;
+    else args.bnb_slab = nullptr;
     args.stamps = g_conv_stamps;
     GatherGeom& g = args.g;
     g.sub = 0; g.oph = g.opw = 0; g.Hfull = g.Hout; g.Wfull = g.Wout;
@@ -2293,7 +2410,7 @@
             return DALI_OK;
         }
     }
-    return launch_igemm_conv_one(st, args);
+    return launch_igemm_conv_one(st, args, bnb_rows);
 }
 
 static bool wgrad_spec(int Cm, int Ntot) { return ((Cm + 127) / 128) * ((Ntot + 255) / 256) <= 100; }
@@ -2514,6 +2631,25 @@
     return launch_igemm_conv((hipStream_t)stream, a);
 }
 
+extern "C" int dali_conv2d_dgrad_bnstats(dali_ctx* ctx, void* stream, const uint16_t* dy, const uint16_t* dy2, int ck1, const uint16_t* wt, const float* bias,
+                                         uint16_t* dx, int n, int h, int wd, int cin, int cout, int r, int s, int stride, int pad, const uint16_t* raw,
+                                         const float* mean, const float* invstd, const float* scale, const float* shift, float* slab, int64_t slab_floats) {
+    DALI_REQUIRE(ctx && dy && wt && dx && raw && mean && invstd && scale && shift && slab, "dali_conv2d_dgrad_bnstats: null argument");
+    DALI_REQUIRE(cout % 32 == 0 && cin % 4 == 0, "dali_conv2d_dgrad_bnstats: cout must be a multiple of 32 and cin of 4 (cin=%d cout=%d)", cin, cout);
+    DALI_REQUIRE(stride == 1 || stride == 2, "dali_conv2d_dgrad_bnstats: stride %d unsupported", stride);
+    DALI_REQUIRE(!dy2 || (r == 1 && s == 1 && stride == 1 && pad == 0 && ck1 > 0 && ck1 < cout), "dali_conv2d_dgrad_bnstats: dy2 needs 1x1 / stride 1 and 0 < ck1 < cout (ck1=%d)", ck1);
+    const int ho = (h + 2 * pad - r) / stride + 1, wo = (wd + 2 * pad - s) / stride + 1;
+    IGemmArgs a{};
+    a.W = wt; a.X = dy; a.X2 = dy2; a.Ck1 = dy2 ? ck1 : 0; a.O = dx; a.bias = bias;
+    a.Cm = cin; a.P = n * h * wd;
+    DALI_REQUIRE(slab_floats >= (int64_t)igemm_conv_bnb_max_rows(a.P) * cin * 2, "dali_conv2d_dgrad_bnstats: the slab needs ceil(pixels / 32) * cin * 2 floats (cin=%d)", cin);
+    a.bnb = BnBwdSide{raw, mean, invstd, scale, shift}; a.bnb_slab = slab;
+    fill_geom(a.g, n, ho, wo, cout, h, wd, r, s, stride, pad, 1);
+    int rows = 0;
+    const int rc = launch_igemm_conv((hipStream_t)stream, a, &rows);
+    return rc ? rc : rows;
+}
+
 extern "C" int dali_conv2d_wgrad(dali_ctx* ctx, void* stream, const uint16_t* x, const uint16_t* dy, float* dw,
                                  int n, int h, int wd, int cin, int cout, int r, int s, int stride, int pad,
                                  const float* in_scale, const float* in_shift, int in_relu, int accumulate) {
diff --git a/daliid_amd/csrc/kernels.h b/daliid_amd/csrc/kernels.h
--- a/daliid_amd/csrc/kernels.h
+++ b/daliid_amd/csrc/kernels.h
@@ -16,6 +16,8 @@
     int r0, rstep, nr, s0, sstep, ns;
     int class_grid;
 };
+
+struct BnBwdSide { const uint16_t* raw; const float* mean; const float* invstd; const float* scale; const float* shift; };
 
 struct IGemmArgs {
     const uint16_t* W;
@@ -43,6 +45,9 @@
     const uint16_t* X2;
     int Ck1;
     int x_rep;
+    BnBwdSide bnb;
+    float* bnb_slab;
+    int bnb_rif;
 };
 
 struct WGradArgs {
@@ -61,9 +66,8 @@
 struct TransposeJob { const uint16_t* w; uint16_t* wt; int Co, T, Ci, first_block; };
 int launch_weight_transpose_batched(hipStream_t st, const TransposeJob* jobs, int n);
 
-struct BnBwdSide { const uint16_t* raw; const float* mean; const float* invstd; const float* scale; const float* shift; };
-
-int launch_igemm_conv(hipStream_t st, const IGemmArgs& a);
+int launch_igemm_conv(hipStream_t st, const IGemmArgs& a, int* bnb_rows = nullptr);
+inline int igemm_conv_bnb_max_rows(int P) { return (P + 31) / 32; }
 int gemm_profile_begin(hipStream_t st, int cls, double flops, const char* what);
 void gemm_profile_end(hipStream_t st, int slot);
 int igemm_conv_stat_tiles(int Cm, int P, int K, bool operand_transform = false);
@@ -105,7 +109,7 @@
 size_t bn_bwd_partial_floats(int P, int C, bool dual);
 int launch_bn_bwd(hipStream_t st, const uint16_t* g, const uint16_t* ymask, const uint8_t* ybits, const BnBwdSide& a, const BnBwdSide* b, int relu, int P, int C,
                   float* partial, float* coef_a, float* coef_b, float* dgamma_a, float* dbeta_a, float* dgamma_b, float* dbeta_b,
-                  uint16_t* draw_a, uint16_t* draw_b, uint16_t* dz_out, double* scratch);
+                  uint16_t* draw_a, uint16_t* draw_b, uint16_t* dz_out, double* scratch, int filled_rows = 0);
 GatherGeom stem_geom(int H, int W);
 int launch_stem_pack_image(hipStream_t st, const float* img, int N, int H, int W, uint16_t* out);
 int launch_stem_pack_weight(hipStream_t st, const float* w, int Cout, uint16_t* out);
diff --git a/daliid_amd/csrc/nnops.hip b/daliid_amd/csrc/nnops.hip
--- a/daliid_amd/csrc/nnops.hip
+++ b/daliid_amd/csrc/nnops.hip
@@ -688,15 +688,18 @@
 }
 int launch_bn_bwd(hipStream_t st, const uint16_t* g, const uint16_t* ymask, const uint8_t* ybits, const BnBwdSide& a, const BnBwdSide* b, int relu, int P, int C,
                   float* partial, float* coef_a, float* coef_b, float* dgamma_a, float* dbeta_a, float* dgamma_b, float* dbeta_b,
-                  uint16_t* draw_a, uint16_t* draw_b, uint16_t* dz_out, double* scratch) {
+                  uint16_t* draw_a, uint16_t* draw_b, uint16_t* dz_out, double* scratch, int filled_rows) {
     int rpb;
-    const int blocks = bn_bwd_blocks(P, C, &rpb);
+    int blocks = bn_bwd_blocks(P, C, &rpb);
     const int rif = 256 / (C / 8);
     const bool dual = b != nullptr;
     const int NV = dual ? 3 : 2;
     const size_t lds = (size_t)rif * C * NV * sizeof(float);
     BnBwdSide bb = dual ? *b : a;
-    if (dual) {
+    if (filled_rows > 0) {
+        if (dual || ymask || ybits || !relu) { set_error("bn_bwd: pre-filled partial sums are those of one side with the recomputed ReLU mask"); return DALI_ERR_INVALID; }
+        blocks = filled_rows;
+    } else if (dual) {
         hipLaunchKernelGGL(bn_bwd_reduce_kernel<true>, dim3(blocks), dim3(256), lds, st, g, ymask, ybits, a, bb, relu, P, C, rpb, partial);
     } else {
         hipLaunchKernelGGL(bn_bwd_reduce_kernel<false>, dim3(blocks), dim3(256), lds, st, g, ymask, ybits, a, bb, relu, P, C, rpb, partial);
@@ -881,6 +884,24 @@
                          dgamma_b, dbeta_b, draw_a, draw_b, dz_out, scratch);
 }
 
+extern "C" int dali_bn_bwd_partials(dali_ctx* ctx, void* stream, const uint16_t* g, int64_t pixels, int C, const uint16_t* raw, const float* mean,
+                                    const float* invstd, const float* scale, const float* shift, const float* partial, int rows, float* dgamma,
+                                    float* dbeta, uint16_t* draw, float* coef) {
+    DALI_REQUIRE(ctx && g && raw && mean && invstd && scale && shift && dgamma && dbeta && draw, "dali_bn_bwd_partials: null argument");
+    DALI_REQUIRE(C % 8 == 0 && C <= 2048 && pixels > 0 && pixels < (1ll << 31), "dali_bn_bwd_partials: C must be a multiple of 8, <= 2048");
+    DALI_REQUIRE(rows >= 0 && (rows == 0 || partial), "dali_bn_bwd_partials: rows > 0 needs the partial sums");
+    const size_t pf = bn_bwd_partial_floats((int)pixels, C, false);
+    const size_t need = align_up(pf * 4, 256) + align_up((size_t)C * 12, 256) + reduce_scratch_bytes(C, 2);
+    char* ws = static_cast<char*>(workspace(ctx, need));
+    if (!ws) return DALI_ERR_NOMEM;
+    float* own_partial = reinterpret_cast<float*>(ws);
+    float* coef_a = coef ? coef : reinterpret_cast<float*>(ws + align_up(pf * 4, 256));
+    double* scratch = reinterpret_cast<double*>(ws + align_up(pf * 4, 256) + align_up((size_t)C * 12, 256));
+    const BnBwdSide a{raw, mean, invstd, scale, shift};
+    return launch_bn_bwd((hipStream_t)stream, g, nullptr, nullptr, a, nullptr, 1, (int)pixels, C, rows ? const_cast<float*>(partial) : own_partial, coef_a, nullptr,
+                         dgamma, dbeta, nullptr, nullptr, draw, nullptr, nullptr, scratch, rows);
+}
+
 extern "C" int dali_maxpool_bn_fwd(dali_ctx* ctx, void* stream, const uint16_t* raw, const float* scale, const float* shift, int n, int h,
                                    int w, int C, uint16_t* out, uint8_t* arg) {
     DALI_REQUIRE(ctx && raw && scale && shift && out && arg, "dali_maxpool_bn_fwd: null argument");
diff --git a/daliid_amd/csrc/resnet_plan.hip b/daliid_amd/csrc/resnet_plan.hip
--- a/daliid_amd/csrc/resnet_plan.hip
+++ b/daliid_amd/csrc/resnet_plan.hip
@@ -327,23 +327,24 @@
 }
 
 int conv_dgrad(dali_resnet* net, hipStream_t st, const Conv& c, const uint16_t* dy, const uint16_t* residual, uint16_t* dx,
-               const uint8_t* out_mask = nullptr) {
+               const uint8_t* out_mask = nullptr, const Bn* next = nullptr, const uint16_t* raw = nullptr, int* rows = nullptr) {
     IGemmArgs a{};
     a.W = c.wt_bf16; a.X = dy; a.O = dx; a.Res = residual; a.out_mask = out_mask;
     a.Cm = c.cin; a.P = net->N * c.hin * c.win;
     a.g = conv_geom(c, 1);
-    return launch_igemm_conv(st, a);
+    if (next) { a.bnb = BnBwdSide{raw, next->mean, next->invstd, next->scale, next->shift}; a.bnb_slab = net->bwd_partial; }
+    return launch_igemm_conv(st, a, rows);
 }
 
 int cat_gemm(dali_resnet* net, hipStream_t st, const Conv& c, int mode, const uint16_t* W, const uint16_t* X, int c1, const uint16_t* X2, int c2, int Cm,
-             uint16_t* O, IGemmArgs stage = IGemmArgs{}) {
+             uint16_t* O, IGemmArgs stage = IGemmArgs{}, int* bnb_rows = nullptr) {
     IGemmArgs& a = stage;
     a.W = W; a.X = X; a.X2 = X2; a.Ck1 = c1; a.O = O;
     a.Cm = Cm; a.P = net->N * (mode == 0 ? c.hout * c.wout : c.hin * c.win);
     Conv cat = c;
     (mode == 0 ? cat.cin : cat.cout) = (a.x_rep ? a.x_rep : 1) * (c1 + c2);
     a.g = conv_geom(cat, mode);
-    return launch_igemm_conv(st, a);
+    return launch_igemm_conv(st, a, bnb_rows);
 }
 
 int linbn_fwd(dali_resnet* net, hipStream_t st, LinBn& l, const Conv& c, Bn& bn, const uint16_t* x) {
@@ -364,10 +365,10 @@
                             net->G + bn.b_off, l.wd, l.wd + l.C, l.bvec, l.qk, ld, ld);
 }
 
-int bn_bwd(dali_resnet* net, hipStream_t st, const Bn& bn, const uint16_t* raw, const uint16_t* g, int relu, int P, uint16_t* out) {
+int bn_bwd(dali_resnet* net, hipStream_t st, const Bn& bn, const uint16_t* raw, const uint16_t* g, int relu, int P, uint16_t* out, int rows = 0) {
     const BnBwdSide s{raw, bn.mean, bn.invstd, bn.scale, bn.shift};
-    return launch_bn_bwd(st, g, nullptr, nullptr, s, nullptr, relu, P, bn.C, net->bwd_partial, bn.coef, nullptr, net->G + bn.g_off, net->G + bn.b_off,
-                         nullptr, nullptr, out, nullptr, nullptr, net->red_scratch);
+    return launch_bn_bwd(st, g, nullptr, nullptr, s, nullptr, relu, P, bn.C, net->bwd_partial, bn.coef, nullptr, net->G + bn.g_off,
+                         net->G + bn.b_off, nullptr, nullptr, out, nullptr, nullptr, net->red_scratch, rows);
 }
 
 uint16_t* next_gbuf(dali_resnet* net, const uint16_t* avoid0, const uint16_t* avoid1 = nullptr, const uint16_t* avoid2 = nullptr,
@@ -471,25 +472,29 @@
     uint16_t* dz = net->cur_dy;
     const int Pout = net->N * b.hout * b.wout, Pin = net->N * b.hin * b.win;
     uint16_t* d_rawd = nullptr;
+    int rows2 = 0;
     if ((rc = linbn_bwd(net, st, b.l3, b.c3, b.b3, dz, b.a2, b.sdz, true))) return rc;
     uint16_t* d_a2 = next_gbuf(net, dz);
     uint16_t* scratch_a = next_gbuf(net, dz, d_a2);
+    if (b.has_ds && !b.lin_ds) {
+        d_rawd = next_gbuf(net, dz, d_a2, scratch_a);
+        if ((rc = bn_bwd(net, st, b.bd, b.rawd, dz, 0, Pout, d_rawd))) return rc;
+    }
     {
         IGemmArgs stage{};
         stage.bias = b.l3.bvec;
-        if ((rc = cat_gemm(net, st, b.c3, 1, b.l3.wd, dz, b.cout, b.a2, b.width, b.width, d_a2, stage))) return rc;
+        stage.bnb = BnBwdSide{b.raw2, b.b2.mean, b.b2.invstd, b.b2.scale, b.b2.shift}; stage.bnb_slab = net->bwd_partial;
+        if ((rc = cat_gemm(net, st, b.c3, 1, b.l3.wd, dz, b.cout, b.a2, b.width, b.width, d_a2, stage, &rows2))) return rc;
     }
     if (b.lin_ds) {
         if ((rc = linbn_bwd(net, st, b.ld, b.cd, b.bd, dz, b.x, b.sdz, false))) return rc;
-    } else if (b.has_ds) {
-        d_rawd = next_gbuf(net, dz, d_a2, scratch_a);
-        if ((rc = bn_bwd(net, st, b.bd, b.rawd, dz, 0, Pout, d_rawd))) return rc;
-    }
-    if ((rc = bn_bwd(net, st, b.b2, b.raw2, d_a2, 1, Pout, d_a2))) return rc;
+    }
+    if ((rc = bn_bwd(net, st, b.b2, b.raw2, d_a2, 1, Pout, d_a2, rows2))) return rc;
     if ((rc = conv_wgrad(net, st, b.c2, b.a1, d_a2))) return rc;
     uint16_t* d_a1 = scratch_a;
-    if ((rc = conv_dgrad(net, st, b.c2, d_a2, nullptr, d_a1))) return rc;
-    if ((rc = bn_bwd(net, st, b.b1, b.raw1, d_a1, 1, Pin, d_a1))) return rc;
+    int rows1 = 0;
+    if ((rc = conv_dgrad(net, st, b.c2, d_a2, nullptr, d_a1, nullptr, &b.b1, b.raw1, &rows1))) return rc;
+    if ((rc = bn_bwd(net, st, b.b1, b.raw1, d_a1, 1, Pin, d_a1, rows1))) return rc;
     b.dbg_d_raw1 = d_a1;
     if ((rc = conv_wgrad(net, st, b.c1, b.x, d_a1))) return rc;
     uint16_t* dx = d_a2;
diff --git a/daliid_amd/ops_nn.py b/daliid_amd/ops_nn.py
--- a/daliid_amd/ops_nn.py
+++ b/daliid_amd/ops_nn.py
@@ -60,6 +60,36 @@
                                              n, h, wd, cin, cout, r, s, stride, pad),
                "dali_conv2d_dgrad")
     return dx
+
+
+def conv2d_dgrad_bnstats(dy, wt, x_hw, raw, mean, invstd, scale, shift, stride=1, pad=0, bias=None, dy2=None):
+    n, ho, wo, c1 = dy.shape
+    cin, r, s, cout = wt.shape
+    h, wd = x_hw
+    assert _out_hw(h, wd, r, s, stride, pad) == (ho, wo) and cout == c1 + (dy2.shape[3] if dy2 is not None else 0)
+    assert tuple(raw.shape) == (n, h, wd, cin)
+    dx = torch.empty(n, h, wd, cin, device=dy.device, dtype=bf16)
+    slab = torch.zeros((n * h * wd + 31) // 32, cin, 2, device=dy.device, dtype=torch.float32)
+    rows = _lib.lib().dali_conv2d_dgrad_bnstats(_lib.ctx(dy.device), _lib.stream_ptr(), _lib.ptr(dy, bf16, "dy"), _lib.ptr(dy2, bf16, "dy2"), c1,
+                                                _lib.ptr(wt, bf16, "wt"), _lib.ptr(bias, torch.float32, "bias"), _lib.ptr(dx), n, h, wd, cin, cout, r, s,
+                                                stride, pad, _lib.ptr(raw, bf16, "raw"), _lib.ptr(mean, torch.float32, "mean"),
+                                                _lib.ptr(invstd, torch.float32, "invstd"), _lib.ptr(scale, torch.float32, "scale"),
+                                                _lib.ptr(shift, torch.float32, "shift"), _lib.ptr(slab), slab.numel())
+    if rows < 0:
+        _lib.check(rows, "dali_conv2d_dgrad_bnstats")
+    return dx, slab[:rows], rows
+
+
+def bn_bwd_partials(g, raw, mean, invstd, scale, shift, slab=None):
+    C = g.shape[-1]
+    dev = g.device
+    rows = 0 if slab is None else slab.shape[0]
+    draw, dga, dba, coef = torch.empty_like(g), _f32(C, dev), _f32(C, dev), torch.empty(3, C, device=dev, dtype=torch.float32)
+    _lib.check(_lib.lib().dali_bn_bwd_partials(_lib.ctx(dev), _lib.stream_ptr(), _lib.ptr(g, bf16, "g"), g.numel() // C, C, _lib.ptr(raw, bf16, "raw"),
+                                                _lib.ptr(mean), _lib.ptr(invstd), _lib.ptr(scale), _lib.ptr(shift),
+                                                _lib.ptr(slab if rows else None), rows, _lib.ptr(dga), _lib.ptr(dba), _lib.ptr(draw), _lib.ptr(coef)),
+               "dali_bn_bwd_partials")
+    return draw, dga, dba, coef
 
 
 def conv2d_wgrad(x, dy, rs, stride=1, pad=0, in_scale=None, in_shift=None, in_relu=False, out=None, accumulate=False):
diff --git a/include/daliid.h b/include/daliid.h
--- a/include/daliid.h
+++ b/include/daliid.h
@@ -109,6 +109,9 @@
 int dali_conv2d_dgrad(dali_ctx* ctx, void* stream, const uint16_t* dy, const uint16_t* wt, uint16_t* dx,
                       const uint16_t* residual, const uint8_t* residual_mask, int n, int h, int wd, int cin, int cout, int r, int s,
                       int stride, int pad);
+int dali_conv2d_dgrad_bnstats(dali_ctx* ctx, void* stream, const uint16_t* dy, const uint16_t* dy2, int ck1, const uint16_t* wt, const float* bias,
+                              uint16_t* dx, int n, int h, int wd, int cin, int cout, int r, int s, int stride, int pad, const uint16_t* raw,
+                              const float* mean, const float* invstd, const float* scale, const float* shift, float* slab, int64_t slab_floats);
 int dali_conv2d_wgrad(dali_ctx* ctx, void* stream, const uint16_t* x, const uint16_t* dy, float* dw,
                       int n, int h, int wd, int cin, int cout, int r, int s, int stride, int pad,
                       const float* in_scale, const float* in_shift, int in_relu, int accumulate);
@@ -125,6 +128,9 @@
                 const uint16_t* raw_b, const float* mean_b, const float* invstd_b, const float* scale_b,
                 float* dgamma_a, float* dbeta_a, float* dgamma_b, float* dbeta_b, uint16_t* draw_a, uint16_t* draw_b,
                 uint16_t* dz_out);
+int dali_bn_bwd_partials(dali_ctx* ctx, void* stream, const uint16_t* g, int64_t pixels, int C, const uint16_t* raw, const float* mean,
+                         const float* invstd, const float* scale, const float* shift, const float* partial, int rows, float* dgamma,
+                         float* dbeta, uint16_t* draw, float* coef);
 int dali_maxpool_bn_fwd(dali_ctx* ctx, void* stream, const uint16_t* raw, const float* scale, const float* shift, int n, int h,
                         int w, int C, uint16_t* out, uint8_t* arg);
 int dali_maxpool_bn_bwd(dali_ctx* ctx, void* stream, const uint16_t* dpool, const uint8_t* arg, const uint16_t* raw,
```

Measured after the change: 17870 images/s, median of 6. About the same (+0.7%).
